# fhausmann/deepgrp

Measured on AMD Instinct MI355X. Metric: Mbp/sec predicted (whole node) at window=200 stride=50, 5-class, higher is better.
Workload: dtype f16

## Files before the change

deepgrp_amd/_lib.py:

```python
from __future__ import annotations

import ctypes as C
import os

_HERE = os.path.dirname(os.path.abspath(__file__))
LIB_PATH = os.path.join(_HERE, "libdeepgrp_hip.so")

i64, i32, vp, cint = C.c_int64, C.c_int32, C.c_void_p, C.c_int


class DgrpError(RuntimeError):
    """A libdeepgrp_hip call failed (message from dgrp_last_error())."""


class Segment(C.Structure):
    _fields_ = [("start", C.c_int64), ("end", C.c_int64), ("label", C.c_int32), ("contig", C.c_int32)]


class TrainJob(C.Structure):
    _fields_ = [("T", cint), ("u", cint), ("C", cint), ("attention", cint), ("d_params", vp), ("d_idx", vp), ("d_truth", vp),
                ("n", i64), ("d_starts", vp), ("B", i64), ("d_masks", vp), ("d_loss", vp), ("d_grads", vp), ("d_work", vp),
                ("work_bytes", i64)]


# ... 11 lines not shown
    "dgrp_fasta_batch_workspace_bytes": (i64, [i64, i64]),
    "dgrp_fasta_encode_batch": (cint, [vp, i64, vp, vp, vp, vp, vp, i64, vp]),
    "dgrp_fasta_chunks_workspace_bytes": (i64, [i64]),
    "dgrp_fasta_chunks": (cint, [vp, i64, i64, vp, vp, C.POINTER(i64), vp, i64, vp]),
    "dgrp_fasta_mask_workspace_bytes": (i64, [i64, i64, i64]),
    "dgrp_fasta_mask_batch": (cint, [vp, i64, vp, vp, vp, vp, cint, C.c_uint64, vp, vp, i64, vp]),
    "dgrp_fasta_extract_workspace_bytes": (i64, [i64, i64, i64]),
    "dgrp_fasta_extract_batch": (cint, [vp, i64, vp, vp, vp, vp, vp, vp, i64, cint, C.c_uint64, vp, i64, C.POINTER(i64), vp, C.POINTER(i64),
                                        vp, i64, vp]),
    "dgrp_twobit_workspace_bytes": (i64, [i64]),
    "dgrp_twobit_encode_batch": (cint, [vp, i64, i64, vp, vp, vp, vp, i64, vp, vp, i64, vp, i64, vp]),
    "dgrp_twobit_text_batch": (cint, [vp, i64, i64, vp, vp, vp, vp, vp, vp, i64, vp, vp, i64, vp, vp, i64, vp, i64, vp]),
    "dgrp_twobit_pack_workspace_bytes": (i64, [i64, i64]),
    "dgrp_twobit_pack_batch": (cint, [vp, i64, vp, vp, vp, i64, i64, vp, vp, vp, i64, vp]),
    "dgrp_format_rows_bound": (i64, [i64, i64]),
    "dgrp_format_rows": (cint, [vp, vp, i64, cint, vp, i64, vp, i64, C.POINTER(i64)]),
    "dgrp_track_workspace_bytes": (i64, [i64, i64]),
    "dgrp_track_text": (cint, [vp, i64, cint, cint, cint, i64, i64, C.c_char_p, i64, vp, i64, C.POINTER(i64), vp, i64, vp]),
    "dgrp_track_batch_workspace_bytes": (i64, [i64, vp, vp, i64, cint, i64]),
    "dgrp_track_text_batch": (cint, [vp, cint, i64, vp, vp, vp, C.c_char_p, vp, vp, cint, cint, i64, vp, i64, vp, vp, i64, vp]),
    "dgrp_track_index_workspace_bytes": (i64, [i64, vp, vp, i64, cint, i64]),
    "dgrp_track_index_batch": (cint, [vp, cint, i64, vp, vp, vp, C.c_char_p, vp, vp, cint, cint, i64, vp, i64, vp, vp, i64, vp, i64, vp]),
    "dgrp_track_sections_workspace_bytes": (i64, [i64, vp, vp, i64, cint]),
    "dgrp_track_sections_batch": (cint, [vp, cint, i64, vp, vp, vp, vp, cint, cint, i64, i64, vp, i64, vp, vp, i64, vp, vp, i64, vp]),
    "dgrp_track_zoom_workspace_bytes": (i64, [i64, vp, vp, i64, cint]),
    "dgrp_track_zoom_batch": (cint, [vp, cint, i64, vp, vp, vp, vp, cint, cint, i64, i64, vp, i64, vp, vp, i64, vp, vp, vp, i64, vp]),
    "dgrp_zlib_bound": (i64, [i64, i64]),
    "dgrp_zlib_workspace_bytes": (i64, [i64, cint]),
    "dgrp_zlib_compress_batch": (cint, [vp, i64, vp, i64, i64, cint, vp, i64, vp, C.POINTER(i64), vp, i64, vp]),
    "dgrp_zlib_compress_host": (cint, [vp, i64, vp, i64, i64, cint, vp, i64, vp, C.POINTER(i64)]),
    "dgrp_window_count":(i64, [i64, i64, i64]),
    "dgrp_windows_onehot": (cint, [vp, i64, i64, i64, i64, i64, cint, vp, vp]),
    "dgrp_model_create": (cint, [C.POINTER(vp), cint, cint, cint, cint, vp, vp, vp, vp, vp, vp]),
    "dgrp_model_create_lstm": (cint, [C.POINTER(vp), cint, cint, cint, vp, vp, vp, vp, vp]),
    "dgrp_model_destroy": (cint, [vp]),
    "dgrp_model_dims": (cint, [vp, C.POINTER(cint), C.POINTER(cint), C.POINTER(cint), C.POINTER(cint)]),
    "dgrp_model_flags": (cint, [vp]),
    "dgrp_model_set_precision": (cint, [vp, cint]),
    "dgrp_model_view": (cint, [vp, cint, C.POINTER(vp)]),
    "dgrp_model_plan": (cint, [vp, cint, i64, C.POINTER(cint), C.POINTER(i64), C.POINTER(cint), C.POINTER(cint)]),
    "dgrp_forward_workspace_bytes": (i64, [vp, i64]),
    "dgrp_forward_window_chunk": (i64, [vp]),
    "dgrp_forward_windows": (cint, [vp, vp, i64, i64, i64, i64, vp, vp, i64, vp]),
    "dgrp_forward_merge": (cint, [vp, vp, i64, i64, i64, i64, i64, vp, vp, i64, vp]),
    "dgrp_forward_merge_record": (cint, [vp, vp, i64, i64, i64, vp, vp, i64, vp]),
    "dgrp_forward_merge_record_workspace_bytes": (i64, [vp, i64, i64]),
    "dgrp_forward_reference_workspace_bytes": (i64, [vp, i64]),
    "dgrp_forward_windows_reference": (cint, [vp, vp, i64, i64, i64, i64, vp, vp, i64, vp]),
    "dgrp_get_max": (cint, [vp, i64, vp, i64, i64, i64, i64, vp]),
    "dgrp_scores": (cint, [vp, i64, cint, vp, vp, vp]),
    "dgrp_softmax_labels": (cint, [vp, i64, cint, vp, vp, vp, i64, vp]),
    "dgrp_mss_workspace_bytes": (i64, [i64]),
    "dgrp_mss_labels": (cint, [vp, vp, i64, cint, cint, cint, vp, vp, vp, i64, vp]),
    "dgrp_mss_segments_host": (cint, [vp, i64, vp, i64, C.POINTER(i64)]),
    "dgrp_mss_batch_workspace_bytes": (i64, [i64, i64]),
    "dgrp_mss_labels_batch": (cint, [vp, vp, i64, i64, vp, cint, cint, cint, vp, vp, i64, vp]),
    "dgrp_segments_workspace_bytes": (i64, [i64]),
    "dgrp_segments": (cint, [vp, i64, i64, i32, vp, i64, vp, vp, i64, vp]),
    "dgrp_record_workspace_bytes": (i64, [vp, i64, i64, cint]),
    "dgrp_predict_record": (cint, [vp, vp, i64, i64, i64, cint, cint, cint, i64, i32, vp, i64, C.POINTER(i64), vp, i64, vp]),
    "dgrp_batch_workspace_bytes": (i64, [vp, i64, vp, i64]),
    "dgrp_predict_batch": (cint, [vp, vp, i64, vp, vp, vp, vp, i64, i64, cint, cint, vp, i64, C.POINTER(i64), vp, i64, vp]),
    "dgrp_batch_rows": (i64, [i64, vp]),
    "dgrp_predict_batch_probs": (cint, [vp, vp, i64, vp, vp, vp, vp, i64, i64, cint, cint, vp, i64, C.POINTER(i64), vp, i64, vp, vp]),
    "dgrp_confusion_matrix": (cint, [vp, vp, i64, cint, vp, vp, vp]),
    "dgrp_filter_segments": (cint, [vp, vp, i64, i64, vp]),
    "dgrp_eval_workspace_bytes": (i64, [i64, i64]),
    "dgrp_paint_rows_batch": (cint, [vp, i64, vp, vp, vp, vp, vp, vp, i64, vp]),
    "dgrp_row_hits_batch": (cint, [vp, i64, vp, vp, vp, vp, vp, vp, vp, i64, vp]),
    "dgrp_row_scores_workspace_bytes": (i64, [i64, i64]),
    "dgrp_row_scores_batch": (cint, [vp, cint, i64, vp, vp, vp, vp, vp, vp, vp, i64, vp]),
    "dgrp_prob_hist_workspace_bytes": (i64, [i64, cint, cint]),
    "dgrp_prob_hist_batch": (cint, [vp, cint, i64, vp, vp, vp, vp, cint, vp, vp, vp, i64, vp]),
    "dgrp_row_detect_workspace_bytes": (i64, [i64, i64]),
    "dgrp_paint_row_keys_batch": (cint, [vp, i64, vp, vp, vp, vp, vp, vp, vp, i64, vp]),
    "dgrp_row_detect_batch": (cint, [vp, i64, vp, vp, vp, vp, vp, vp, vp, vp, i64, vp]),
    "dgrp_format_bed_bound": (i64, [i64, i64]),
    "dgrp_format_bed_rows": (cint, [vp, vp, i64, cint, vp, vp, i64, cint, vp, i64, C.POINTER(i64)]),
    "dgrp_bed_text_workspace_bytes": (i64, [i64, i64, i64]),
    "dgrp_bed_text_batch": (cint, [vp, vp, i64, cint, vp, vp, i64, cint, vp, i64, C.POINTER(i64), vp, i64, vp]),
    "dgrp_bed_index_workspace_bytes": (i64, [i64, i64, i64, i64]),
    "dgrp_bed_index_batch": (cint, [vp, vp, i64, cint, vp, vp, i64, cint, i64, vp, vp, i64, C.POINTER(i64), vp, i64, vp, vp, i64, vp]),
    "dgrp_gff_text_workspace_bytes": (i64, [i64, i64, i64, i64, i64]),
    "dgrp_gff_text_batch": (cint, [vp, vp, i64, cint, vp, vp, i64, vp, vp, i64, cint, i64, vp, i64, C.POINTER(i64), C.POINTER(i64), vp, i64,
                                   vp]),
    "dgrp_gff_index_workspace_bytes": (i64, [i64, i64, i64, i64, i64, i64]),
    "dgrp_gff_index_batch": (cint, [vp, vp, i64, cint, vp, vp, i64, vp, vp, i64, cint, i64, i64, vp, vp, i64, C.POINTER(i64), vp, i64, vp, vp,
                                    i64, vp]),
    "dgrp_bed_blocks_workspace_bytes": (i64, [i64, i64, vp]),
    "dgrp_bed_blocks_batch": (cint, [cint, vp, vp, i64, cint, i64, vp, i64, vp, i64, C.POINTER(i64), vp, i64, C.POINTER(i64), C.POINTER(i64),
                                     vp, i64, vp]),
    "dgrp_bed_zoom_workspace_bytes": (i64, [i64, i64, vp]),
    "dgrp_bed_zoom_batch": (cint, [cint, vp, vp, i64, cint, i64, vp, i64, vp, i64, vp, vp, i64, vp, vp, vp, i64, vp]),
    "dgrp_inflate_raw_host": (cint, [vp, i64, vp, i64, C.POINTER(i64), C.POINTER(i64), C.POINTER(cint)]),
    "dgrp_inflate_workspace_bytes": (i64, [i64]),
    "dgrp_inflate_batch": (cint, [vp, i64, i64, vp, vp, vp, vp, i64, C.POINTER(i64), C.POINTER(cint), vp, i64, vp]),
    "dgrp_bgzf_bound": (i64, [i64, cint]),
    "dgrp_bgzf_workspace_bytes": (i64, [i64]),
    "dgrp_bgzf_compress": (cint, [vp, i64, vp, i64, C.POINTER(i64), cint, vp, i64, vp]),
    "dgrp_bgzf_compress_host": (cint, [vp, i64, vp, i64, C.POINTER(i64), cint]),
    "dgrp_bgzf_workspace_bytes_level": (i64, [i64, cint]),
    "dgrp_bgzf_compress_level": (cint, [vp, i64, vp, i64, C.POINTER(i64), cint, cint, vp, i64, vp]),
    "dgrp_bgzf_compress_host_level": (cint, [vp, i64, vp, i64, C.POINTER(i64), cint, cint]),
    "dgrp_train_param_count": (i64, [cint, cint, cint]),
    "dgrp_train_workspace_bytes": (i64, [cint, cint, cint, cint, i64]),
    "dgrp_train_step": (cint, [cint, cint, cint, cint, vp, vp, vp, i64, vp, i64, vp, vp, vp, vp, i64, vp]),
# ... 50 lines not shown
```

deepgrp_amd/csrc/api.hip:

```cpp
#include "dgrp_model.h"

#include <stdarg.h>
#include <string.h>

#include <algorithm>
#include <vector>
#include <mutex>

static thread_local char g_err[512] = "";

void dgrp_set_error(const char *fmt, ...)
{
    va_list ap;
    va_start(ap, fmt);
    vsnprintf(g_err, sizeof(g_err), fmt, ap);
    va_end(ap);
}

DGRP_EXPORT int dgrp_abi_version(void) { return DGRP_ABI_VERSION; }
DGRP_EXPORT const char *dgrp_last_error(void) { return g_err; }

DGRP_EXPORT int dgrp_device_info(char *name, size_t name_cap, int *cu_count, int64_t *hbm_bytes)
{
    int dev = 0;
// ... 795 lines not shown

struct record_layout {
    int64_t out, scores, cls, labels, count, fwd, post, bytes, post_bytes, fwd_bytes;
};

static record_layout record_carve(const dgrp_model *m, int64_t n, int64_t s, int use_mss)
{
    record_layout l;
    int64_t p = 0;
    auto take = [&](int64_t b) { const int64_t q = p; p += dgrp_align_up(b, 256); return q; };
    const int64_t nwin = dgrp_window_count(n, m->T, s);
    l.out = take(n * m->C * 4);
    l.scores = take(use_mss ? n * 8 : 0);
    l.cls = take(use_mss ? n : 0);
    l.labels = take(n);
    l.count = take(8);
    l.fwd_bytes = record_forward_bytes(m, nwin);
    l.fwd = take(l.fwd_bytes);
    l.post_bytes = std::max<int64_t>(std::max<int64_t>(use_mss ? dgrp_mss_workspace_bytes(n) : 4096, dgrp_segments_workspace_bytes(n)), 4096);
    l.post = take(l.post_bytes);
    l.bytes = p;
    return l;
}

DGRP_EXPORT int64_t dgrp_record_workspace_bytes(const dgrp_model *m, int64_t n, int64_t s, int use_mss)
{
    if (!m || n < 0 || s < 1) return 0;
    return record_carve(m, n, s, use_mss).bytes;
}

DGRP_EXPORT int dgrp_predict_record(const dgrp_model *m, const uint8_t *d_idx, int64_t n, int64_t s, int64_t batch,
                                    int min_mss_len, int xdrop_len, int use_mss, int64_t offset, int32_t contig,
                                    dgrp_segment *d_records, int64_t cap, int64_t *h_count, void *d_work,
                                    int64_t work_bytes, void *stream_)
{
    hipStream_t stream = (hipStream_t)stream_;
    DGRP_REQUIRE(m && n >= 0 && s >= 1 && batch >= 1 && cap >= 0 && h_count, "dgrp_predict_record: bad arguments");
    *h_count = 0;
    if (n == 0) return DGRP_OK;
    DGRP_REQUIRE(d_idx && d_work && (cap == 0 || d_records), "dgrp_predict_record: NULL pointer");
    const record_layout l = record_carve(m, n, s, use_mss);
    if (work_bytes < l.bytes) {
        dgrp_set_error("dgrp_predict_record: workspace %lld < %lld bytes", (long long)work_bytes, (long long)l.bytes);
        return DGRP_ENOMEM;
    }
    char *w = (char *)d_work;
    float *out = (float *)(w + l.out);
    int8_t *labels = (int8_t *)(w + l.labels);
    int64_t *d_count = (int64_t *)(w + l.count);
    DGRP_HIP(hipMemsetAsync(out, 0, (size_t)n * m->C * 4, stream));
    int rc = dgrp_forward_merge_record(m, d_idx, n, s, batch, out, w + l.fwd, l.fwd_bytes, stream);
    if (rc) return rc;
    if (use_mss) {
        rc = dgrp_scores(out, n, m->C, (double *)(w + l.scores), (int8_t *)(w + l.cls), stream);
        if (rc) return rc;
        rc = dgrp_mss_labels((const double *)(w + l.scores), (const int8_t *)(w + l.cls), n, m->C, min_mss_len, xdrop_len,
                             labels, nullptr, w + l.post, l.post_bytes, stream);
    } else {
        rc = dgrp_softmax_labels(out, n, m->C, nullptr, labels, w + l.post, l.post_bytes, stream);
    }
    if (rc) return rc;
    rc = dgrp_segments(labels, n, offset, contig, d_records, cap, d_count, w + l.post, l.post_bytes, stream);
    if (rc) return rc;
    DGRP_HIP(hipMemcpyAsync(h_count, d_count, 8, hipMemcpyDeviceToHost, stream));
    DGRP_HIP(hipStreamSynchronize(stream));
    return DGRP_OK;
}

int dgrp_batch_marks(const int64_t *d_start, const int64_t *d_len, int64_t nrec, int64_t total_n, uint8_t *d_marks,
                     double *d_scores, int8_t *d_cls, hipStream_t stream);
int dgrp_batch_segments(const int8_t *d_labels, const uint8_t *d_marks, int64_t total_n, const int64_t *d_start, int64_t nrec,
                        const int64_t *d_startpos, const int32_t *d_contig, dgrp_segment *d_records, int64_t cap,
                        int64_t *d_count, void *d_work, int64_t work_bytes, hipStream_t stream);

struct batch_layout {
    int64_t out, scores, cls, labels, marks, count, recs, wgf, start, len, spos, contig, post, post_bytes, avg, pl, queue, bytes;
};

static batch_layout batch_carve(const dgrp_model *m, int64_t nrec, int64_t total_rows, int64_t total_windows)
{
    batch_layout l;
    int64_t p = 0;
    auto take = [&](int64_t b) { const int64_t q = p; p += dgrp_align_up(b, 256); return q; };
    l.out = take(total_rows * m->C * 4);
    l.scores = take(total_rows * 8);
    l.cls = take(total_rows);
    l.labels = take(total_rows);
    l.marks = take(total_rows);
    l.count = take(8);
    l.recs = take(nrec * 64);
    l.wgf = take((nrec + 1) * 8);
    l.start = take((nrec + 1) * 8);
    l.len = take(nrec * 8);
    l.spos = take(nrec * 8);
    l.contig = take(nrec * 4);
    l.post_bytes = std::max<int64_t>(std::max<int64_t>(dgrp_mss_batch_workspace_bytes(total_rows, nrec), dgrp_segments_workspace_bytes(total_rows)), 4096);
    l.post = take(l.post_bytes);
    l.avg = take(m->attention ? total_windows * m->T * (int64_t)m->UP * 4 : 0);
    l.pl = take(m->attention ? total_windows * m->T * (int64_t)m->C * 4 : 0);
    l.queue = take(4);
    l.bytes = p;
    return l;
}

static int64_t batch_windows(const dgrp_model *m, int64_t nrec, const int64_t *h_n, int64_t s)
{
    int64_t w = 0;
    for (int64_t r = 0; r < nrec; ++r) w += dgrp_window_count(h_n[r], m->T, s);
    return w;
}
// ... 114 lines not shown
```

deepgrp_amd/csrc/bigbed_kernels.hip:

```cpp
#include "dgrp_common.h"
#include "bbi_zoom.h"
#include "bed_rows.h"
#include "scan.h"
#include <string.h>
#include <vector>

namespace {

#define BB_BLOCK_ITEMS 512
#define BB_ITEM_MAX 60
#define BB_MAX_END 0xffffffffll
#define BB_R0 1024

struct bb_in {
    const dgrp_segment *rows;
    const dgrp_row_score *scores;
    int64_t nrows;
    const int64_t *rec_end;
    int64_t nrec;
    int by_contig;
    uint64_t min_score;
};

__device__ __forceinline__ int64_t bb_rec(const bb_in &A, const dgrp_segment &row) { return A.by_contig ? row.contig : 0; }
// ... 330 lines not shown
                                    dgrp_track_zoom_block *d_table, int64_t table_cap, int64_t *h_block_off, dgrp_track_totals *h_totals,
                                    void *d_work, int64_t work_bytes, void *stream_)
{
    static const char who[] = "dgrp_bed_zoom_batch";
    hipStream_t stream = (hipStream_t)stream_;
    DGRP_REQUIRE(h_record_off && h_block_off && h_totals, "%s: NULL h_record_off, h_block_off or h_totals", who);
    for (int s = 0; s <= BBI_LEVELS; ++s) h_record_off[s] = h_block_off[s] = 0;
    memset(h_totals, 0, sizeof *h_totals);
    const int rc = bb_check(who, by_contig, nrows, nrec, h_rec_end, chrom0, cap, table_cap);
    if (rc != DGRP_OK) return rc;
    if (nrows == 0) return DGRP_OK;
    DGRP_REQUIRE(d_rows && d_scores && (d_out || cap == 0) && (d_table || table_cap == 0), "%s: bad arguments (NULL rows, scores, output or table)",
                 who);
    DGRP_REQUIRE(((uintptr_t)d_out & 15) == 0 && ((uintptr_t)d_table & 7) == 0, "%s: d_out must be 16-byte and d_table 8-byte aligned", who);
    bbz_layout l;
    DGRP_REQUIRE(bbz_carve(nrows, nrec, h_rec_end, &l), "%s: too many zoom windows in one call", who);
    if (!d_work || work_bytes < l.bytes) {
        dgrp_set_error("%s: workspace too small (%lld < %lld bytes)", who, (long long)work_bytes, (long long)l.bytes);
        return DGRP_ENOMEM;
    }
    char *w = (char *)d_work;
    const bbi_levels &Z = l.Z;
    const std::vector<int64_t> wpref = bbi_wpref(Z, nrec, nullptr, h_rec_end);
    int64_t *d_wpref = (int64_t *)(w + l.wpref);
    DGRP_HIP(hipMemcpyAsync(d_wpref, wpref.data(), wpref.size() * 8, hipMemcpyHostToDevice, stream));
    std::vector<int64_t> tab;
    bb_in A;
    int rc2 = bb_front(by_contig, d_rows, d_scores, nrows, min_score, nrec, h_rec_end, w, l.rec_end, l.eidx, 0, l.len, l.tiles, stream, tab, &A);
    if (rc2 != DGRP_OK) return rc2;
    bed_head *d_head = (bed_head *)w;
    uint64_t *eidx = (uint64_t *)(w + l.eidx), *len = (uint64_t *)(w + l.len), *tiles = (uint64_t *)(w + l.tiles);
    uint64_t *wtiles = (uint64_t *)(w + l.wtiles), *grand = (uint64_t *)(w + l.grand), *segb = (uint64_t *)(w + l.segb);
    bbz_win *win = (bbz_win *)(w + l.win);
    bbz_rows Rw;
    Rw.count = &d_head->lines;
    Rw.skey = (uint64_t *)(w + l.skey); Rw.ekey = (uint64_t *)(w + l.ekey); Rw.lpref = (uint64_t *)(w + l.lpref);
    const dim3 grid((unsigned)((nrows + 255) / 256)), block(256);
    uint64_t *lsum = (uint64_t *)(w + l.lsum);
    rc2 = device_exclusive_scan(len, lsum, nrows, tiles, nullptr, stream);
    if (rc2 != DGRP_OK) return rc2;
    hipLaunchKernelGGL(bbz_compact_kernel, grid, block, 0, stream, A, (const uint64_t *)len, (const uint64_t *)lsum, (const uint64_t *)eidx, Rw);
    DGRP_LAUNCH_CHECK();
    hipLaunchKernelGGL(bbz_level0_kernel, dim3((unsigned)((Z.seg[1] - Z.seg[0]) / 256)), block, 0, stream, Rw, A.rec_end, (const int64_t *)d_wpref,
                       nrec, Z, win);
    DGRP_LAUNCH_CHECK();
    for (int k = 1; k < BBI_LEVELS; ++k) {
        hipLaunchKernelGGL((bbi_reduce_kernel<bbz_win, bbz_start>), dim3((unsigned)((Z.seg[k + 1] - Z.seg[k]) / 256)), block, 0, stream, bbz_start(),
                           (const int64_t *)d_wpref, nrec, Z, k, win);
        DGRP_LAUNCH_CHECK();
    }
    const int64_t ntiles = Z.seg[BBI_LEVELS] / 256;
    hipLaunchKernelGGL(bbi_count_kernel<bbz_win>, dim3((unsigned)ntiles), block, 0, stream, (const bbz_win *)win, wtiles);
    DGRP_LAUNCH_CHECK();
    hipLaunchKernelGGL(scan_sums_kernel, dim3(1), block, 0, stream, wtiles, ntiles, grand);
    DGRP_LAUNCH_CHECK();
    hipLaunchKernelGGL((bbi_bounds_kernel<bbz_win, true>), dim3(1), block, 0, stream, (const bbz_win *)win, (const uint64_t *)wtiles,
                       (const uint64_t *)grand, Z, 1, segb, grand + 1);
    DGRP_LAUNCH_CHECK();
    bed_head head;
    uint64_t off[2 * (BBI_LEVELS + 1)], covered = 0;
    DGRP_HIP(hipMemcpyAsync(&head, w, sizeof head, hipMemcpyDeviceToHost, stream));
    DGRP_HIP(hipMemcpyAsync(off, segb, sizeof off, hipMemcpyDeviceToHost, stream));
    DGRP_HIP(hipMemcpyAsync(&covered, grand + 1, 8, hipMemcpyDeviceToHost, stream));
    DGRP_HIP(hipStreamSynchronize(stream));
    rc2 = bed_refusal(who, head);
    if (rc2 != DGRP_OK) return rc2;
    for (int s = 0; s <= BBI_LEVELS; ++s) {
        h_record_off[s] = (int64_t)off[s];
        h_block_off[s] = (int64_t)off[BBI_LEVELS + 1 + s];
    }
    if (covered) {
        h_totals->covered = h_totals->sum = h_totals->sumsq = covered;
        h_totals->qmin = h_totals->qmax = 1;
    }
    if (h_record_off[BBI_LEVELS] == 0 || 32 * h_record_off[BBI_LEVELS] > cap || h_block_off[BBI_LEVELS] > table_cap) return DGRP_OK;
    hipLaunchKernelGGL((bbi_write_kernel<bbz_win, bbz_tail>), dim3((unsigned)ntiles), block, 0, stream, (const bbz_win *)win, (const int64_t *)d_wpref,
                       nrec, Z, bbz_tail(), (const uint64_t *)wtiles, (const uint64_t *)segb, 1, (uint32_t)chrom0, (uint4 *)d_out, d_table);
    DGRP_LAUNCH_CHECK();
    return DGRP_OK;
}
```

deepgrp_amd/csrc/bigwig_kernels.hip:

```cpp
#include "dgrp_common.h"
#include "deflate.h"
#include "deflate_blocks.h"
#include "scan.h"
#include "track_chain.h"
#include "bbi_zoom.h"
#include <string.h>
#include <vector>

namespace {

#define BW_SECTION_ITEMS 1024
#define BW_MAX_END 0xffffffffll

__device__ __forceinline__ float bw_value(uint64_t v, double scale) { return (float)((double)v / scale); }

struct bw_run { uint32_t v; bool first, last; int64_t r, lo, hi; };

__device__ __forceinline__ bw_run bw_run_of(const uint32_t *__restrict__ qk, const tb_rec *__restrict__ recs,
                                            const int64_t *__restrict__ pref, const tb_geom &G, int64_t r0, int64_t f0, int64_t f)
{
    bw_run t;
    t.v = f < G.NB ? qk[f] : 0u;
    t.first = t.last = false;
    t.r = t.lo = t.hi = 0;
// ... 396 lines not shown
}

static int64_t zlib_workspace(int64_t nblk, int level)
{
    const int64_t base = dgrp_align_up(nblk * DGRP_BGZF_SLOT, 256) + dgrp_align_up((nblk + 2) * 8, 256);
    return level == 0 ? base : base + nblk * DGRP_BGZF_BLOCK * (int64_t)sizeof(uint32_t);
}

}

DGRP_EXPORT int64_t dgrp_track_sections_workspace_bytes(int64_t nrec, const int64_t *h_n, const int64_t *h_startpos, int64_t bin, int ncls)
{
    bws_layout l;
    if (bin < 1 || ncls < 1) return 0;
    return bws_carve(nrec, h_n, h_startpos, bin, ncls, &l) ? l.bytes : 0;
}

DGRP_EXPORT int dgrp_track_sections_batch(const float *d_probs, int C, int64_t nrec, const int64_t *h_row0, const int64_t *h_n,
                                          const int64_t *h_startpos, const int *h_cls, int ncls, int digits, int64_t bin, int64_t chrom0,
                                          char *d_out, int64_t cap, int64_t *h_class_off, dgrp_track_section *d_table, int64_t table_cap,
                                          int64_t *h_section_off, void *d_work, int64_t work_bytes, void *stream_)
{
    const char *who = "dgrp_track_sections_batch";
    DGRP_REQUIRE(h_class_off && h_section_off, "%s: NULL h_class_off or h_section_off", who);
    if (ncls >= 1 && ncls <= DGRP_MAXC)
        for (int k = 0; k <= ncls; ++k) h_class_off[k] = h_section_off[k] = 0;
    const int rc0 = bw_check(who, d_probs, C, nrec, h_row0, h_n, h_startpos, h_cls, ncls, digits, bin, chrom0);
    if (rc0 != DGRP_OK) return rc0;
    DGRP_REQUIRE(cap >= 0 && table_cap >= 0, "%s: bad cap/table_cap (%lld, %lld)", who, (long long)cap, (long long)table_cap);
    if (nrec == 0) return DGRP_OK;
    DGRP_REQUIRE((d_out || cap == 0) && (d_table || table_cap == 0) && d_work, "%s: NULL pointer", who);
    DGRP_REQUIRE(((uintptr_t)d_out & 3) == 0 && ((uintptr_t)d_table & 7) == 0, "%s: d_out must be 4-byte and d_table 8-byte aligned", who);
    bws_layout l;
    DGRP_REQUIRE(bws_carve(nrec, h_n, h_startpos, bin, ncls, &l), "%s: too many bins in one call", who);
    if (work_bytes < l.bytes) {
        dgrp_set_error("%s: workspace %lld < %lld bytes", who, (long long)work_bytes, (long long)l.bytes);
        return DGRP_ENOMEM;
    }
    hipStream_t stream = (hipStream_t)stream_;
    char *w = (char *)d_work;
    unsigned long long *cnt = (unsigned long long *)(w + l.cnt);
    uint64_t *ipref = (uint64_t *)(w + l.ipref), *spref = (uint64_t *)(w + l.spref), *base = (uint64_t *)(w + l.base);
    uint64_t *hb = (uint64_t *)(w + l.hb);
    std::vector<int64_t> name_off((size_t)nrec + 1, 0);
    std::vector<char> tab;
    tb_dev D;
    const int rc = dgrp_tb_bins(d_probs, C, nrec, h_row0, h_n, h_startpos, nullptr, name_off.data(), h_cls, ncls, digits, bin, d_work, l.t,
                                stream, tab, &D);
    if (rc != DGRP_OK) return rc;
    DGRP_HIP(hipMemsetAsync(cnt, 0, (size_t)(nrec * ncls) * 8, stream));
    const dim3 grid((unsigned)D.ntiles), block(256);
    hipLaunchKernelGGL(bw_count_kernel, grid, block, 0, stream, D.q, D.recs, D.pref, D.G, D.tiles, cnt);
    DGRP_LAUNCH_CHECK();
    hipLaunchKernelGGL(scan_sums_kernel, dim3(1), block, 0, stream, D.tiles, D.ntiles, D.grand);
    DGRP_LAUNCH_CHECK();
    hipLaunchKernelGGL(bw_prefix_kernel, dim3((unsigned)ncls), block, 0, stream, cnt, nrec, ipref, spref);
    DGRP_LAUNCH_CHECK();
    hipLaunchKernelGGL(bw_bounds_kernel, dim3(1), dim3(64), 0, stream, ipref, spref, nrec, ncls, base, hb);
    DGRP_LAUNCH_CHECK();
    std::vector<uint64_t> off(2 * ((size_t)ncls + 1), 0);
    DGRP_HIP(hipMemcpyAsync(off.data(), hb, off.size() * 8, hipMemcpyDeviceToHost, stream));
    DGRP_HIP(hipStreamSynchronize(stream));
    for (int k = 0; k <= ncls; ++k) {
        h_class_off[k] = (int64_t)off[(size_t)k];
        h_section_off[k] = (int64_t)off[(size_t)(ncls + 1 + k)];
    }
    if (h_class_off[ncls] == 0 || h_class_off[ncls] > cap || h_section_off[ncls] > table_cap) return DGRP_OK;
    double scale = 1.0;
    for (int k = 0; k < digits; ++k) scale *= 10.0;
    hipLaunchKernelGGL(bw_write_kernel, grid, block, 0, stream, D.q, D.recs, D.pref, D.G, scale, D.tiles, cnt, ipref, spref, base, (uint32_t)chrom0,
                       d_out, d_table);
    DGRP_LAUNCH_CHECK();
    DGRP_HIP(hipStreamSynchronize(stream));
    return DGRP_OK;
}

DGRP_EXPORT int64_t dgrp_track_zoom_workspace_bytes(int64_t nrec, const int64_t *h_n, const int64_t *h_startpos, int64_t bin, int ncls)
{
    bwz_layout l;
    if (bin < 1 || ncls < 1) return 0;
    return bwz_carve(nrec, h_n, h_startpos, bin, ncls, &l) ? l.bytes : 0;
}

DGRP_EXPORT int dgrp_track_zoom_batch(const float *d_probs, int C, int64_t nrec, const int64_t *h_row0, const int64_t *h_n,
                                      const int64_t *h_startpos, const int *h_cls, int ncls, int digits, int64_t bin, int64_t chrom0,
                                      char *d_out, int64_t cap, int64_t *h_record_off, dgrp_track_zoom_block *d_table, int64_t table_cap,
                                      int64_t *h_block_off, dgrp_track_totals *h_totals, void *d_work, int64_t work_bytes, void *stream_)
{
    const char *who = "dgrp_track_zoom_batch";
    DGRP_REQUIRE(h_record_off && h_block_off && h_totals, "%s: NULL h_record_off, h_block_off or h_totals", who);
    if (ncls >= 1 && ncls <= DGRP_MAXC) {
        for (int s = 0; s <= ncls * BBI_LEVELS; ++s) h_record_off[s] = h_block_off[s] = 0;
        memset(h_totals, 0, (size_t)ncls * sizeof(dgrp_track_totals));
    }
    const int rc0 = bw_check(who, d_probs, C, nrec, h_row0, h_n, h_startpos, h_cls, ncls, digits, bin, chrom0);
    if (rc0 != DGRP_OK) return rc0;
    DGRP_REQUIRE(bin <= (1ll << 32), "%s: bad bin %lld (zoom windows of 16 * bin * 4^9 bases)", who, (long long)bin);
    DGRP_REQUIRE(cap >= 0 && table_cap >= 0, "%s: bad cap/table_cap (%lld, %lld)", who, (long long)cap, (long long)table_cap);
    if (nrec == 0) return DGRP_OK;
    DGRP_REQUIRE((d_out || cap == 0) && (d_table || table_cap == 0) && d_work, "%s: NULL pointer", who);
    DGRP_REQUIRE(((uintptr_t)d_out & 15) == 0 && ((uintptr_t)d_table & 7) == 0, "%s: d_out must be 16-byte and d_table 8-byte aligned", who);
    bwz_layout l;
    DGRP_REQUIRE(bwz_carve(nrec, h_n, h_startpos, bin, ncls, &l), "%s: too many bins in one call", who);
    if (work_bytes < l.bytes) {
        dgrp_set_error("%s: workspace %lld < %lld bytes", who, (long long)work_bytes, (long long)l.bytes);
        return DGRP_ENOMEM;
    }
    hipStream_t stream = (hipStream_t)stream_;
    char *w = (char *)d_work;
    const bbi_levels &Z = l.Z;
    int64_t *d_wpref = (int64_t *)(w + l.wpref);
    bwz_win *win = (bwz_win *)(w + l.win);
    uint64_t *tiles = (uint64_t *)(w + l.tiles), *grand = (uint64_t *)(w + l.grand), *segb = (uint64_t *)(w + l.segb);
    dgrp_track_totals *d_totals = (dgrp_track_totals *)(w + l.totals);
    const int nseg = ncls * BBI_LEVELS;
    const std::vector<int64_t> wpref = bbi_wpref(Z, nrec, h_startpos, h_n);
    DGRP_HIP(hipMemcpyAsync(d_wpref, wpref.data(), wpref.size() * 8, hipMemcpyHostToDevice, stream));
    std::vector<int64_t> name_off((size_t)nrec + 1, 0);
    std::vector<char> tab;
    tb_dev D;
    const int rc = dgrp_tb_bins(d_probs, C, nrec, h_row0, h_n, h_startpos, nullptr, name_off.data(), h_cls, ncls, digits, bin, d_work, l.t,
                                stream, tab, &D);
    if (rc != DGRP_OK) return rc;
    const dim3 block(256);
    hipLaunchKernelGGL(bwz_level0_kernel, dim3((unsigned)((Z.seg[1] - Z.seg[0]) / 256 * ncls)), block, 0, stream, D.q, D.recs, D.pref, d_wpref,
                       D.G, Z, win);
    DGRP_LAUNCH_CHECK();
    for (int k = 1; k < BBI_LEVELS; ++k) {
        hipLaunchKernelGGL((bbi_reduce_kernel<bwz_win, bwz_start>), dim3((unsigned)((Z.seg[k + 1] - Z.seg[k]) / 256 * ncls)), block, 0, stream,
                           bwz_start{D.recs}, d_wpref, nrec, Z, k, win);
        DGRP_LAUNCH_CHECK();
    }
    const int64_t ntiles = Z.seg[BBI_LEVELS] / 256 * ncls;
    hipLaunchKernelGGL(bbi_count_kernel<bwz_win>, dim3((unsigned)ntiles), block, 0, stream, win, tiles);
    DGRP_LAUNCH_CHECK();
    hipLaunchKernelGGL(scan_sums_kernel, dim3(1), block, 0, stream, tiles, ntiles, grand);
    DGRP_LAUNCH_CHECK();
    hipLaunchKernelGGL((bbi_bounds_kernel<bwz_win, false>), dim3(1), dim3(64), 0, stream, win, tiles, grand, Z, ncls, segb, nullptr);
    DGRP_LAUNCH_CHECK();
    hipLaunchKernelGGL(bwz_totals_kernel, dim3((unsigned)ncls), block, 0, stream, win, Z, d_totals);
    DGRP_LAUNCH_CHECK();
    std::vector<uint64_t> off(2 * ((size_t)nseg + 1), 0);
    DGRP_HIP(hipMemcpyAsync(off.data(), segb, off.size() * 8, hipMemcpyDeviceToHost, stream));
    DGRP_HIP(hipMemcpyAsync(h_totals, d_totals, (size_t)ncls * sizeof(dgrp_track_totals), hipMemcpyDeviceToHost, stream));
    DGRP_HIP(hipStreamSynchronize(stream));
    for (int s = 0; s <= nseg; ++s) {
        h_record_off[s] = (int64_t)off[(size_t)s];
        h_block_off[s] = (int64_t)off[(size_t)(nseg + 1 + s)];
    }
    if (h_record_off[nseg] == 0 || 32 * h_record_off[nseg] > cap || h_block_off[nseg] > table_cap) return DGRP_OK;
    double scale = 1.0;
    for (int k = 0; k < digits; ++k) scale *= 10.0;
    hipLaunchKernelGGL((bbi_write_kernel<bwz_win, bwz_tail>), dim3((unsigned)ntiles), block, 0, stream, win, d_wpref, nrec, Z, bwz_tail{scale}, tiles,
                       segb, ncls, (uint32_t)chrom0, (uint4 *)d_out, d_table);
    DGRP_LAUNCH_CHECK();
    DGRP_HIP(hipStreamSynchronize(stream));
    return DGRP_OK;
}

DGRP_EXPORT int64_t dgrp_zlib_bound(int64_t nblk, int64_t in_bytes) { return nblk < 0 || in_bytes < 0 ? 0 : in_bytes + ZLIB_EMPTY * nblk; }

DGRP_EXPORT int64_t dgrp_zlib_workspace_bytes(int64_t nblk, int level)
{
    return nblk < 0 || nblk > INT32_MAX - 1 || level < 0 || level > 1 ? 0 : zlib_workspace(nblk, level);
}

DGRP_EXPORT int dgrp_zlib_compress_batch(const uint8_t *d_in, int64_t in_bytes, const void *d_rows, int64_t stride, int64_t nblk, int level,
                                         uint8_t *d_out, int64_t out_cap, int64_t *d_sizes, int64_t *h_out_bytes, void *d_work,
                                         int64_t work_bytes, void *stream_)
{
    const char *who = "dgrp_zlib_compress_batch";
    DGRP_REQUIRE(h_out_bytes, "%s: NULL h_out_bytes", who);
    *h_out_bytes = 0;
    DGRP_REQUIRE(in_bytes >= 0 && nblk >= 0 && nblk <= INT32_MAX - 1 && out_cap >= 0 && work_bytes >= 0, "%s: bad arguments", who);
    DGRP_REQUIRE(stride >= 16 && stride % 8 == 0, "%s: a row is at least an int64 offset and an int64 length (stride %lld)", who,
                 (long long)stride);
    DGRP_REQUIRE(level == 0 || level == 1, "%s: level %d (0: literals, 1: matches)", who, level);
    if (nblk == 0) return DGRP_OK;
    DGRP_REQUIRE((d_in || in_bytes == 0) && d_rows && (d_out || out_cap == 0) && d_sizes && d_work, "%s: NULL pointer", who);
    DGRP_REQUIRE(((uintptr_t)d_work & 15) == 0 && ((uintptr_t)d_rows & 7) == 0, "%s: d_work must be 16-byte, d_rows 8-byte aligned", who);
    if (work_bytes < zlib_workspace(nblk, level)) {
        dgrp_set_error("%s: workspace too small", who);
        return DGRP_ENOMEM;
    }
    hipStream_t stream = (hipStream_t)stream_;
    uint8_t *slots = (uint8_t *)d_work;
    uint64_t *sizes = (uint64_t *)(slots + dgrp_align_up(nblk * DGRP_BGZF_SLOT, 256));
    uint32_t *lz = level == 0 ? nullptr : (uint32_t *)((uint8_t *)sizes + dgrp_align_up((nblk + 2) * 8, 256));
    unsigned long long *bad = (unsigned long long *)(sizes + nblk + 1);
    const char *rows = (const char *)d_rows;
    DGRP_HIP(hipMemsetAsync(bad, 0, 8, stream));
    const int rc = dgrp_deflate_members(d_in, in_bytes, rows, stride, nblk, level, slots, sizes, lz, stream);
    if (rc != DGRP_OK) return rc;
    hipLaunchKernelGGL(zlib_sizes_kernel, dim3((unsigned)((nblk + 255) / 256)), dim3(256), 0, stream, rows, stride, nblk, in_bytes, sizes, bad);
    DGRP_LAUNCH_CHECK();
    hipLaunchKernelGGL(scan_sums_kernel, dim3(1), dim3(256), 0, stream, sizes, nblk, sizes + nblk);
    DGRP_LAUNCH_CHECK();
    hipLaunchKernelGGL(zlib_place_kernel, dim3((unsigned)nblk), dim3(256), 0, stream, d_in, rows, stride, slots, sizes, nblk, bad, d_out, out_cap,
                       d_sizes);
    DGRP_LAUNCH_CHECK();
    uint64_t tail[2] = {0, 0};
    DGRP_HIP(hipMemcpyAsync(tail, sizes + nblk, 16, hipMemcpyDeviceToHost, stream));
    DGRP_HIP(hipStreamSynchronize(stream));
    DGRP_REQUIRE(tail[1] == 0, "%s: %llu rows do not lie in the input or are longer than 65280 bytes (nothing written)", who,
                 (unsigned long long)tail[1]);
    *h_out_bytes = (int64_t)tail[0];
    if (*h_out_bytes > out_cap) {
        dgrp_set_error("%s: output of %lld bytes, %lld needed (nothing written)", who, (long long)out_cap, (long long)*h_out_bytes);
        return DGRP_ENOMEM;
    }
    return DGRP_OK;
}

DGRP_EXPORT int dgrp_zlib_compress_host(const uint8_t *h_in, int64_t in_bytes, const void *h_rows, int64_t stride, int64_t nblk, int level,
                                        uint8_t *h_out, int64_t out_cap, int64_t *h_sizes, int64_t *h_out_bytes)
{
    const char *who = "dgrp_zlib_compress_host";
    DGRP_REQUIRE(h_out_bytes, "%s: NULL h_out_bytes", who);
    *h_out_bytes = 0;
    DGRP_REQUIRE(in_bytes >= 0 && nblk >= 0 && out_cap >= 0, "%s: bad arguments", who);
    DGRP_REQUIRE(stride >= 16 && stride % 8 == 0, "%s: a row is at least an int64 offset and an int64 length (stride %lld)", who,
                 (long long)stride);
    DGRP_REQUIRE(level == 0 || level == 1, "%s: level %d (0: literals, 1: matches)", who, level);
    if (nblk == 0) return DGRP_OK;
    DGRP_REQUIRE((h_in || in_bytes == 0) && h_rows && (h_out || out_cap == 0) && h_sizes, "%s: NULL pointer", who);
    for (int64_t m = 0; m < nblk; ++m) {
        const int64_t *row = (const int64_t *)((const char *)h_rows + m * stride);
        DGRP_REQUIRE(row[0] >= 0 && row[1] >= 0 && row[1] <= DGRP_BGZF_BLOCK && row[0] <= in_bytes - row[1],
                     "%s: row %lld (offset %lld, %lld bytes) does not lie in the input or is longer than 65280 bytes", who, (long long)m,
                     (long long)row[0], (long long)row[1]);
    }
    std::vector<uint32_t> slot(DGRP_BGZF_SLOT / 4), lz(level ? DGRP_BGZF_BLOCK : 0);
    std::vector<uint16_t> head(level ? 1 << DGRP_LZ_HASH_BITS : 0);
    dgrp_deflate_plan plan;
    dgrp_lz_plan lzplan;
    int64_t pos = 0;
    bool fits = true;
    for (int64_t m = 0; m < nblk; ++m) {
        const int64_t *row = (const int64_t *)((const char *)h_rows + m * stride);
        const uint8_t *src = h_in + row[0];
        const uint32_t len = (uint32_t)row[1];
        uint32_t size = ZLIB_EMPTY;
        if (len > 0)
            size = (level ? dgrp_bgzf_member_serial_lz(src, len, slot.data(), &plan, &lzplan, lz.data(), head.data())
                          : dgrp_bgzf_member_serial(src, len, slot.data(), &plan)) - 20;
        uint32_t a = 1, b = 0;
        for (uint32_t i = 0; i < len; ++i) {
            a = (a + src[i]) % ZLIB_MOD;
            b = (b + a) % ZLIB_MOD;
// ... 24 lines not shown
```

deepgrp_amd/csrc/deflate_kernels.hip:

```cpp
#include "dgrp_common.h"
#include "deflate.h"
#include "deflate_blocks.h"
#include "scan.h"
#include <string.h>
#include <mutex>
#include <vector>

namespace {

#define DEFLATE_THREADS 256
#define DEFLATE_RUN 16
#define DEFLATE_ROUND (DEFLATE_THREADS * DEFLATE_RUN)

struct deflate_shared {
    dgrp_deflate_plan plan;
    uint32_t hist[DEFLATE_THREADS / 64][DGRP_DEFLATE_NSYM];
    uint32_t crctab[256];
    uint64_t scan[4];
    uint32_t crc[DEFLATE_THREADS / 64];
};
struct deflate_lds {
    uint32_t image[DGRP_BGZF_SLOT / 4];
    deflate_shared s;
};
// ... 484 lines not shown

DGRP_EXPORT int64_t dgrp_bgzf_workspace_bytes(int64_t n) { return n < 0 ? 0 : bgzf_workspace(n, 0); }

DGRP_EXPORT int64_t dgrp_bgzf_workspace_bytes_level(int64_t n, int level)
{
    return n < 0 || level < 0 || level > 1 ? 0 : bgzf_workspace(n, level);
}

static int bgzf_compress_device(const char *who, const uint8_t *d_in, int64_t n, uint8_t *d_out, int64_t out_cap, int64_t *h_out_bytes, int eof,
                                int level, void *d_work, int64_t work_bytes, hipStream_t stream)
{
    if (!(n >= 0 && out_cap >= 0 && work_bytes >= 0 && h_out_bytes)) {
        dgrp_set_error("%s: bad arguments", who);
        return DGRP_EINVAL;
    }
    *h_out_bytes = 0;
    const int64_t nmem = bgzf_members(n);
    if (level < 0 || level > 1) {
        dgrp_set_error("%s: level %d (0: literals, 1: matches)", who, level);
        return DGRP_EINVAL;
    }
    if (nmem > INT32_MAX - 1) {
        dgrp_set_error("%s: too many members", who);
        return DGRP_EINVAL;
    }
    if (!(n == 0 || (d_in && d_work)) || !(d_out || (n == 0 && !eof) || out_cap == 0)) {
        dgrp_set_error("%s: NULL pointer", who);
        return DGRP_EINVAL;
    }
    if (n == 0) {
        if (!eof) return DGRP_OK;
        *h_out_bytes = DGRP_BGZF_EOF_BYTES;
        if (out_cap < DGRP_BGZF_EOF_BYTES) {
            dgrp_set_error("%s: output of %lld bytes, the EOF member takes %d", who, (long long)out_cap, DGRP_BGZF_EOF_BYTES);
            return DGRP_ENOMEM;
        }
        DGRP_HIP(hipMemcpyAsync(d_out, BGZF_EOF_MEMBER, DGRP_BGZF_EOF_BYTES, hipMemcpyHostToDevice, stream));
        DGRP_HIP(hipStreamSynchronize(stream));
        return DGRP_OK;
    }
    if (work_bytes < bgzf_workspace(n, level)) {
        dgrp_set_error("%s: workspace too small", who);
        return DGRP_ENOMEM;
    }
    if (((uintptr_t)d_work & 15) != 0) {
        dgrp_set_error("%s: d_work must be 16-byte aligned", who);
        return DGRP_EINVAL;
    }
    uint8_t *slots = (uint8_t *)d_work;
    uint64_t *sizes = (uint64_t *)(slots + dgrp_align_up(nmem * DGRP_BGZF_SLOT, 256));
    uint32_t *lz = level == 0 ? nullptr : (uint32_t *)((uint8_t *)sizes + dgrp_align_up((nmem + 1) * 8, 256));
    const int rc = dgrp_deflate_members(d_in, n, nullptr, 0, nmem, level, slots, sizes, lz, stream);
    if (rc != DGRP_OK) return rc;
    hipLaunchKernelGGL(scan_sums_kernel, dim3(1), dim3(256), 0, stream, sizes, nmem, sizes + nmem);
    DGRP_LAUNCH_CHECK();
    hipLaunchKernelGGL(bgzf_place_kernel, dim3((unsigned)(nmem + (eof ? 1 : 0))), dim3(256), 0, stream, slots, sizes, nmem, eof, d_out, out_cap);
    DGRP_LAUNCH_CHECK();
    uint64_t all = 0;
    DGRP_HIP(hipMemcpyAsync(&all, sizes + nmem, 8, hipMemcpyDeviceToHost, stream));
    DGRP_HIP(hipStreamSynchronize(stream));
    *h_out_bytes = (int64_t)all + (eof ? DGRP_BGZF_EOF_BYTES : 0);
    if (*h_out_bytes > out_cap) {
        dgrp_set_error("%s: output of %lld bytes, %lld needed (nothing written)", who, (long long)out_cap, (long long)*h_out_bytes);
        return DGRP_ENOMEM;
    }
    return DGRP_OK;
}

static int bgzf_compress_host(const char *who, const uint8_t *h_in, int64_t n, uint8_t *h_out, int64_t out_cap, int64_t *h_out_bytes, int eof,
                              int level)
{
    if (!(n >= 0 && out_cap >= 0 && h_out_bytes)) {
        dgrp_set_error("%s: bad arguments", who);
        return DGRP_EINVAL;
    }
    *h_out_bytes = 0;
    if (level < 0 || level > 1) {
        dgrp_set_error("%s: level %d (0: literals, 1: matches)", who, level);
        return DGRP_EINVAL;
    }
    if (!(h_in || n == 0) || !(h_out || (n == 0 && !eof) || out_cap == 0)) {
        dgrp_set_error("%s: NULL pointer", who);
        return DGRP_EINVAL;
    }
    std::vector<uint32_t> slot(DGRP_BGZF_SLOT / 4), lz(level ? DGRP_BGZF_BLOCK : 0);
    std::vector<uint16_t> head(level ? 1 << DGRP_LZ_HASH_BITS : 0);
    dgrp_deflate_plan plan;
    dgrp_lz_plan lzplan;
    int64_t pos = 0;
    bool fits = true;
    for (int64_t o = 0; o < n; o += DGRP_BGZF_BLOCK) {
        const uint32_t k = (uint32_t)(n - o < DGRP_BGZF_BLOCK ? n - o : DGRP_BGZF_BLOCK);
        const uint32_t size = level ? dgrp_bgzf_member_serial_lz(h_in + o, k, slot.data(), &plan, &lzplan, lz.data(), head.data())
                                    : dgrp_bgzf_member_serial(h_in + o, k, slot.data(), &plan);
        fits = fits && pos + size <= out_cap;
        if (fits) memcpy(h_out + pos, slot.data(), size);
        pos += size;
    }
    if (eof) {
        fits = fits && pos + DGRP_BGZF_EOF_BYTES <= out_cap;
        if (fits) memcpy(h_out + pos, BGZF_EOF_MEMBER, DGRP_BGZF_EOF_BYTES);
        pos += DGRP_BGZF_EOF_BYTES;
    }
    *h_out_bytes = pos;
    if (!fits) {
        dgrp_set_error("%s: output of %lld bytes, %lld needed", who, (long long)out_cap, (long long)pos);
        return DGRP_ENOMEM;
// ... 28 lines not shown
```

deepgrp_amd/csrc/extract_kernels.hip:

```cpp
#include "dgrp_common.h"
#include "body_tiles.h"
#include "scan.h"
#include <vector>

namespace {

#define EXTRACT_TILE 4096
#define BODY_WORDS (BODY_TILE / 16)

__global__ void __launch_bounds__(256) extract_count_kernel(const uint8_t *__restrict__ raw, const int64_t *__restrict__ tile0,
                                                            const int64_t *__restrict__ off, const int64_t *__restrict__ len,
                                                            int64_t nrec, uint64_t *__restrict__ tilecnt, uint16_t *__restrict__ wordpre)
{
    __shared__ uint64_t lds[4];
    __shared__ int64_t s_rec;
    const int64_t t = blockIdx.x;
    if (threadIdx.x == 0) s_rec = dgrp_record_of(tile0, nrec, t);
    __syncthreads();
    const int64_t r = s_rec;
    const body_span s = body_lane_span(off[r], len[r], t - tile0[r]);
    alignas(16) uint8_t b[16];
    body_load(raw, s, b);
    uint64_t c = 0;
    for (int j = 0; j < 16; ++j) c += body_lineend(b[j]) ? 0 : 1;
// ... 289 lines not shown
                     "dgrp_fasta_extract_batch: record ranges must ascend and not overlap (record %lld)", (long long)r);
        DGRP_REQUIRE(h_row_off[r + 1] >= h_row_off[r], "dgrp_fasta_extract_batch: row offsets must ascend (record %lld)", (long long)r);
        DGRP_REQUIRE(h_name_off[r + 1] >= h_name_off[r] && h_name_off[r + 1] - h_name_off[r] <= (1 << 20),
                     "dgrp_fasta_extract_batch: name offsets must ascend, a name has at most 2^20 bytes (record %lld)", (long long)r);
        total += h_len[r];
        off[r] = h_off[r];
        len[r] = h_len[r];
        tile0[r + 1] = tile0[r] + body_tiles_of(h_off[r], h_len[r]);
    }
    for (int64_t r = 0; r <= nrec; ++r) {
        row_off[r] = h_row_off[r];
        name_off[r] = h_name_off[r];
    }
    const int64_t ntiles = tile0[nrec], nrows = row_off[nrec] - row_off[0];
    if (nrows == 0) return DGRP_OK;
    DGRP_REQUIRE(nrows < ((int64_t)1 << 31), "dgrp_fasta_extract_batch: more than 2^31 - 1 rows");
    if (work_bytes < dgrp_fasta_extract_workspace_bytes(nrec, total, nrows)) {
        dgrp_set_error("dgrp_fasta_extract_batch: workspace too small");
        return DGRP_ENOMEM;
    }
    DGRP_REQUIRE(d_work && d_rows && (ntiles == 0 || d_raw) && (name_off[nrec] == name_off[0] || d_names) && (text_cap == 0 || d_text),
                 "dgrp_fasta_extract_batch: NULL device pointer");
    DGRP_REQUIRE(((uintptr_t)d_raw & 15) == 0, "dgrp_fasta_extract_batch: d_raw must be 16-byte aligned");
    DGRP_REQUIRE(((uintptr_t)d_entries & 7) == 0 && ((uintptr_t)d_rows & 7) == 0 && ((uintptr_t)d_work & 255) == 0,
                 "dgrp_fasta_extract_batch: d_rows and d_entries must be 8-byte aligned, d_work 256-byte aligned");
    char *w = (char *)d_work;
    unsigned long long *g = (unsigned long long *)w;
    w += 256;
    uint64_t *ex = (uint64_t *)w;
    w += dgrp_align_up((body_tile_bound(nrec, total) + 1) * 8, 256);
    uint16_t *wordpre = (uint16_t *)w;
    w += dgrp_align_up(body_tile_bound(nrec, total) * BODY_WORDS * 2, 256);
    int64_t *d_tab = (int64_t *)w;
    w += dgrp_align_up((5 * nrec + 3) * 8, 256);
    uint64_t *rowpos = (uint64_t *)w;
    w += dgrp_align_up((nrows + 1) * 8, 256);
    uint64_t *kidx = (uint64_t *)w;
    w += dgrp_align_up((nrows + 1) * 8, 256);
    uint64_t *scan_a = (uint64_t *)w;
    w += dgrp_align_up(extract_scan_tiles(nrows) * 8, 256);
    uint64_t *scan_b = (uint64_t *)w;
    extract_tables T;
    T.tile0 = d_tab; T.off = d_tab + nrec + 1; T.len = T.off + nrec; T.row_off = T.len + nrec; T.name_off = T.row_off + nrec + 1;
    T.ex = ex; T.wordpre = wordpre; T.rows = d_rows; T.names = d_names;
    T.nrec = nrec; T.flank = flank; T.width = width; T.class_mask = class_mask;
    const unsigned long long init[4] = { 0ull, ~0ull, 0ull, 0ull };
    DGRP_HIP(hipMemcpyAsync(g, init, sizeof(init), hipMemcpyHostToDevice, stream));
    DGRP_HIP(hipMemcpyAsync(d_tab, tab.data(), tab.size() * 8, hipMemcpyHostToDevice, stream));
    if (ntiles > 0) {
        hipLaunchKernelGGL(extract_count_kernel, dim3((unsigned)ntiles), dim3(256), 0, stream, d_raw, T.tile0, T.off, T.len, nrec, ex,
                           wordpre);
        DGRP_LAUNCH_CHECK();
    }
    hipLaunchKernelGGL(scan_sums_kernel, dim3(1), dim3(256), 0, stream, ex, ntiles, ex + ntiles);
    DGRP_LAUNCH_CHECK();
    hipLaunchKernelGGL(extract_size_kernel, dim3((unsigned)((nrows + 1 + 255) / 256)), dim3(256), 0, stream, T, g, rowpos, kidx);
    DGRP_LAUNCH_CHECK();
    int rc = device_exclusive_scan(rowpos, rowpos, nrows + 1, scan_a, (uint64_t *)(g + 2), stream);
    if (rc != DGRP_OK) return rc;
    rc = device_exclusive_scan(kidx, kidx, nrows + 1, scan_b, (uint64_t *)(g + 3), stream);
    if (rc != DGRP_OK) return rc;
    unsigned long long hg[4];
    DGRP_HIP(hipMemcpyAsync(hg, g, sizeof(hg), hipMemcpyDeviceToHost, stream));
    DGRP_HIP(hipStreamSynchronize(stream));
    if (hg[0]) {
        const int64_t i = (int64_t)hg[1];
        int64_t r = 0;
        while (r + 1 < nrec && row_off[r + 1] <= i) ++r;
        dgrp_segment q;
        uint64_t e[2];
        DGRP_HIP(hipMemcpyAsync(&q, d_rows + i, sizeof(q), hipMemcpyDeviceToHost, stream));
        DGRP_HIP(hipMemcpyAsync(&e[0], ex + tile0[r], 8, hipMemcpyDeviceToHost, stream));
        DGRP_HIP(hipMemcpyAsync(&e[1], ex + tile0[r + 1], 8, hipMemcpyDeviceToHost, stream));
        DGRP_HIP(hipStreamSynchronize(stream));
        DGRP_REQUIRE(false, "dgrp_fasta_extract_batch: row %lld [%lld, %lld) of record %lld is empty, out of order or beyond its "
                            "sequence of %lld characters", (long long)i, (long long)q.start, (long long)q.end, (long long)r,
                     (long long)(e[1] - e[0]));
    }
    const int64_t text_bytes = (int64_t)hg[2];
    *h_text_bytes = text_bytes;
    *h_kept = (int64_t)hg[3];
    if (text_bytes > text_cap) {
        dgrp_set_error("dgrp_fasta_extract_batch: the text has %lld bytes, d_text holds %lld", (long long)text_bytes, (long long)text_cap);
        return DGRP_ENOMEM;
    }
    if (text_bytes == 0) return DGRP_OK;
    DGRP_REQUIRE((text_bytes + EXTRACT_TILE - 1) / EXTRACT_TILE < ((int64_t)1 << 31), "dgrp_fasta_extract_batch: more than 2^43 bytes of text");
    if (d_entries) {
        hipLaunchKernelGGL(extract_entries_kernel, dim3((unsigned)((nrows + 255) / 256)), dim3(256), 0, stream, T, rowpos, kidx,
                           d_entries);
        DGRP_LAUNCH_CHECK();
    }
    hipLaunchKernelGGL(extract_write_kernel, dim3((unsigned)((text_bytes + EXTRACT_TILE - 1) / EXTRACT_TILE)), dim3(256), 0, stream,
                       d_raw, T, rowpos, text_bytes, d_text);
    DGRP_LAUNCH_CHECK();
    return DGRP_OK;
}
```

deepgrp_amd/csrc/fasta_kernels.hip:

```cpp
#include "dgrp_common.h"
#include "scan.h"
#include <vector>
#include <algorithm>
#include <string.h>

__device__ __forceinline__ uint32_t fasta_class_of(uint32_t c)
{
    uint32_t l = c | 0x20u;
    return l == 'a' ? 0u : l == 'c' ? 1u : l == 'g' ? 2u : l == 't' ? 3u : 4u;
}

__global__ void __launch_bounds__(256) fasta_count_kernel(const uint8_t *__restrict__ raw, int64_t n, uint64_t *__restrict__ tilecnt,
                                                          unsigned long long *__restrict__ g)
{
    __shared__ uint64_t lds[4];
    const int64_t base = (int64_t)blockIdx.x * SCAN_TILE;
    uint64_t c = 0;
    bool bad = false;
    for (int j = 0; j < 8; ++j) {
        const int64_t i = base + j * 256 + threadIdx.x;
        if (i < n) {
            const uint32_t b = raw[i];
            const bool lineend = b == '\n' || b == '\r';
            c += lineend ? 0 : 1;
// ... 34 lines not shown
        if ((b[j] | 0x20u) != 'n') {
            if ((long long)ex < first) first = (long long)ex;
            last = (long long)ex + 1;
        }
        ++ex;
    }
    for (int o = 32; o > 0; o >>= 1) {
        const long long f2 = __shfl_xor(first, o), l2 = __shfl_xor(last, o);
        first = f2 < first ? f2 : first;
        last = l2 > last ? l2 : last;
    }
    __shared__ long long red[8];
    if ((threadIdx.x & 63) == 0) { red[threadIdx.x >> 6] = first; red[4 + (threadIdx.x >> 6)] = last; }
    __syncthreads();
    if (threadIdx.x == 0) {
        for (int w = 1; w < 4; ++w) {
            first = red[w] < first ? red[w] : first;
            last = red[4 + w] > last ? red[4 + w] : last;
        }
        if (last >= 0) {
            const volatile unsigned long long *gv = g;
            if ((unsigned long long)first < gv[1]) atomicMin((unsigned long long *)&g[1], (unsigned long long)first);
            if ((unsigned long long)last > gv[2]) atomicMax((unsigned long long *)&g[2], (unsigned long long)last);
        }
    }
}

DGRP_EXPORT int64_t dgrp_fasta_workspace_bytes(int64_t nbytes)
{
    if (nbytes < 0) return 0;
    return dgrp_align_up(((nbytes + SCAN_TILE - 1) / SCAN_TILE + 2) * 8, 256) + 256;
}

DGRP_EXPORT int dgrp_fasta_encode(const uint8_t *d_raw, int64_t nbytes, uint8_t *d_idx, int64_t *h_info, void *d_work,
                                  int64_t work_bytes, void *stream_)
{
    hipStream_t stream = (hipStream_t)stream_;
    DGRP_REQUIRE(nbytes >= 0 && h_info, "dgrp_fasta_encode: bad arguments");
    h_info[0] = 1; h_info[1] = 0; h_info[2] = 0; h_info[3] = 0;
    if (nbytes == 0) return DGRP_OK;
    DGRP_REQUIRE(d_raw && d_idx && d_work, "dgrp_fasta_encode: NULL pointer");
    if (work_bytes < dgrp_fasta_workspace_bytes(nbytes)) {
        dgrp_set_error("dgrp_fasta_encode: workspace too small");
        return DGRP_ENOMEM;
    }
    const int64_t ntiles = (nbytes + SCAN_TILE - 1) / SCAN_TILE;
    uint64_t *tiles = (uint64_t *)d_work;
    uint64_t *grand = tiles + ntiles + 1;
    unsigned long long *g = (unsigned long long *)((char *)d_work + dgrp_fasta_workspace_bytes(nbytes) - 256);
    const unsigned long long init[3] = { 0ull, 0x7fffffffffffffffull, 0ull };
    DGRP_HIP(hipMemcpyAsync(g, init, sizeof(init), hipMemcpyHostToDevice, stream));
    hipLaunchKernelGGL(fasta_count_kernel, dim3((unsigned)ntiles), dim3(256), 0, stream, d_raw, nbytes, tiles, g);
    DGRP_LAUNCH_CHECK();
    hipLaunchKernelGGL(scan_sums_kernel, dim3(1), dim3(256), 0, stream, tiles, ntiles, grand);
    DGRP_LAUNCH_CHECK();
    hipLaunchKernelGGL(fasta_scatter_kernel, dim3((unsigned)ntiles), dim3(256), 0, stream, d_raw, nbytes, tiles, d_idx, g);
    DGRP_LAUNCH_CHECK();
    unsigned long long hg[3];
    uint64_t total = 0;
    DGRP_HIP(hipMemcpyAsync(hg, g, sizeof(hg), hipMemcpyDeviceToHost, stream));
    DGRP_HIP(hipMemcpyAsync(&total, grand, 8, hipMemcpyDeviceToHost, stream));
    DGRP_HIP(hipStreamSynchronize(stream));
    h_info[0] = hg[0] ? 0 : 1;
    h_info[1] = (int64_t)total;
    if (hg[2] == 0) {
        h_info[2] = (int64_t)total;
        h_info[3] = -(int64_t)total;
    } else {
        h_info[2] = (int64_t)hg[1];
        h_info[3] = (int64_t)hg[2] - (int64_t)hg[1];
    }
    return DGRP_OK;
}

__global__ void __launch_bounds__(256) fasta_record_kernel(const uint8_t *__restrict__ raw_base, const int64_t *__restrict__ off,
                                                           const int64_t *__restrict__ len, const uint8_t *__restrict__ small,
                                                           uint8_t *__restrict__ idx_base, unsigned long long *__restrict__ gbase)
{
    __shared__ uint64_t lds[4];
    const int64_t r = blockIdx.x;
    if (!small[r]) return;
    const int64_t n = len[r];
    const uint8_t *raw = raw_base + off[r];
    uint8_t *idx = idx_base + off[r];
    unsigned long long *g = gbase + r * 32;
    uint64_t running = 0;
    bool bad = false;
    long long first = 0x7fffffffffffffffll, last = -1;
    for (int64_t t0 = 0; t0 < n; t0 += SCAN_TILE) {
        const int64_t base = t0 + (int64_t)threadIdx.x * 8;
        uint32_t b[8];
        uint64_t c = 0;
        for (int j = 0; j < 8; ++j) {
            const int64_t i = base + j;
            b[j] = i < n ? raw[i] : (uint32_t)'\n';
            if (i < n) {
                const bool lineend = b[j] == '\n' || b[j] == '\r';
                c += lineend ? 0 : 1;
                if (b[j] >= 128 || (b[j] <= 32 && !lineend)) bad = true;
                if (b[j] == '\r' && (i + 1 >= n || raw[i + 1] != '\n')) bad = true;
                if (b[j] == '\n') {
                    if (i == 0) bad = true;
                    if (i + 1 < n && raw[i + 1] == '\n') bad = true;
                    if (i + 2 < n && raw[i + 1] == '\r' && raw[i + 2] == '\n') bad = true;
                }
                if (b[j] == '\r' && i == 0) bad = true;
            }
// ... 31 lines not shown
{
    if (nrec < 0 || total_bytes < 0) return 0;
    return dgrp_align_up(((total_bytes + SCAN_TILE - 1) / SCAN_TILE + 4 * nrec + 8) * 8, 256) + nrec * 256 + dgrp_align_up(nrec * 17, 256) + 256;
}

DGRP_EXPORT int dgrp_fasta_encode_batch(const uint8_t *d_raw, int64_t nrec, const int64_t *h_off, const int64_t *h_len,
                                        uint8_t *d_idx, int64_t *h_info, void *d_work, int64_t work_bytes, void *stream_)
{
    hipStream_t stream = (hipStream_t)stream_;
    DGRP_REQUIRE(nrec >= 0 && (nrec == 0 || (h_off && h_len && h_info)), "dgrp_fasta_encode_batch: bad arguments");
    if (nrec == 0) return DGRP_OK;
    int64_t total = 0;
    for (int64_t r = 0; r < nrec; ++r) {
        DGRP_REQUIRE(h_off[r] >= 0 && h_len[r] >= 0, "dgrp_fasta_encode_batch: negative range");
        total += h_len[r];
    }
    DGRP_REQUIRE(total == 0 || (d_raw && d_idx && d_work), "dgrp_fasta_encode_batch: NULL pointer");
    if (work_bytes < dgrp_fasta_batch_workspace_bytes(nrec, total)) {
        dgrp_set_error("dgrp_fasta_encode_batch: workspace too small");
        return DGRP_ENOMEM;
    }
    const int64_t tile_words = (total + SCAN_TILE - 1) / SCAN_TILE + 4 * nrec + 8;
    uint64_t *tiles_base = (uint64_t *)d_work;
    unsigned long long *gbase = (unsigned long long *)((char *)d_work + dgrp_align_up(tile_words * 8, 256));
    std::vector<unsigned long long> init((size_t)nrec * 32, 0ull);
    for (int64_t r = 0; r < nrec; ++r) init[(size_t)r * 32 + 1] = 0x7fffffffffffffffull;
    DGRP_HIP(hipMemcpyAsync(gbase, init.data(), init.size() * 8, hipMemcpyHostToDevice, stream));
    const int64_t SMALL_BYTES = 1 << 20;
    unsigned char *tab = (unsigned char *)(gbase + nrec * 32);
    int64_t *d_off = (int64_t *)tab, *d_len = d_off + nrec;
    uint8_t *d_small = (uint8_t *)(d_len + nrec);
    std::vector<uint8_t> small((size_t)nrec);
    bool any_small = false;
    for (int64_t r = 0; r < nrec; ++r) { small[(size_t)r] = h_len[r] > 0 && h_len[r] <= SMALL_BYTES; any_small |= small[(size_t)r] != 0; }
    if (any_small) {
        DGRP_HIP(hipMemcpyAsync(d_off, h_off, (size_t)nrec * 8, hipMemcpyHostToDevice, stream));
        DGRP_HIP(hipMemcpyAsync(d_len, h_len, (size_t)nrec * 8, hipMemcpyHostToDevice, stream));
        DGRP_HIP(hipMemcpyAsync(d_small, small.data(), (size_t)nrec, hipMemcpyHostToDevice, stream));
        hipLaunchKernelGGL(fasta_record_kernel, dim3((unsigned)nrec), dim3(256), 0, stream, d_raw, d_off, d_len, d_small, d_idx, gbase);
    }
    std::vector<int64_t> grand_at((size_t)nrec, -1);
    int64_t word = 0;
    for (int64_t r = 0; r < nrec; ++r) {
        const int64_t nbytes = h_len[r];
        if (nbytes == 0 || small[(size_t)r]) continue;
        const int64_t ntiles = (nbytes + SCAN_TILE - 1) / SCAN_TILE;
        uint64_t *tiles = tiles_base + word;
        uint64_t *grand = tiles + ntiles + 1;
        grand_at[(size_t)r] = word + ntiles + 1;
        word += ntiles + 3;
        unsigned long long *g = gbase + r * 32;
        const uint8_t *raw = d_raw + h_off[r];
        hipLaunchKernelGGL(fasta_count_kernel, dim3((unsigned)ntiles), dim3(256), 0, stream, raw, nbytes, tiles, g);
        hipLaunchKernelGGL(scan_sums_kernel, dim3(1), dim3(256), 0, stream, tiles, ntiles, grand);
        hipLaunchKernelGGL(fasta_scatter_kernel, dim3((unsigned)ntiles), dim3(256), 0, stream, raw, nbytes, tiles,
                           d_idx + h_off[r], g);
    }
    DGRP_LAUNCH_CHECK();
    std::vector<unsigned long long> hg((size_t)nrec * 32);
    std::vector<uint64_t> htiles((size_t)(word > 0 ? word : 1));
    DGRP_HIP(hipMemcpyAsync(hg.data(), gbase, hg.size() * 8, hipMemcpyDeviceToHost, stream));
    if (word > 0) DGRP_HIP(hipMemcpyAsync(htiles.data(), tiles_base, (size_t)word * 8, hipMemcpyDeviceToHost, stream));
    DGRP_HIP(hipStreamSynchronize(stream));
    for (int64_t r = 0; r < nrec; ++r) {
        int64_t *info = h_info + 4 * r;
        if (h_len[r] == 0) { info[0] = 1; info[1] = 0; info[2] = 0; info[3] = 0; continue; }
        const unsigned long long *g = hg.data() + (size_t)r * 32;
        const int64_t tot = small[(size_t)r] ? (int64_t)g[3] : (int64_t)htiles[(size_t)grand_at[(size_t)r]];
        info[0] = g[0] ? 0 : 1;
        info[1] = tot;
        if (g[2] == 0) { info[2] = tot; info[3] = -tot; }
        else { info[2] = (int64_t)g[1]; info[3] = (int64_t)g[2] - (int64_t)g[1]; }
    }
    return DGRP_OK;
}

__global__ void __launch_bounds__(256) fasta_gt_kernel(const uint8_t *__restrict__ raw, int64_t n, int64_t cap,
                                                       unsigned long long *__restrict__ count, int64_t *__restrict__ list)
{
    const int64_t nvec = n / 16;
    for (int64_t v = (int64_t)blockIdx.x * blockDim.x + threadIdx.x; v <= nvec; v += (int64_t)gridDim.x * blockDim.x) {
        const int64_t p0 = v * 16;
        union { uint4 q; uint8_t b[16]; } u;
        uint8_t *b = u.b;
        int m = 16;
        if (v < nvec) {
            u.q = *(const uint4 *)(raw + p0);
        } else {
            m = (int)(n - p0);
            for (int j = 0; j < m; ++j) b[j] = raw[p0 + j];
        }
        bool any = false;
        for (int j = 0; j < m; ++j) any = any || b[j] == '>';
        if (!any) continue;
        uint8_t prev = p0 > 0 ? raw[p0 - 1] : 0;
        for (int j = 0; j < m; ++j) {
            if (b[j] == '>' && prev == 10 ) {
                const unsigned long long at = atomicAdd(count, 1ull);
                if ((int64_t)at < cap) list[at] = p0 + j;
            }
            prev = b[j];
        }
    }
}

__global__ void __launch_bounds__(256) fasta_firstlf_kernel(const uint8_t *__restrict__ raw, int64_t n, const int64_t *__restrict__ start,
                                                            int64_t nchunks, int64_t *__restrict__ first_lf)
// ... 169 lines not shown
```

deepgrp_amd/csrc/mask_kernels.hip:

```cpp
#include "dgrp_common.h"
#include "body_tiles.h"
#include "scan.h"
#include <vector>

namespace {

#define MASK_LDS_ROWS 256

__global__ void __launch_bounds__(256) mask_count_kernel(const uint8_t *__restrict__ raw, const int64_t *__restrict__ tile0,
                                                         const int64_t *__restrict__ off, const int64_t *__restrict__ len,
                                                         int64_t nrec, uint64_t *__restrict__ tilecnt)
{
    __shared__ uint64_t lds[4];
    __shared__ int64_t s_rec;
    const int64_t t = blockIdx.x;
    if (threadIdx.x == 0) s_rec = dgrp_record_of(tile0, nrec, t);
    __syncthreads();
    const int64_t r = s_rec;
    const body_span s = body_lane_span(off[r], len[r], t - tile0[r]);
    alignas(16) uint8_t b[16];
    body_load(raw, s, b);
    uint64_t c = 0;
    for (int j = 0; j < 16; ++j) c += body_lineend(b[j]) ? 0 : 1;
    for (int o = 32; o > 0; o >>= 1) c += __shfl_xor(c, o);
// ... 98 lines not shown
    } else {
        for (int k = s.lo; k < s.hi; ++k) out[s.word + k] = b[k];
    }
}

}

DGRP_EXPORT int64_t dgrp_fasta_mask_workspace_bytes(int64_t nrec, int64_t total_bytes, int64_t nrows)
{
    if (nrec < 0 || total_bytes < 0 || nrows < 0) return 0;
    const int64_t tiles = body_tile_bound(nrec, total_bytes);
    return 256 + dgrp_align_up((tiles + 1) * 8, 256) + dgrp_align_up((4 * nrec + 2) * 8, 256);
}

DGRP_EXPORT int dgrp_fasta_mask_batch(const uint8_t *d_raw, int64_t nrec, const int64_t *h_off, const int64_t *h_len,
                                      const dgrp_segment *d_rows, const int64_t *h_row_off, int mode, uint64_t class_mask,
                                      uint8_t *d_out, void *d_work, int64_t work_bytes, void *stream_)
{
    hipStream_t stream = (hipStream_t)stream_;
    DGRP_REQUIRE(nrec >= 0 && (nrec == 0 || (h_off && h_len && h_row_off)), "dgrp_fasta_mask_batch: bad arguments");
    DGRP_REQUIRE(mode == 0 || mode == 1, "dgrp_fasta_mask_batch: mode must be 0 (soft) or 1 (hard), got %d", mode);
    if (nrec == 0) return DGRP_OK;
    int64_t total = 0;
    std::vector<int64_t> tab((size_t)(4 * nrec + 2));
    int64_t *tile0 = tab.data(), *off = tile0 + nrec + 1, *len = off + nrec, *row_off = len + nrec;
    DGRP_REQUIRE(h_row_off[0] >= 0, "dgrp_fasta_mask_batch: negative row offset");
    tile0[0] = 0;
    for (int64_t r = 0; r < nrec; ++r) {
        DGRP_REQUIRE(h_off[r] >= 0 && h_len[r] >= 0, "dgrp_fasta_mask_batch: negative range (record %lld)", (long long)r);
        DGRP_REQUIRE(h_row_off[r + 1] >= h_row_off[r], "dgrp_fasta_mask_batch: row offsets must ascend (record %lld)", (long long)r);
        total += h_len[r];
        off[r] = h_off[r];
        len[r] = h_len[r];
        tile0[r + 1] = tile0[r] + body_tiles_of(h_off[r], h_len[r]);
    }
    for (int64_t r = 0; r <= nrec; ++r) row_off[r] = h_row_off[r];
    const int64_t ntiles = tile0[nrec], nrows = row_off[nrec] - row_off[0];
    if (ntiles == 0) return DGRP_OK;
    DGRP_REQUIRE(d_raw && d_out && d_work && (nrows == 0 || d_rows), "dgrp_fasta_mask_batch: NULL pointer");
    DGRP_REQUIRE(((uintptr_t)d_raw & 15) == 0 && ((uintptr_t)d_out & 15) == 0, "dgrp_fasta_mask_batch: d_raw and d_out must be 16-byte aligned");
    if (work_bytes < dgrp_fasta_mask_workspace_bytes(nrec, total, nrows)) {
        dgrp_set_error("dgrp_fasta_mask_batch: workspace too small");
        return DGRP_ENOMEM;
    }
    unsigned long long *g = (unsigned long long *)d_work;
    uint64_t *ex = (uint64_t *)((char *)d_work + 256);
    int64_t *d_tab = (int64_t *)((char *)ex + dgrp_align_up((ntiles + 1) * 8, 256));
    int64_t *d_tile0 = d_tab, *d_off = d_tile0 + nrec + 1, *d_len = d_off + nrec, *d_row_off = d_len + nrec;
    const unsigned long long init[2] = { 0ull, ~0ull };
    DGRP_HIP(hipMemcpyAsync(g, init, sizeof(init), hipMemcpyHostToDevice, stream));
    DGRP_HIP(hipMemcpyAsync(d_tab, tab.data(), tab.size() * 8, hipMemcpyHostToDevice, stream));
    hipLaunchKernelGGL(mask_count_kernel, dim3((unsigned)ntiles), dim3(256), 0, stream, d_raw, d_tile0, d_off, d_len, nrec, ex);
    DGRP_LAUNCH_CHECK();
    hipLaunchKernelGGL(scan_sums_kernel, dim3(1), dim3(256), 0, stream, ex, ntiles, ex + ntiles);
    DGRP_LAUNCH_CHECK();
    if (nrows > 0) {
        hipLaunchKernelGGL(mask_check_kernel, dim3((unsigned)((nrows + 255) / 256)), dim3(256), 0, stream, d_rows, d_row_off, nrec,
                           d_tile0, ex, g);
        DGRP_LAUNCH_CHECK();
        unsigned long long hg[2];
        DGRP_HIP(hipMemcpyAsync(hg, g, sizeof(hg), hipMemcpyDeviceToHost, stream));
        DGRP_HIP(hipStreamSynchronize(stream));
        if (hg[0]) {
            const int64_t i = (int64_t)hg[1];
            int64_t r = 0;
            while (r + 1 < nrec && row_off[r + 1] <= i) ++r;
            dgrp_segment q;
            uint64_t e[2];
            DGRP_HIP(hipMemcpy(&q, d_rows + i, sizeof(q), hipMemcpyDeviceToHost));
            DGRP_HIP(hipMemcpy(&e[0], ex + tile0[r], 8, hipMemcpyDeviceToHost));
            DGRP_HIP(hipMemcpy(&e[1], ex + tile0[r + 1], 8, hipMemcpyDeviceToHost));
            DGRP_REQUIRE(false, "dgrp_fasta_mask_batch: row %lld [%lld, %lld) of record %lld is empty, out of order or beyond its "
                                "sequence of %lld characters", (long long)i, (long long)q.start, (long long)q.end, (long long)r,
                         (long long)(e[1] - e[0]));
        }
    }
    hipLaunchKernelGGL(mask_apply_kernel, dim3((unsigned)ntiles), dim3(256), 0, stream, d_raw, d_out, d_tile0, d_off, d_len,
                       d_row_off, nrec, ex, d_rows, mode, class_mask);
    DGRP_LAUNCH_CHECK();
    if (nrows == 0) DGRP_HIP(hipStreamSynchronize(stream));
    return DGRP_OK;
}
```

deepgrp_amd/csrc/mss_kernels.hip:

```cpp
#include "dgrp_common.h"
#include "scan.h"
#include <vector>
#include <math.h>

struct mss_cand { int32_t st, en; double L, R; int32_t pre, pad; };

#define MSS_SUB_MIN 256
#define MSS_SUBENT_BYTES 80
struct mss_subent {
    int64_t start, run;
    double L, peak, run_L;
    int64_t run_st;
    int32_t open, first;
    int32_t vci, nst;
    int32_t reset, pad;
    double Lf;
};
static_assert(sizeof(mss_subent) == 80, "MSS_SUBENT_BYTES");
#define MSS_LCAP 160
#define MSS_NEG (-1e30)
#define MSS_QNONE (-4096)
#define MSS_QBAD 4096

struct mss_layout {
    int64_t nblk;
    uint64_t *blk;
    double *blk_sum;
    double *blk_abs;
    int32_t *blk_q;
    uint8_t *flags;
    int64_t nsup;
    double *sup_sum, *sup_abs;
    int32_t *sup_q;
    uint8_t *sup_flags;
    uint64_t *tiles;
    uint64_t *grand;
    int64_t *ustart;
    int64_t *urun;
    double *exitL[2];
    uint64_t *segcnt;
    uint64_t *cutcnt;
    uint64_t *lblk;
    int64_t *lstart, *lrun;
    uint8_t *lforced;
    void *lstate[2];
    int64_t *cut_st, *cut_run;
    double *cut_L;
    int2 *cut_kj;
    int64_t *ustart2, *urun2;
    double *entry2;
    void *subs;
    int64_t dump_cap;
    mss_cand *dump;
    mss_cand *stack;
// ... 71 lines not shown
{
    const int qL = quantum_exp(L);
    const int Q = qL > q_scores ? qL : q_scores;
    if (Q >= MSS_QBAD) return false;
    const int ex = 53 - Q;
    if (ex > 1000) return true;
    if (ex < -1000) return false;
    return (fabs(L) + sumabs) * 1.0000001 < ldexp(1.0, ex);
}

__device__ __forceinline__ double wave_sum(double v)
{
#pragma unroll
    for (int o = 32; o > 0; o >>= 1) v += __shfl_xor(v, o);
    return v;
}
__device__ __forceinline__ int wave_max(int v)
{
#pragma unroll
    for (int o = 32; o > 0; o >>= 1) { int w = __shfl_xor(v, o); v = w > v ? w : v; }
    return v;
}

__device__ __forceinline__ double lane_value(double x, int l)
{
    const long long b = __double_as_longlong(x);
    const int lo = __builtin_amdgcn_readlane((int)b, l), hi = __builtin_amdgcn_readlane((int)(b >> 32), l);
    return __longlong_as_double(((long long)hi << 32) | (unsigned int)lo);
}

__global__ void __launch_bounds__(256) mss_blockstat_kernel(const double *__restrict__ S, int64_t n,
                                                            uint64_t *__restrict__ blk, double *__restrict__ blk_sum,
                                                            double *__restrict__ blk_abs, int32_t *__restrict__ blk_q,
                                                            uint8_t *__restrict__ flags)
{
    const int lane = threadIdx.x & 63;
    const int64_t b = (int64_t)blockIdx.x * 4 + (threadIdx.x >> 6);
    if (b * 64 >= n) return;
    const int64_t i = b * 64 + lane;
    const double s = i < n ? S[i] : 0.0;
    const bool pos = i < n && s > 0;
    const bool prevpos = i > 0 && i < n && S[i - 1] > 0;
    const unsigned long long mpos = __ballot(pos);
    const unsigned long long mstart = __ballot(pos && !prevpos);
    const double sum = wave_sum(s), sabs = wave_sum(fabs(s));
    const int q = wave_max(quantum_exp(s));
    if (lane == 0) {
        flags[b] = (uint8_t)(mpos != 0ull ? 1 : 0);
        blk[b] = (uint64_t)__popcll(mstart);
        blk_sum[b] = sum;
        blk_abs[b] = sabs;
        blk_q[b] = q;
    }
}

__global__ void __launch_bounds__(256) mss_superstat_kernel(const double *__restrict__ blk_sum, const double *__restrict__ blk_abs,
                                                            const int32_t *__restrict__ blk_q, const uint8_t *__restrict__ flags,
                                                            int64_t nblk, double *__restrict__ sup_sum, double *__restrict__ sup_abs,
                                                            int32_t *__restrict__ sup_q, uint8_t *__restrict__ sup_flags)
{
    const int lane = threadIdx.x & 63;
    const int64_t g = (int64_t)blockIdx.x * 4 + (threadIdx.x >> 6);
    if (g * 64 >= nblk) return;
    const int64_t b = g * 64 + lane;
    const bool in = b < nblk;
    const unsigned long long mp = __ballot(in && (flags[b] & 1));
    const double sum = wave_sum(in ? blk_sum[b] : 0.0), sabs = wave_sum(in ? blk_abs[b] : 0.0);
    const int q = wave_max(in ? blk_q[b] : MSS_QNONE);
    if (lane == 0) {
        sup_flags[g] = (uint8_t)(mp != 0ull ? 1 : 0);
        sup_sum[g] = sum;
        sup_abs[g] = sabs;
        sup_q[g] = q;
    }
}

__device__ __forceinline__ bool mss_is_boundary(const uint8_t *flags, const double *blk_sum, int64_t b, int64_t nblk,
                                                int64_t n, double thr)
{
    if (!(thr > 0.0) || b + 1 >= nblk || (flags[b] & 1) || !(flags[b + 1] & 1)) return false;
    if (b * 64 + 64 > n) return false;
    double cum = 0.0;
    for (int64_t j = b; j >= 0 && j > b - 16; --j) {
        if (flags[j] & 1) break;
        cum += blk_sum[j];
        if (cum < -thr) return true;
    }
    return false;
}

__global__ void __launch_bounds__(256) mss_boundary_kernel(const uint8_t *__restrict__ flags, const double *__restrict__ blk_sum,
                                                           int64_t nblk, int64_t n, double thr, uint64_t *__restrict__ blk)
{
    const int64_t b = (int64_t)blockIdx.x * blockDim.x + threadIdx.x;
    if (b >= nblk) return;
    if (mss_is_boundary(flags, blk_sum, b, nblk, n, thr)) blk[b] |= 1ull << 32;
}

__global__ void __launch_bounds__(256) mss_units_kernel(const uint64_t *__restrict__ blk, const uint8_t *__restrict__ flags,
                                                        const double *__restrict__ blk_sum, int64_t nblk, int64_t n, double thr,
                                                        int64_t *__restrict__ ustart, int64_t *__restrict__ urun,
                                                        const uint64_t *__restrict__ grand)
{
    const int64_t b = (int64_t)blockIdx.x * blockDim.x + threadIdx.x;
    if (b == 0) {
        ustart[0] = 0;
// ... 889 lines not shown
            for (int c = 2; c < nof_labels; ++c)
                if (bv < hist[c]) { best = c; bv = hist[c]; }
        }
        for (int64_t c0 = st + (int64_t)blockIdx.x * MSS_VOTE_CHUNK; c0 < en; c0 += (int64_t)gridDim.x * MSS_VOTE_CHUNK) {
            const int64_t c1 = min(c0 + (int64_t)MSS_VOTE_CHUNK, en);
            if (PHASE == 0) {
                __shared__ int sh[DGRP_MAXC];
                if (threadIdx.x < DGRP_MAXC) sh[threadIdx.x] = 0;
                __syncthreads();
                for (int b0 = 0; b0 < nof_labels; b0 += 16) {
                    int cnt[16];
#pragma unroll
                    for (int c = 0; c < 16; ++c) cnt[c] = 0;
                    for (int64_t j = c0 + threadIdx.x; j < c1; j += 256) {
                        const int l = cls[j] - b0;
#pragma unroll
                        for (int c = 0; c < 16; ++c) cnt[c] += (l == c);
                    }
#pragma unroll
                    for (int c = 0; c < 16; ++c) {
                        int v = cnt[c];
                        for (int o = 32; o > 0; o >>= 1) v += __shfl_xor(v, o);
                        if ((threadIdx.x & 63) == 0 && v && b0 + c >= 1 && b0 + c < DGRP_MAXC) atomicAdd(&sh[b0 + c], v);
                    }
                }
                __syncthreads();
                if (threadIdx.x >= 1 && threadIdx.x < DGRP_MAXC && sh[threadIdx.x]) atomicAdd(&hist[threadIdx.x], sh[threadIdx.x]);
                __syncthreads();
            } else {
                for (int64_t j = c0 + threadIdx.x; j < c1; j += 256)
                    if (cls[j] == 0) out[j] = (int8_t)best;
            }
        }
    }
}

static int mss_vote_all(const mss_layout &l, const int8_t *d_cls, int nof_labels, int8_t *d_labels_out, int64_t n, hipStream_t stream)
{
    const int64_t longcap = n / MSS_VOTE_LONG + 1;
    unsigned long long *nlong = (unsigned long long *)l.grand;
    DGRP_HIP(hipMemsetAsync(nlong, 0, 8, stream));
    hipLaunchKernelGGL(mss_vote_kernel, dim3(1024), dim3(256), 0, stream, l.segs_out, l.grand + 3, d_cls, nof_labels, d_labels_out, nlong,
                       l.segs, longcap);
    DGRP_LAUNCH_CHECK();
    hipLaunchKernelGGL(mss_vote_long_kernel<0>, dim3(1024), dim3(256), 0, stream, l.segs_out, d_cls, nof_labels, d_labels_out, nlong, l.segs,
                       longcap);
    DGRP_LAUNCH_CHECK();
    hipLaunchKernelGGL(mss_vote_long_kernel<1>, dim3(1024), dim3(256), 0, stream, l.segs_out, d_cls, nof_labels, d_labels_out, nlong, l.segs,
                       longcap);
    DGRP_LAUNCH_CHECK();
    return DGRP_OK;
}

DGRP_EXPORT int dgrp_mss_labels(const double *d_scores, const int8_t *d_cls, int64_t n, int nof_labels,
                                int min_mss_len, int xdrop_len, int8_t *d_labels_out, int64_t *d_nseg,
                                void *d_work, int64_t work_bytes, void *stream_)
{
    hipStream_t stream = (hipStream_t)stream_;
    DGRP_REQUIRE(n >= 0 && n < (1ll << 31), "dgrp_mss_labels: n=%lld out of range (the reference indexes with int)", (long long)n);
    DGRP_REQUIRE(nof_labels >= 2 && nof_labels <= DGRP_MAXC, "dgrp_mss_labels: nof_labels must be in 2..64");
    if (n == 0) {
        if (d_nseg) DGRP_HIP(hipMemsetAsync(d_nseg, 0, sizeof(int64_t), stream));
        return DGRP_OK;
    }
    DGRP_REQUIRE(d_scores && d_cls && d_labels_out && d_work, "dgrp_mss_labels: NULL pointer");
    mss_layout l = mss_carve(d_work, n);
    if (work_bytes < l.bytes) {
        dgrp_set_error("dgrp_mss_labels: workspace %lld < %lld bytes", (long long)work_bytes, (long long)l.bytes);
        return DGRP_ENOMEM;
    }
    const double s0 = log(0.99 / (1.0 - 0.99));
    const double xdrop = xdrop_len > 0 ? s0 * xdrop_len * 10.0 : -1;
    const int min_sc = (int)(s0 * min_mss_len);
    const double thr = xdrop > 0.0 ? xdrop + 1.0 : -1.0;

    DGRP_HIP(hipMemsetAsync(l.blk, 0, (l.nblk + 1) * 8, stream));
    hipLaunchKernelGGL(mss_blockstat_kernel, dim3((unsigned)((l.nblk + 3) / 4)), dim3(256), 0, stream, d_scores, n, l.blk,
                       l.blk_sum, l.blk_abs, l.blk_q, l.flags);
    DGRP_LAUNCH_CHECK();
    hipLaunchKernelGGL(mss_superstat_kernel, dim3((unsigned)((l.nsup + 3) / 4)), dim3(256), 0, stream, l.blk_sum, l.blk_abs,
                       l.blk_q, l.flags, l.nblk, l.sup_sum, l.sup_abs, l.sup_q, l.sup_flags);
    DGRP_LAUNCH_CHECK();

    bool single = false;
    for (int attempt = 0; attempt < 2; ++attempt) {
        int64_t nunits = 1;
        DGRP_HIP(hipMemsetAsync(l.grand, 0, 64, stream));
        if (!single && xdrop > 0.0) {
            if (attempt == 0) {
                hipLaunchKernelGGL(mss_boundary_kernel, dim3((unsigned)((l.nblk + 255) / 256)), dim3(256), 0, stream,
                                   l.flags, l.blk_sum, l.nblk, n, thr, l.blk);
                DGRP_LAUNCH_CHECK();
                int rc = device_exclusive_scan(l.blk, l.blk, l.nblk, l.tiles, l.grand, stream);
                if (rc) return rc;
            }
            hipLaunchKernelGGL(mss_units_kernel, dim3((unsigned)((l.nblk + 255) / 256)), dim3(256), 0, stream, l.blk, l.flags,
                               l.blk_sum, l.nblk, n, thr, l.ustart, l.urun, l.grand);
            DGRP_LAUNCH_CHECK();
            uint64_t g = 0;
            DGRP_HIP(hipMemcpyAsync(&g, l.grand, 8, hipMemcpyDeviceToHost, stream));
            DGRP_HIP(hipStreamSynchronize(stream));
            nunits = (int64_t)(g >> 32) + 1;
        } else {
            int64_t h[2] = { 0, n };
            DGRP_HIP(hipMemcpyAsync(l.ustart, h, 16, hipMemcpyHostToDevice, stream));
            int64_t r[2] = { 0, 0 };
            DGRP_HIP(hipMemcpyAsync(l.urun, r, 16, hipMemcpyHostToDevice, stream));
            DGRP_HIP(hipStreamSynchronize(stream));
        }
        DGRP_REQUIRE(nunits < (1ll << 31), "dgrp_mss_labels: too many stretches");
        DGRP_HIP(hipMemsetAsync(l.exitL[0], 0, nunits * 8, stream));
        DGRP_HIP(hipMemsetAsync(l.exitL[1], 0, nunits * 8, stream));
        bool failed = false;
        bool done = false;
        if (!single && !getenv("DGRP_MSS_NO_CUTS")) {
            int64_t nl = 1;
            if (xdrop > 0.0) {
                const char *e = getenv("DGRP_MSS_SUB");
                const int sub = e && atoi(e) > 0 ? atoi(e) : MSS_LIGHT_SUB;
                hipLaunchKernelGGL(mss_lightflag_kernel, dim3((unsigned)((l.nblk + 255) / 256)), dim3(256), 0, stream, l.flags, l.blk_sum,
                                   l.nblk, n, thr, sub, 1, l.lblk);
                DGRP_LAUNCH_CHECK();
                int rc1 = device_exclusive_scan(l.lblk, l.lblk, l.nblk, l.tiles, l.grand + 6, stream);
                if (rc1) return rc1;
                hipLaunchKernelGGL(mss_lightunits_kernel, dim3((unsigned)((l.nblk + 255) / 256)), dim3(256), 0, stream, l.lblk, l.grand + 6,
                                   l.flags, l.blk_sum, l.blk, l.grand, l.nblk, n, thr, sub, 1, l.lstart, l.lrun, l.lforced);
                DGRP_LAUNCH_CHECK();
                uint64_t g6 = 0;
                DGRP_HIP(hipMemcpyAsync(&g6, l.grand + 6, 8, hipMemcpyDeviceToHost, stream));
                DGRP_HIP(hipStreamSynchronize(stream));
                nl = (int64_t)g6 + 1;
            } else {
// ... 104 lines not shown
                uint64_t g[3] = { 0, 0, 0 };
                DGRP_HIP(hipMemcpyAsync(g, l.grand, 24, hipMemcpyDeviceToHost, stream));
                DGRP_HIP(hipStreamSynchronize(stream));
                if (!g[1] && !g[2]) {
                    int rc3 = device_exclusive_scan(l.segcnt, l.segcnt, npieces, l.tiles, l.grand + 3, stream);
                    if (rc3) return rc3;
                    hipLaunchKernelGGL(mss_compact_kernel, dim3((unsigned)((npieces + 255) / 256)), dim3(256), 0, stream, l.segs, l.urun2,
                                       l.segcnt, l.grand + 3, npieces, l.segs_out, (const mss_subent *)nullptr);
                    DGRP_LAUNCH_CHECK();
                    done = true;
                }
                }
            }
            if (done) break;
            DGRP_HIP(hipMemsetAsync(l.exitL[0], 0, nunits * 8, stream));
            DGRP_HIP(hipMemsetAsync(l.exitL[1], 0, nunits * 8, stream));
            DGRP_HIP(hipMemsetAsync(l.grand + 1, 0, 16, stream));
        }
        for (int pass = 0;; ++pass) {
            DGRP_HIP(hipMemsetAsync(l.grand + 1, 0, 8, stream));
            hipLaunchKernelGGL(mss_scan_kernel, dim3((unsigned)nunits), dim3(64), 0, stream, d_scores, l.ustart, l.urun,
                               nunits, l.exitL[(pass + 1) & 1], l.exitL[pass & 1], l.stack, l.segs, l.segcnt, min_sc, xdrop,
                               l.grand, pass, l.blk_sum, l.blk_abs, l.blk_q, l.flags, l.sup_sum, l.sup_abs, l.sup_q,
                               l.sup_flags, 1, 0, 0, (mss_subent *)nullptr, (mss_cand *)nullptr);
            DGRP_LAUNCH_CHECK();
            uint64_t g[3] = { 0, 0, 0 };
            DGRP_HIP(hipMemcpyAsync(g, l.grand, 24, hipMemcpyDeviceToHost, stream));
            DGRP_HIP(hipStreamSynchronize(stream));
            if (g[2]) { failed = true; break; }
            if (nunits == 1 || (pass > 0 && g[1] == 0)) break;
            if (pass > nunits + 2) { failed = true; break; }
        }
        if (failed) {
            if (single) { dgrp_set_error("dgrp_mss_labels: sequential scan reported an inconsistent state"); return DGRP_EHIP; }
            single = true;
            continue;
        }
        int rc = device_exclusive_scan(l.segcnt, l.segcnt, nunits, l.tiles, l.grand + 3, stream);
        if (rc) return rc;
        hipLaunchKernelGGL(mss_compact_kernel, dim3((unsigned)((nunits + 255) / 256)), dim3(256), 0, stream, l.segs, l.urun,
                           l.segcnt, l.grand + 3, nunits, l.segs_out, (const mss_subent *)nullptr);
        DGRP_LAUNCH_CHECK();
        break;
    }
    DGRP_HIP(hipMemcpyAsync(d_labels_out, d_cls, n, hipMemcpyDeviceToDevice, stream));
    {
        const int rcv = mss_vote_all(l, d_cls, nof_labels, d_labels_out, n, stream);
        if (rcv) return rcv;
    }
    if (d_nseg) DGRP_HIP(hipMemcpyAsync(d_nseg, l.grand + 3, 8, hipMemcpyDeviceToDevice, stream));
    return DGRP_OK;
}

DGRP_EXPORT int dgrp_mss_segments_host(const void *d_work, int64_t work_bytes, int32_t *h_st_en, int64_t cap, int64_t *n_seg)
{
    DGRP_REQUIRE(d_work && n_seg, "dgrp_mss_segments_host: NULL pointer");
    int64_t lo = 0, hi = (1ll << 31) - 1;
    while (lo < hi) {
        int64_t mid = lo + (hi - lo + 1) / 2;
        if (mss_carve(nullptr, mid).bytes <= work_bytes) lo = mid; else hi = mid - 1;
    }
    mss_layout l = mss_carve((void *)d_work, lo);
    uint64_t cnt = 0;
    DGRP_HIP(hipDeviceSynchronize());
    DGRP_HIP(hipMemcpy(&cnt, l.grand + 3, 8, hipMemcpyDeviceToHost));
    *n_seg = (int64_t)cnt;
    const int64_t take = (int64_t)cnt < cap ? (int64_t)cnt : cap;
    if (take > 0 && h_st_en) DGRP_HIP(hipMemcpy(h_st_en, l.segs_out, take * 8, hipMemcpyDeviceToHost));
    return DGRP_OK;
}

DGRP_EXPORT int64_t dgrp_mss_batch_workspace_bytes(int64_t total_n, int64_t nrec)
{
    if (total_n < 0 || nrec < 0) return 0;
    return mss_carve(nullptr, total_n + 4 * nrec + 64).bytes;
}

DGRP_EXPORT int dgrp_mss_labels_batch(const double *d_scores, const int8_t *d_cls, int64_t total_n, int64_t nrec,
                                      const int64_t *h_start, int nof_labels, int min_mss_len, int xdrop_len,
                                      int8_t *d_labels_out, void *d_work, int64_t work_bytes, void *stream_)
{
    hipStream_t stream = (hipStream_t)stream_;
    DGRP_REQUIRE(total_n >= 0 && total_n < (1ll << 31) && nrec >= 0 && (nrec == 0 || h_start), "dgrp_mss_labels_batch: bad arguments");
    DGRP_REQUIRE(nof_labels >= 2 && nof_labels <= DGRP_MAXC, "dgrp_mss_labels_batch: nof_labels must be in 2..64");
    if (nrec == 0 || total_n == 0) return DGRP_OK;
    DGRP_REQUIRE(d_scores && d_cls && d_labels_out && d_work, "dgrp_mss_labels_batch: NULL pointer");
    DGRP_REQUIRE(h_start[0] == 0 && h_start[nrec] == total_n, "dgrp_mss_labels_batch: starts must run from 0 to total_n");
    for (int64_t r = 0; r < nrec; ++r)
        DGRP_REQUIRE((h_start[r] & 63) == 0 && h_start[r + 1] > h_start[r], "dgrp_mss_labels_batch: record %lld: starts must be increasing multiples of 64", (long long)r);
    mss_layout l = mss_carve(d_work, total_n + 4 * nrec + 64);
    if (work_bytes < l.bytes) {
        dgrp_set_error("dgrp_mss_labels_batch: workspace %lld < %lld bytes", (long long)work_bytes, (long long)l.bytes);
        return DGRP_ENOMEM;
    }
    l.nblk = (total_n + 63) / 64;
    l.nsup = (l.nblk + 63) / 64;
    const double s0 = log(0.99 / (1.0 - 0.99));
    const double xdrop = xdrop_len > 0 ? s0 * xdrop_len * 10.0 : -1;
    const int min_sc = (int)(s0 * min_mss_len);
    hipLaunchKernelGGL(mss_blockstat_kernel, dim3((unsigned)((l.nblk + 3) / 4)), dim3(256), 0, stream, d_scores, total_n, l.blk,
                       l.blk_sum, l.blk_abs, l.blk_q, l.flags);
    hipLaunchKernelGGL(mss_superstat_kernel, dim3((unsigned)((l.nsup + 3) / 4)), dim3(256), 0, stream, l.blk_sum, l.blk_abs,
                       l.blk_q, l.flags, l.nblk, l.sup_sum, l.sup_abs, l.sup_q, l.sup_flags);
    DGRP_LAUNCH_CHECK();
    std::vector<int64_t> urun((size_t)nrec + 1);
    for (int64_t r = 0; r <= nrec; ++r) urun[(size_t)r] = h_start[r] / 2 + 2 * r;
// ... 21 lines not shown
```

deepgrp_amd/csrc/post_kernels.hip:

```cpp
#include "dgrp_common.h"
#include "scan.h"
#include <vector>

#include <math.h>

__device__ __forceinline__ float np_logf(float xin)
{
    const uint32_t bits = __float_as_uint(xin);
    float k = (float)((int)(bits >> 23) - 126);
    float m = __uint_as_float((bits & 0x007fffffu) | 0x3f000000u);
    if (m <= 0.70710678118654752440f) { m = m + m; k = k - 1.0f; }
    const float x = m - 1.0f;
    float den = fmaf(5.875095403124574342950e-03f, x, 1.546476374983906719538e-01f);
    den = fmaf(den, x, 9.864942958519418960339e-01f);
    den = fmaf(den, x, 2.453006071784736363091e+00f);
    den = fmaf(den, x, 2.612677543073109236779e+00f);
    den = fmaf(den, x, 1.0f);
    float num = fmaf(2.589979117907922693523e-02f, x, 3.808837741388407920751e-01f);
    num = fmaf(num, x, 1.480000633576506585156e+00f);
    num = fmaf(num, x, 2.112677543073053063722e+00f);
    num = fmaf(num, x, 9.999999999999998702752e-01f);
    num = fmaf(num, x, 0.0f);
    return fmaf(k, 0.693147180559945309417232121458176568f, __fdiv_rn(num, den));
}

__device__ __forceinline__ float np_expf(float x)
{
    if (x != x) return x;
    if (x >= 88.72283905206835f) return INFINITY;
    if (x <= -103.97208404541015625f) return 0.0f;
    const float q = rintf(x * 1.44269504088896340736f);
    float r = fmaf(q, -6.93145752e-1f, x);
    r = fmaf(q, -1.42860677e-6f, r);
    float num = fmaf(5.082762527590693718096e-04f, r, 6.757896990527504603057e-03f);
    num = fmaf(num, r, 5.114512081637298353406e-02f);
    num = fmaf(num, r, 2.473615434895520810817e-01f);
    num = fmaf(num, r, 7.257664613233124478488e-01f);
    num = fmaf(num, r, 9.999999999980870924916e-01f);
    float den = fmaf(2.159509375685829852307e-02f, r, -2.742335390411667452936e-01f);
    den = fmaf(den, r, 1.0f);
    return ldexpf(__fdiv_rn(num, den), (int)q);
}

__global__ void __launch_bounds__(256) scores_kernel(const float *__restrict__ probs, int64_t n, int C,
                                                     double *__restrict__ scores, int8_t *__restrict__ cls)
{
    const int64_t nthreads = (int64_t)gridDim.x * blockDim.x;
    for (int64_t i = (int64_t)blockIdx.x * blockDim.x + threadIdx.x; i < n; i += nthreads) {
        const float *p = probs + i * C;
        int a = 0;
        float mx = p[0];
        for (int c = 1; c < C; ++c) {
            const float v = p[c];
            if (v > mx) { mx = v; a = c; }
        }
        float m = mx + 1e-6f;
        if (m > 0.99f) m = 0.99f;
        const float t = np_logf(__fdiv_rn(m, 1.0f - m));
        const float sc = a > 0 ? t : -10.0f * t;
        scores[i] = (double)sc;
        cls[i] = (int8_t)a;
    }
}

DGRP_EXPORT int dgrp_scores(const float *d_probs, int64_t n, int C, double *d_scores, int8_t *d_cls, void *stream)
{
    DGRP_REQUIRE(n >= 0 && C >= 1 && C <= DGRP_MAXC, "dgrp_scores: bad n/C");
    if (n == 0) return DGRP_OK;
    DGRP_REQUIRE(d_probs && d_scores && d_cls, "dgrp_scores: NULL pointer");
    hipLaunchKernelGGL(scores_kernel, dim3(grid_for(n, 256, 256 * 16)), dim3(256), 0, (hipStream_t)stream, d_probs, n,
                       C, d_scores, d_cls);
    DGRP_LAUNCH_CHECK();
    return DGRP_OK;
}

__global__ void __launch_bounds__(256) blockmax_kernel(const float *__restrict__ a, int64_t total, float *__restrict__ part)
{
    __shared__ float red[4];
    const int64_t nthreads = (int64_t)gridDim.x * blockDim.x;
    float m = -INFINITY;
    for (int64_t i = (int64_t)blockIdx.x * blockDim.x + threadIdx.x; i < total; i += nthreads) m = fmaxf(m, a[i]);
    for (int o = 32; o > 0; o >>= 1) m = fmaxf(m, __shfl_xor(m, o));
    if ((threadIdx.x & 63) == 0) red[threadIdx.x >> 6] = m;
    __syncthreads();
    if (threadIdx.x == 0) part[blockIdx.x] = fmaxf(fmaxf(red[0], red[1]), fmaxf(red[2], red[3]));
}

__global__ void __launch_bounds__(256) softmax_labels_kernel(const float *__restrict__ a, int64_t n, int C,
                                                             const float *__restrict__ part, int nparts,
                                                             float *__restrict__ sm, int8_t *__restrict__ labels)
{
    float gmax = -INFINITY;
    for (int i = 0; i < nparts; ++i) gmax = fmaxf(gmax, part[i]);
    const int64_t nthreads = (int64_t)gridDim.x * blockDim.x;
    for (int64_t i = (int64_t)blockIdx.x * blockDim.x + threadIdx.x; i < n; i += nthreads) {
        const float *row = a + i * C;
        float sum;
        if (C < 8) {
            sum = np_expf(row[0] - gmax);
            for (int c = 1; c < C; ++c) sum = sum + np_expf(row[c] - gmax);
        } else {
            float r[8];
#pragma unroll
            for (int k = 0; k < 8; ++k) r[k] = np_expf(row[k] - gmax);
            const int whole = C - C % 8;
            int c = 8;
            for (; c < whole; c += 8) {
#pragma unroll
                for (int k = 0; k < 8; ++k) r[k] = r[k] + np_expf(row[c + k] - gmax);
            }
            sum = ((r[0] + r[1]) + (r[2] + r[3])) + ((r[4] + r[5]) + (r[6] + r[7]));
            for (; c < C; ++c) sum = sum + np_expf(row[c] - gmax);
        }
        int best = 0;
        float bv = __fdiv_rn(np_expf(a[i * C] - gmax), sum);
        if (sm) sm[i * C] = bv;
        for (int c = 1; c < C; ++c) {
            const float v = __fdiv_rn(np_expf(a[i * C + c] - gmax), sum);
            if (sm) sm[i * C + c] = v;
            if (v > bv) { bv = v; best = c; }
        }
        labels[i] = (int8_t)best;
    }
}

DGRP_EXPORT int dgrp_softmax_labels(const float *d_probs, int64_t n, int C, float *d_softmax, int8_t *d_labels,
                                    void *d_work, int64_t work_bytes, void *stream)
{
    DGRP_REQUIRE(n >= 0 && C >= 1 && C <= DGRP_MAXC, "dgrp_softmax_labels: bad n/C");
    if (n == 0) return DGRP_OK;
    const int nparts = 1024;
    DGRP_REQUIRE(d_probs && d_labels && d_work && work_bytes >= (int64_t)(nparts * sizeof(float)),
                 "dgrp_softmax_labels: need %d bytes of workspace", (int)(nparts * sizeof(float)));
    float *part = (float *)d_work;
    hipLaunchKernelGGL(blockmax_kernel, dim3(nparts), dim3(256), 0, (hipStream_t)stream, d_probs, n * C, part);
    DGRP_LAUNCH_CHECK();
    hipLaunchKernelGGL(softmax_labels_kernel, dim3(grid_for(n, 256, 256 * 16)), dim3(256), 0, (hipStream_t)stream,
                       d_probs, n, C, part, nparts, d_softmax, d_labels);
    DGRP_LAUNCH_CHECK();
    return DGRP_OK;
}

__device__ __forceinline__ bool seg_is_start(const int8_t *lab, int64_t i, int64_t n)
{
    const int8_t v = lab[i];
    return v != 0 && (i == 0 || i == n - 1 || lab[i - 1] != v);
}
__device__ __forceinline__ bool seg_is_end(const int8_t *lab, int64_t i, int64_t n)
{
    const int8_t v = lab[i];
    return v != 0 && (i >= n - 2 || lab[i + 1] != v);
}

__device__ __forceinline__ uint64_t seg_flags_batch(const int8_t *lab, const uint8_t *marks, int64_t i)
{
    const uint8_t m = marks[i];
    const int8_t v = lab[i];
    if ((m & 8) || v == 0) return 0;
    const bool st = (m & 1) || (m & 2) || lab[i - 1] != v;
    const bool en = (m & 2) || (m & 4) || lab[i + 1] != v;
    return ((uint64_t)st << 32) + (uint64_t)en;
}

template <bool BATCH>
__device__ __forceinline__ uint64_t seg_flags(const int8_t *lab, const uint8_t *marks, int64_t i, int64_t n)
{
    if (BATCH) return seg_flags_batch(lab, marks, i);
    return ((uint64_t)seg_is_start(lab, i, n) << 32) + (uint64_t)seg_is_end(lab, i, n);
}

struct seg_records {
    const int64_t *start;
    const int64_t *startpos;
    const int32_t *contig;
    int64_t nrec;
};

template <bool BATCH>
__global__ void __launch_bounds__(256) seg_count_kernel(const int8_t *__restrict__ lab, const uint8_t *__restrict__ marks, int64_t n,
                                                        uint64_t *__restrict__ tilecnt)
{
    __shared__ uint64_t lds[4];
    const int64_t base = (int64_t)blockIdx.x * SCAN_TILE;
    uint64_t c = 0;
    for (int j = 0; j < 8; ++j) {
        const int64_t i = base + j * 256 + threadIdx.x;
        if (i < n) c += seg_flags<BATCH>(lab, marks, i, n);
    }
    for (int o = 32; o > 0; o >>= 1) c += __shfl_xor(c, o);
    if ((threadIdx.x & 63) == 0) lds[threadIdx.x >> 6] = c;
    __syncthreads();
    if (threadIdx.x == 0) tilecnt[blockIdx.x] = lds[0] + lds[1] + lds[2] + lds[3];
}

template <bool BATCH>
__global__ void __launch_bounds__(256) seg_emit_kernel(const int8_t *__restrict__ lab, const uint8_t *__restrict__ marks, int64_t n,
                                                       int64_t offset, int32_t contig, seg_records recs,
                                                       const uint64_t *__restrict__ tileoff, dgrp_segment *__restrict__ rec, int64_t cap)
{
    __shared__ uint64_t lds[4];
    const int64_t base = (int64_t)blockIdx.x * SCAN_TILE + (int64_t)threadIdx.x * 8;
    uint64_t f[8], s = 0;
    for (int j = 0; j < 8; ++j) {
        const int64_t i = base + j;
        f[j] = i < n ? seg_flags<BATCH>(lab, marks, i, n) : 0;
        s += f[j];
    }
    uint64_t ex = block_exclusive_scan(s, nullptr, lds) + tileoff[blockIdx.x];
    for (int j = 0; j < 8; ++j) {
        const int64_t i = base + j;
        if (f[j]) {
            int64_t off = offset;
            int32_t tag = contig;
            if (BATCH) {
                int64_t lo = 0, hi = recs.nrec;
                while (hi - lo > 1) {
                    const int64_t mid = (lo + hi) >> 1;
                    if (recs.start[mid] <= i) lo = mid; else hi = mid;
                }
                off = recs.startpos[lo] - recs.start[lo];
                tag = recs.contig[lo];
            }
            if (f[j] >> 32) {
                const int64_t k = (int64_t)(ex >> 32);
                if (k < cap) { rec[k].start = i + off; rec[k].label = lab[i]; rec[k].contig = tag; }
            }
            if (f[j] & 1) {
                const int64_t k = (int64_t)(ex & 0xffffffffull);
                if (k < cap) rec[k].end = i + 1 + off;
            }
        }
        ex += f[j];
    }
}

__global__ void seg_total_kernel(const uint64_t *__restrict__ grand, int64_t *__restrict__ count)
{
    *count = (int64_t)(*grand >> 32);
}

__global__ void __launch_bounds__(64) rec_marks_kernel(const int64_t *__restrict__ start, const int64_t *__restrict__ len,
                                                       int64_t nrec, uint8_t *__restrict__ marks, double *__restrict__ scores,
                                                       int8_t *__restrict__ cls)
{
    const int64_t r = blockIdx.x;
    if (r >= nrec) return;
    const int64_t a = start[r], n = len[r], b = start[r + 1];
    if (threadIdx.x == 0) {
        uint8_t m0 = 1;
        if (n == 1) m0 |= 2;
        if (n == 2) m0 |= 4;
        marks[a] = m0;
        if (n >= 2) marks[a + n - 1] = (uint8_t)(2 | (n == 1 ? 1 : 0));
        if (n >= 3) marks[a + n - 2] = 4;
    }
    for (int64_t i = a + n + threadIdx.x; i < b; i += 64) {
        marks[i] = 8;
        if (scores) scores[i] = 0.0;
        if (cls) cls[i] = 0;
    }
}

int dgrp_batch_marks(const int64_t *d_start, const int64_t *d_len, int64_t nrec, int64_t total_n, uint8_t *d_marks,
                     double *d_scores, int8_t *d_cls, hipStream_t stream)
{
    DGRP_HIP(hipMemsetAsync(d_marks, 0, (size_t)total_n, stream));
    hipLaunchKernelGGL(rec_marks_kernel, dim3((unsigned)nrec), dim3(64), 0, stream, d_start, d_len, nrec, d_marks, d_scores, d_cls);
    DGRP_LAUNCH_CHECK();
    return DGRP_OK;
}

int dgrp_batch_segments(const int8_t *d_labels, const uint8_t *d_marks, int64_t total_n, const int64_t *d_start, int64_t nrec,
                        const int64_t *d_startpos, const int32_t *d_contig, dgrp_segment *d_records, int64_t cap,
                        int64_t *d_count, void *d_work, int64_t work_bytes, hipStream_t stream)
{
    if (work_bytes < dgrp_segments_workspace_bytes(total_n)) {
        dgrp_set_error("dgrp_batch_segments: workspace too small");
        return DGRP_ENOMEM;
    }
    const int64_t ntiles = (total_n + SCAN_TILE - 1) / SCAN_TILE;
    uint64_t *tiles = (uint64_t *)d_work;
    uint64_t *grand = tiles + ntiles + 1;
    hipLaunchKernelGGL(seg_count_kernel<true>, dim3((unsigned)ntiles), dim3(256), 0, stream, d_labels, d_marks, total_n, tiles);
    hipLaunchKernelGGL(scan_sums_kernel, dim3(1), dim3(256), 0, stream, tiles, ntiles, grand);
    hipLaunchKernelGGL(seg_emit_kernel<true>, dim3((unsigned)ntiles), dim3(256), 0, stream, d_labels, d_marks, total_n, (int64_t)0,
                       (int32_t)0, seg_records{ d_start, d_startpos, d_contig, nrec }, tiles, d_records, cap);
    hipLaunchKernelGGL(seg_total_kernel, dim3(1), dim3(1), 0, stream, grand, d_count);
    DGRP_LAUNCH_CHECK();
    return DGRP_OK;
}

DGRP_EXPORT int64_t dgrp_segments_workspace_bytes(int64_t n)
{
    if (n < 0) return 0;
    return dgrp_align_up(((n + SCAN_TILE - 1) / SCAN_TILE + 2) * 8, 256) + 256;
}

DGRP_EXPORT int dgrp_segments(const int8_t *d_labels, int64_t n, int64_t offset, int32_t contig, dgrp_segment *d_records,
                              int64_t cap, int64_t *d_count, void *d_work, int64_t work_bytes, void *stream_)
{
    hipStream_t stream = (hipStream_t)stream_;
    DGRP_REQUIRE(n >= 0 && n < (1ll << 31) && cap >= 0 && d_count, "dgrp_segments: bad arguments");
    if (n == 0) {
        DGRP_HIP(hipMemsetAsync(d_count, 0, sizeof(int64_t), stream));
        return DGRP_OK;
    }
    DGRP_REQUIRE(d_labels && d_work && (cap == 0 || d_records), "dgrp_segments: NULL pointer");
    if (work_bytes < dgrp_segments_workspace_bytes(n)) {
        dgrp_set_error("dgrp_segments: workspace too small");
        return DGRP_ENOMEM;
    }
    const int64_t ntiles = (n + SCAN_TILE - 1) / SCAN_TILE;
    uint64_t *tiles = (uint64_t *)d_work;
    uint64_t *grand = tiles + ntiles + 1;
    hipLaunchKernelGGL(seg_count_kernel<false>, dim3((unsigned)ntiles), dim3(256), 0, stream, d_labels, (const uint8_t *)nullptr, n, tiles);
    DGRP_LAUNCH_CHECK();
    hipLaunchKernelGGL(scan_sums_kernel, dim3(1), dim3(256), 0, stream, tiles, ntiles, grand);
    DGRP_LAUNCH_CHECK();
    hipLaunchKernelGGL(seg_emit_kernel<false>, dim3((unsigned)ntiles), dim3(256), 0, stream, d_labels, (const uint8_t *)nullptr, n, offset,
                       contig, seg_records{ nullptr, nullptr, nullptr, 0 }, tiles, d_records, cap);
    DGRP_LAUNCH_CHECK();
    hipLaunchKernelGGL(seg_total_kernel, dim3(1), dim3(1), 0, stream, grand, d_count);
    DGRP_LAUNCH_CHECK();
    return DGRP_OK;
}
```

deepgrp_amd/csrc/scan.h:

```cpp
#pragma once
#include "dgrp_common.h"

namespace {

static inline int grid_for(int64_t work_items, int block, int max_blocks = 256 * 8)
{
    int64_t g = (work_items + block - 1) / block;
    if (g < 1) g = 1;
    if (g > max_blocks) g = max_blocks;
    return (int)g;
}

#define SCAN_TILE 2048

__device__ __forceinline__ uint64_t block_exclusive_scan(uint64_t v, uint64_t *total, uint64_t *lds)
{
    const int lane = threadIdx.x & 63, wave = threadIdx.x >> 6;
    uint64_t x = v;
#pragma unroll
    for (int o = 1; o < 64; o <<= 1) {
        uint64_t y = __shfl_up(x, o);
        if (lane >= o) x += y;
    }
    if (lane == 63) lds[wave] = x;
    __syncthreads();
    uint64_t base = 0;
    for (int w = 0; w < wave; ++w) base += lds[w];
    if (total) *total = lds[0] + lds[1] + lds[2] + lds[3];
    __syncthreads();
    return base + x - v;
}

__global__ void __launch_bounds__(256) scan_tilesum_kernel(const uint64_t *__restrict__ in, int64_t n, uint64_t *__restrict__ tilesum)
{
    __shared__ uint64_t lds[4];
    const int64_t base = (int64_t)blockIdx.x * SCAN_TILE;
    uint64_t s = 0;
    for (int j = 0; j < 8; ++j) {
        const int64_t i = base + j * 256 + threadIdx.x;
        if (i < n) s += in[i];
    }
    for (int o = 32; o > 0; o >>= 1) s += __shfl_xor(s, o);
    if ((threadIdx.x & 63) == 0) lds[threadIdx.x >> 6] = s;
    __syncthreads();
    if (threadIdx.x == 0) tilesum[blockIdx.x] = lds[0] + lds[1] + lds[2] + lds[3];
}

__global__ void __launch_bounds__(256) scan_sums_kernel(uint64_t *__restrict__ tilesum, int64_t ntiles, uint64_t *__restrict__ grand)
{
    __shared__ uint64_t lds[4];
    uint64_t carry = 0;
    for (int64_t base = 0; base < ntiles; base += 256) {
        const int64_t i = base + threadIdx.x;
        const uint64_t v = i < ntiles ? tilesum[i] : 0;
        uint64_t tot;
        const uint64_t ex = block_exclusive_scan(v, &tot, lds);
        if (i < ntiles) tilesum[i] = carry + ex;
        carry += tot;
    }
    if (threadIdx.x == 0 && grand) *grand = carry;
}

__global__ void __launch_bounds__(256) scan_apply_kernel(const uint64_t *__restrict__ in, int64_t n,
                                                         const uint64_t *__restrict__ tilesum, uint64_t *__restrict__ out)
{
    __shared__ uint64_t lds[4];
    const int64_t base = (int64_t)blockIdx.x * SCAN_TILE + (int64_t)threadIdx.x * 8;
    uint64_t v[8], s = 0;
    for (int j = 0; j < 8; ++j) { v[j] = base + j < n ? in[base + j] : 0; s += v[j]; }
    uint64_t ex = block_exclusive_scan(s, nullptr, lds) + tilesum[blockIdx.x];
    for (int j = 0; j < 8; ++j) {
        if (base + j < n) out[base + j] = ex;
        ex += v[j];
    }
}

static int device_exclusive_scan(const uint64_t *in, uint64_t *out, int64_t n, uint64_t *tiles, uint64_t *grand,
                                 hipStream_t stream)
{
    if (n <= 0) {
        if (grand) DGRP_HIP(hipMemsetAsync(grand, 0, sizeof(uint64_t), stream));
        return DGRP_OK;
    }
    const int64_t ntiles = (n + SCAN_TILE - 1) / SCAN_TILE;
    hipLaunchKernelGGL(scan_tilesum_kernel, dim3((unsigned)ntiles), dim3(256), 0, stream, in, n, tiles);
    DGRP_LAUNCH_CHECK();
    hipLaunchKernelGGL(scan_sums_kernel, dim3(1), dim3(256), 0, stream, tiles, ntiles, grand);
    DGRP_LAUNCH_CHECK();
    hipLaunchKernelGGL(scan_apply_kernel, dim3((unsigned)ntiles), dim3(256), 0, stream, in, n, tiles, out);
    DGRP_LAUNCH_CHECK();
    return DGRP_OK;
}

}
```

deepgrp_amd/csrc/track_kernels.hip:

```cpp
#include "dgrp_common.h"
#include "scan.h"
#include "tabix_bins.h"
#include "track_chain.h"
#include <string.h>
#include <vector>

namespace {

#define TRACK_WAVE_BIN 64

__device__ __forceinline__ uint32_t track_quantise(float v, float scale, uint32_t qmax)
{
    const float t = v * scale;
    const float q = floorf(t + 0.5f);
    return q <= 0.0f ? 0u : q >= (float)qmax ? qmax : (uint32_t)q;
}

__device__ __forceinline__ int track_decimal_width(uint64_t v)
{
    int w = 1;
    for (uint64_t p = 10; w < 19 && v >= p; p *= 10) ++w;
    return w;
}

// ... 256 lines not shown
    for (int64_t r = 0; r < nrec; ++r) {
        tb_rec &R = recs[r];
        R.row0 = h_row0[r]; R.n = h_n[r]; R.offset = h_startpos[r];
        R.kb0 = R.offset / bin;
        R.nb = (R.offset + R.n - 1) / bin - R.kb0 + 1;
        R.name_off = h_name_off[r]; R.name_len = h_name_off[r + 1] - h_name_off[r]; R.pad = 0;
        pref[r + 1] = pref[r] + R.nb;
    }
    memcpy(tab.data() + l.cls, h_cls, (size_t)ncls * 4);
    if (names_bytes > 0) memcpy(tab.data() + l.names, names, (size_t)names_bytes);
    char *w = (char *)d_work;
    DGRP_HIP(hipMemcpyAsync(w + l.tables, tab.data(), tab.size(), hipMemcpyHostToDevice, stream));
    uint64_t *grand = (uint64_t *)w, *bounds = (uint64_t *)(w + 256);
    const tb_rec *d_recs = (const tb_rec *)(w + l.tables + l.recs);
    const int64_t *d_pref = (const int64_t *)(w + l.tables + l.pref);
    const int *d_cls = (const int *)(w + l.tables + l.cls);
    uint32_t *q = (uint32_t *)(w + l.q);
    uint64_t *tiles = (uint64_t *)(w + l.tiles);
    tb_geom G;
    G.nrec = nrec; G.NB = pref[nrec]; G.NBpad = l.NBpad; G.bin = bin; G.C = C; G.ncls = ncls; G.digits = digits;
    uint32_t qmax = 1;
    for (int k = 0; k < digits; ++k) qmax *= 10;
    const float scale = (float)qmax;
    const int64_t tpc = l.NBpad / TRACK_TILE, ntiles = tpc * ncls;

    if (bin <= TRACK_WAVE_BIN) {
        hipLaunchKernelGGL(tb_bin_lane_kernel, dim3((unsigned)((G.NB + 255) / 256)), dim3(256), 0, stream, d_probs, d_recs, d_pref, d_cls, G,
                           scale, qmax, q);
    } else {
        hipLaunchKernelGGL(tb_bin_wave_kernel, dim3(grid_for(G.NB * 64, 256)), dim3(256), 0, stream, d_probs, d_recs, d_pref, d_cls, G,
                           scale, qmax, q);
    }
    DGRP_LAUNCH_CHECK();
    D->grand = grand; D->bounds = bounds; D->recs = d_recs; D->pref = d_pref; D->cls = d_cls; D->names = w + l.tables + l.names;
    D->q = q; D->tiles = tiles; D->G = G; D->qmax = qmax; D->tpc = tpc; D->ntiles = ntiles;
    return DGRP_OK;
}

static int tb_front(const float *d_probs, int C, int64_t nrec, const int64_t *h_row0, const int64_t *h_n, const int64_t *h_startpos,
                    const char *names, const int64_t *h_name_off, const int *h_cls, int ncls, int digits, int64_t bin,
                    int64_t *h_class_off, void *d_work, const tb_layout &l, hipStream_t stream, tb_dev *D)
{
    std::vector<char> tab;
    const int rc = tb_bins(d_probs, C, nrec, h_row0, h_n, h_startpos, names, h_name_off, h_cls, ncls, digits, bin, d_work, l, stream, tab, D);
    if (rc != DGRP_OK) return rc;
    const tb_rec *d_recs = D->recs;
    const int64_t *d_pref = D->pref;
    uint32_t *q = D->q;
    uint64_t *tiles = D->tiles, *grand = D->grand, *bounds = D->bounds;
    const tb_geom G = D->G;
    const int64_t tpc = D->tpc, ntiles = D->ntiles;
    hipLaunchKernelGGL(tb_count_kernel, dim3((unsigned)ntiles), dim3(256), 0, stream, q, d_recs, d_pref, G, tiles);
    DGRP_LAUNCH_CHECK();
    hipLaunchKernelGGL(scan_sums_kernel, dim3(1), dim3(256), 0, stream, tiles, ntiles, grand);
    DGRP_LAUNCH_CHECK();
    hipLaunchKernelGGL(tb_bounds_kernel, dim3(1), dim3(128), 0, stream, tiles, tpc, ncls, grand, bounds);
    DGRP_LAUNCH_CHECK();
    std::vector<uint64_t> off((size_t)ncls + 1, 0);
    DGRP_HIP(hipMemcpyAsync(off.data(), bounds, off.size() * 8, hipMemcpyDeviceToHost, stream));
    DGRP_HIP(hipStreamSynchronize(stream));
    for (int k = 0; k <= ncls; ++k) h_class_off[k] = (int64_t)off[(size_t)k];
    return DGRP_OK;
}

static int tb_run(const float *d_probs, int C, int64_t nrec, const int64_t *h_row0, const int64_t *h_n, const int64_t *h_startpos,
                  const char *names, const int64_t *h_name_off, const int *h_cls, int ncls, int digits, int64_t bin, char *d_text,
                  int64_t cap, int64_t *h_class_off, void *d_work, const tb_layout &l, hipStream_t stream)
{
    tb_dev D;
    const int rc = tb_front(d_probs, C, nrec, h_row0, h_n, h_startpos, names, h_name_off, h_cls, ncls, digits, bin, h_class_off, d_work, l,
                            stream, &D);
    if (rc != DGRP_OK) return rc;
    const int64_t total = h_class_off[ncls];
    if (total == 0 || total > cap) return DGRP_OK;
    hipLaunchKernelGGL(tb_write_kernel, dim3((unsigned)D.ntiles), dim3(256), 0, stream, D.q, D.recs, D.pref, D.names, D.G, D.qmax, D.tiles,
                       d_text);
    DGRP_LAUNCH_CHECK();
    DGRP_HIP(hipStreamSynchronize(stream));
    return DGRP_OK;
}

static bool track_carve_one(int64_t n, int64_t bin, tb_layout *l)
{
    if (n < 0 || n > TRACK_MAX_EXTENT || bin < 1 || bin > TRACK_MAX_EXTENT) return false;
    return tb_carve_bins(1, n / bin + 2, 1, DGRP_TRACK_NAME_ROOM, l);
}

struct ix_top2 { int64_t a, b; };
struct ix_state { ix_top2 F, L; };

__device__ __forceinline__ ix_top2 ix_join(ix_top2 l, ix_top2 r)
{
    if (r.a < 0) return l;
    ix_top2 o;
    o.a = r.a;
    o.b = r.b >= 0 ? r.b : l.a;
    return o;
}

__device__ __forceinline__ ix_state ix_join(const ix_state &l, const ix_state &r)
{
    ix_state o;
    o.F = ix_join(l.F, r.F);
    o.L = ix_join(l.L, r.L);
    return o;
}

// ... 296 lines not shown
        DGRP_REQUIRE(h_cls[k] >= 0 && h_cls[k] < C, "dgrp_track_index_batch: class %d is not in 0..%d", h_cls[k], C - 1);
    DGRP_REQUIRE(digits >= 1 && digits <= 4, "dgrp_track_index_batch: digits must lie in 1..4, got %d", digits);
    DGRP_REQUIRE(bin >= 1 && bin <= TRACK_MAX_EXTENT, "dgrp_track_index_batch: bad bin %lld", (long long)bin);
    DGRP_REQUIRE(chunk_cap >= 0 && linear_cap >= 0, "dgrp_track_index_batch: bad chunk_cap/linear_cap (%lld, %lld)", (long long)chunk_cap,
                 (long long)linear_cap);
    if (nrec == 0) return DGRP_OK;
    DGRP_REQUIRE(h_row0 && h_n && h_startpos && h_name_off, "dgrp_track_index_batch: NULL host table");
    DGRP_REQUIRE(h_name_off[0] >= 0, "dgrp_track_index_batch: record 0: bad name offset %lld", (long long)h_name_off[0]);
    std::vector<int64_t> wpref((size_t)nrec + 1, 0);
    for (int64_t r = 0; r < nrec; ++r) {
        DGRP_REQUIRE(h_n[r] >= 1 && h_n[r] <= TRACK_MAX_EXTENT, "dgrp_track_index_batch: record %lld: bad n %lld", (long long)r,
                     (long long)h_n[r]);
        DGRP_REQUIRE(h_startpos[r] >= 0 && h_startpos[r] <= TRACK_MAX_EXTENT, "dgrp_track_index_batch: record %lld: bad offset %lld",
                     (long long)r, (long long)h_startpos[r]);
        DGRP_REQUIRE(h_startpos[r] + h_n[r] <= TABIX_MAX_END,
                     "dgrp_track_index_batch: record %lld ends at %lld, above 2^29 = 536870912, the largest coordinate of a tabix index",
                     (long long)r, (long long)(h_startpos[r] + h_n[r]));
        DGRP_REQUIRE(h_row0[r] >= 0, "dgrp_track_index_batch: record %lld: bad first row %lld", (long long)r, (long long)h_row0[r]);
        DGRP_REQUIRE(h_name_off[r + 1] >= h_name_off[r], "dgrp_track_index_batch: record %lld: descending name offsets (%lld, %lld)",
                     (long long)r, (long long)h_name_off[r], (long long)h_name_off[r + 1]);
        wpref[(size_t)r + 1] = wpref[(size_t)r] + ((h_startpos[r] + h_n[r] - 1) >> TABIX_MIN_SHIFT) + 1;
    }
    const int64_t names_bytes = h_name_off[nrec], W = wpref[(size_t)nrec];
    DGRP_REQUIRE(linear_cap >= W * ncls, "dgrp_track_index_batch: linear_cap %lld < %lld windows of %d classes", (long long)linear_cap,
                 (long long)(W * ncls), ncls);
    DGRP_REQUIRE((names || names_bytes == 0) && (d_chunks || chunk_cap == 0) && d_linear && d_probs && d_work,
                 "dgrp_track_index_batch: NULL pointer");
    ix_layout l;
    DGRP_REQUIRE(ix_carve(nrec, h_n, h_startpos, bin, ncls, names_bytes, &l), "dgrp_track_index_batch: too many bins in one call");
    if (work_bytes < l.bytes) {
        dgrp_set_error("dgrp_track_index_batch: workspace %lld < %lld bytes", (long long)work_bytes, (long long)l.bytes);
        return DGRP_ENOMEM;
    }
    hipStream_t stream = (hipStream_t)stream_;
    char *w = (char *)d_work;
    int64_t *d_wpref = (int64_t *)(w + l.wpref);
    ix_state *state = (ix_state *)(w + l.state);
    uint64_t *tilechunks = (uint64_t *)(w + l.tilechunks), *cgrand = (uint64_t *)(w + l.cgrand), *cbounds = (uint64_t *)(w + l.cbounds);
    DGRP_HIP(hipMemcpyAsync(d_wpref, wpref.data(), wpref.size() * 8, hipMemcpyHostToDevice, stream));
    tb_dev D;
    std::vector<int64_t> text_off((size_t)ncls + 1, 0);
    const int rc = tb_front(d_probs, C, nrec, h_row0, h_n, h_startpos, names, h_name_off, h_cls, ncls, digits, bin, text_off.data(), d_work,
                            l.t, stream, &D);
    if (rc != DGRP_OK) return rc;
    const dim3 grid((unsigned)D.ntiles), block(256);
    hipLaunchKernelGGL(ix_tile_kernel<0>, grid, block, 0, stream, D.q, D.recs, D.pref, d_wpref, D.G, W, D.tiles, D.bounds, state, tilechunks,
                       cbounds, d_chunks, d_linear);
    DGRP_LAUNCH_CHECK();
    hipLaunchKernelGGL(ix_carry_kernel, dim3((unsigned)ncls), block, 0, stream, state, D.tpc);
    DGRP_LAUNCH_CHECK();
    hipLaunchKernelGGL(ix_tile_kernel<1>, grid, block, 0, stream, D.q, D.recs, D.pref, d_wpref, D.G, W, D.tiles, D.bounds, state, tilechunks,
                       cbounds, d_chunks, d_linear);
    DGRP_LAUNCH_CHECK();
    hipLaunchKernelGGL(scan_sums_kernel, dim3(1), block, 0, stream, tilechunks, D.ntiles, cgrand);
    DGRP_LAUNCH_CHECK();
    hipLaunchKernelGGL(tb_bounds_kernel, dim3(1), dim3(128), 0, stream, tilechunks, D.tpc, ncls, cgrand, cbounds);
    DGRP_LAUNCH_CHECK();
    std::vector<uint64_t> off((size_t)ncls + 1, 0);
    DGRP_HIP(hipMemcpyAsync(off.data(), cbounds, off.size() * 8, hipMemcpyDeviceToHost, stream));
    DGRP_HIP(hipStreamSynchronize(stream));
    for (int k = 0; k <= ncls; ++k) h_chunk_off[k] = (int64_t)off[(size_t)k];
    if (h_chunk_off[ncls] > chunk_cap) return DGRP_OK;
    DGRP_HIP(hipMemsetAsync(d_linear, 0xff, (size_t)(W * ncls) * 8, stream));
    hipLaunchKernelGGL(ix_tile_kernel<2>, grid, block, 0, stream, D.q, D.recs, D.pref, d_wpref, D.G, W, D.tiles, D.bounds, state, tilechunks,
                       cbounds, d_chunks, d_linear);
    DGRP_LAUNCH_CHECK();
    hipLaunchKernelGGL(ix_ends_kernel, dim3(1), dim3(128), 0, stream, cbounds, D.bounds, ncls, d_chunks);
    DGRP_LAUNCH_CHECK();
    DGRP_HIP(hipStreamSynchronize(stream));
    return DGRP_OK;
}
```

deepgrp_amd/pipeline.py:

```python
from __future__ import annotations

import ctypes as C
from typing import NamedTuple, Optional, Tuple

import numpy as np
import torch

from ._lib import check, lib, name_blob
from .fasta import DeviceRecord

SEGMENT_DTYPE = np.dtype([("start", "<i8"), ("end", "<i8"), ("label", "<i4"), ("contig", "<i4")])
ROW_SCORE_DTYPE = np.dtype([("sum", "<u8"), ("bases", "<i8"), ("agree", "<i8"), ("qmin", "<u4"), ("pad", "<u4")])


def require_gpu() -> torch.device:
    if not torch.cuda.is_available():
        raise RuntimeError("deepgrp_amd needs an AMD MI355X (gfx950) visible to PyTorch-ROCm; "
                           "there is no CPU fallback")
    return torch.device("cuda", torch.cuda.current_device())


def stream_ptr() -> int:
    return torch.cuda.current_stream().cuda_stream

# ... 280 lines not shown
        out = torch.zeros((n, m.classes), dtype=torch.float32, device=d_idx.device)
        nwin = L.dgrp_window_count(n, m.vecsize, self.step)
        if self.fp32:
            B = self.batch
            fit = (4 << 30) // (2 * m.vecsize * m.units * 4 + m.vecsize * (m.classes + 1) * 4)
            per = max(B, min(self.chunk_windows, fit) // B * B)
            w0 = i = 0
            while w0 < nwin:
                nw = min(per, nwin - w0)
                probs = m.forward_windows_reference(d_idx, self.step, w0, nw)
                for off in range(0, nw, B):
                    b = min(B, nw - off)
                    index = i * b * self.step
                    if index < n:
                        check(L.dgrp_get_max(_ptr(out[index:]), n - index, _ptr(probs[off:off + b]), m.vecsize, m.classes,
                                             self.step, b, stream_ptr()), "dgrp_get_max")
                    i += 1
                w0 += nw
            return out
        if self.event_log is None and self.chunk_windows >= (1 << 20):
            wb = L.dgrp_forward_merge_record_workspace_bytes(self.handle, n, self.step)
            work = torch.empty(max(wb, 256), dtype=torch.uint8, device=d_idx.device)
            check(L.dgrp_forward_merge_record(self.handle, _ptr(d_idx), n, self.step, self.batch, _ptr(out), _ptr(work), work.numel(),
                                              stream_ptr()), "dgrp_forward_merge_record")
            return out
        chunk = max(16, min(self.chunk_windows, L.dgrp_forward_window_chunk(self.handle)))
        work = None
        w0 = 0
        while w0 < nwin:
            nw = min(chunk, nwin - w0)
            wb = L.dgrp_forward_workspace_bytes(self.handle, nw)
            if work is None or work.numel() < wb:
                work = torch.empty(max(wb, 256), dtype=torch.uint8, device=d_idx.device)
            if self.event_log is not None:
                ev0, ev1 = torch.cuda.Event(enable_timing=True), torch.cuda.Event(enable_timing=True)
                ev0.record()
            check(L.dgrp_forward_merge(self.handle, _ptr(d_idx), n, self.step, self.batch, w0, nw, _ptr(out),
                                       _ptr(work), work.numel(), stream_ptr()), "dgrp_forward_merge")
            if self.event_log is not None:
                ev1.record()
                self.event_log.append((ev0, ev1, nw))
            w0 += nw
        return out

    def labels(self, merged: torch.Tensor) -> torch.Tensor:
        L = lib()
        n, c = merged.shape
        dev = merged.device
        if n == 0:
            return torch.empty(0, dtype=torch.int8, device=dev)
        if self.use_mss:
            scores = torch.empty(n, dtype=torch.float64, device=dev)
            cls = torch.empty(n, dtype=torch.int8, device=dev)
            check(L.dgrp_scores(_ptr(merged), n, c, _ptr(scores), _ptr(cls), stream_ptr()), "dgrp_scores")
            return self.labels_from_scores(scores, cls)
        labels = torch.empty(n, dtype=torch.int8, device=dev)
        work = torch.empty(4096, dtype=torch.uint8, device=dev)
        check(L.dgrp_softmax_labels(_ptr(merged), n, c, None, _ptr(labels), _ptr(work), work.numel(),
                                    stream_ptr()), "dgrp_softmax_labels")
        return labels

    def labels_from_scores(self, scores: torch.Tensor, cls: torch.Tensor) -> torch.Tensor:
        L = lib()
        n, dev = scores.numel(), scores.device
        labels = torch.empty(n, dtype=torch.int8, device=dev)
        if n == 0:
            return labels
        wb = L.dgrp_mss_workspace_bytes(n)
        work = torch.empty(wb, dtype=torch.uint8, device=dev)
        check(L.dgrp_mss_labels(_ptr(scores), _ptr(cls), n, self.model.classes, self.min_mss_len, self.xdrop_len, _ptr(labels),
                                None, _ptr(work), wb, stream_ptr()), "dgrp_mss_labels")
        return labels

    def segments(self, labels: torch.Tensor, offset: int, contig: int = 0, cap: Optional[int] = None) -> np.ndarray:
        L = lib()
        n = labels.numel()
        dev = labels.device
        if n == 0:
            return np.zeros(0, SEGMENT_DTYPE)
        wb = L.dgrp_segments_workspace_bytes(n)
        work = torch.empty(wb, dtype=torch.uint8, device=dev)
        count = torch.zeros(1, dtype=torch.int64, device=dev)

        def launch(rec, cap):
            check(L.dgrp_segments(_ptr(labels), n, offset, contig, _ptr(rec), cap, _ptr(count), _ptr(work), wb,
                                  stream_ptr()), "dgrp_segments")
            return int(count.item())
        return _segment_rows(dev, cap if cap is not None else max(1024, n // 64), launch)

    def track_text(self, merged: torch.Tensor, startpos: int, name, cls: int, digits: int = 2, bin: int = 1) -> bytes:
        return self.track_text_device(merged, startpos, name, cls, digits, bin).cpu().numpy().tobytes()

    def track_text_device(self, merged: torch.Tensor, startpos: int, name, cls: int, digits: int = 2, bin: int = 1) -> torch.Tensor:
        if merged.ndim == 2 and merged.shape[0] == 0:
            return torch.empty(0, dtype=torch.uint8, device=merged.device)
        return self.track_text_batch_device(merged, [0], [len(merged)], [startpos], [name], [cls], digits, bin)[0]

    def run_idx(self, d_idx: torch.Tensor, startpos: int, contig: int = 0) -> np.ndarray:
        if self.event_log is not None or self.fp32:
            return self.segments(self.labels(self.merged(d_idx)), startpos, contig)
        L = lib()
        n = d_idx.numel()
        if n == 0:
            return np.zeros(0, SEGMENT_DTYPE)
        dev = d_idx.device
        wb = L.dgrp_record_workspace_bytes(self.handle, n, self.step, int(self.use_mss))
        work = torch.empty(wb, dtype=torch.uint8, device=dev)
        count = C.c_int64(0)
# ... 486 lines not shown
```

include/deepgrp_hip.h:

```cpp
#ifndef DEEPGRP_HIP_H_
#define DEEPGRP_HIP_H_

#include <stddef.h>
#include <stdint.h>

#ifdef __cplusplus
extern "C" {
#endif

#define DGRP_OK 0
#define DGRP_EINVAL (-1)
#define DGRP_EHIP (-2)
#define DGRP_ENOMEM (-3)
#define DGRP_ENODEV (-4)

#define DGRP_ABI_VERSION 1

typedef struct dgrp_segment {
    int64_t start;
    int64_t end;
    int32_t label;
    int32_t contig;
} dgrp_segment;

// ... 59 lines not shown
int dgrp_model_create(dgrp_model **out, int T, int u, int C, int attention, const float *h_kernel,
                      const float *h_recurrent, const float *h_bias, const float *h_scale,
                      const float *h_ff_kernel, const float *h_ff_bias);
int dgrp_model_create_lstm(dgrp_model **out, int T, int u, int C, const float *h_kernel,
                           const float *h_recurrent, const float *h_bias, const float *h_ff_kernel,
                           const float *h_ff_bias);
int dgrp_model_destroy(dgrp_model *m);
int dgrp_model_dims(const dgrp_model *m, int *T, int *u, int *C, int *attention);
int dgrp_model_flags(const dgrp_model *m);
int dgrp_model_set_precision(dgrp_model *m, int level);
int dgrp_model_view(const dgrp_model *m, int level, dgrp_model **out);

#define DGRP_KERNEL_NONE 0
#define DGRP_KERNEL_WAVE 1
#define DGRP_KERNEL_SPLIT2 2
#define DGRP_KERNEL_STREAM64 3
#define DGRP_KERNEL_STREAM 4
#define DGRP_KERNEL_SPLIT 5
#define DGRP_KERNEL_LSTM 6
#define DGRP_KERNEL_FUSED 7
#define DGRP_KERNEL_FP32 8
int dgrp_model_plan(const dgrp_model *m, int mode, int64_t step, int *kernel, int64_t *lds_bytes, int *ospan, int *avg_up);

int64_t dgrp_forward_workspace_bytes(const dgrp_model *m, int64_t nw);
int64_t dgrp_forward_window_chunk(const dgrp_model *m);
int dgrp_forward_windows(const dgrp_model *m, const uint8_t *d_idx, int64_t n, int64_t s,
                         int64_t w0, int64_t nw, float *d_probs, void *d_work, int64_t work_bytes,
                         void *stream);

int dgrp_forward_merge(const dgrp_model *m, const uint8_t *d_idx, int64_t n, int64_t s,
                       int64_t batch, int64_t w0, int64_t nw, float *d_out, void *d_work,
                       int64_t work_bytes, void *stream);

int64_t dgrp_forward_merge_record_workspace_bytes(const dgrp_model *m, int64_t n, int64_t s);
int dgrp_forward_merge_record(const dgrp_model *m, const uint8_t *d_idx, int64_t n, int64_t s, int64_t batch, float *d_out,
                              void *d_work, int64_t work_bytes, void *stream);

int64_t dgrp_forward_reference_workspace_bytes(const dgrp_model *m, int64_t nw);
int dgrp_forward_windows_reference(const dgrp_model *m, const uint8_t *d_idx, int64_t n, int64_t s, int64_t w0,
                                   int64_t nw, float *d_probs, void *d_work, int64_t work_bytes, void *stream);

int dgrp_get_max(float *d_output, int64_t out_rows, const float *d_inputs, int64_t dim0,
                 int64_t dim1, int64_t stride, int64_t batchsize, void *stream);

int dgrp_scores(const float *d_probs, int64_t n, int C, double *d_scores, int8_t *d_cls,
                void *stream);
int dgrp_softmax_labels(const float *d_probs, int64_t n, int C, float *d_softmax, int8_t *d_labels,
                        void *d_work, int64_t work_bytes, void *stream);

int64_t dgrp_mss_workspace_bytes(int64_t n);
int dgrp_mss_labels(const double *d_scores, const int8_t *d_cls, int64_t n, int nof_labels,
                    int min_mss_len, int xdrop_len, int8_t *d_labels_out, int64_t *d_nseg,
                    void *d_work, int64_t work_bytes, void *stream);
int dgrp_mss_segments_host(const void *d_work, int64_t work_bytes, int32_t *h_st_en, int64_t cap,
                           int64_t *n_seg);

int64_t dgrp_mss_batch_workspace_bytes(int64_t total_n, int64_t nrec);
int dgrp_mss_labels_batch(const double *d_scores, const int8_t *d_cls, int64_t total_n, int64_t nrec,
                          const int64_t *h_start, int nof_labels, int min_mss_len, int xdrop_len,
                          int8_t *d_labels_out, void *d_work, int64_t work_bytes, void *stream);

int64_t dgrp_segments_workspace_bytes(int64_t n);
int dgrp_segments(const int8_t *d_labels, int64_t n, int64_t offset, int32_t contig,
                  dgrp_segment *d_records, int64_t cap, int64_t *d_count, void *d_work,
                  int64_t work_bytes, void *stream);

int64_t dgrp_format_rows_bound(int64_t nrows, int64_t longest_prefix);
int dgrp_format_rows(const char *prefixes, const int64_t *prefix_off, int64_t nprefix, int by_contig,
                     const dgrp_segment *rows, int64_t nrows, char *out, int64_t cap, int64_t *written);

#define DGRP_TRACK_NAME_ROOM 65536
int64_t dgrp_track_workspace_bytes(int64_t n, int64_t bin);
int dgrp_track_text(const float *d_probs, int64_t n, int C, int cls, int digits, int64_t bin, int64_t offset,
                    const char *name, int64_t name_len, char *d_text, int64_t cap, int64_t *h_bytes,
                    void *d_work, int64_t work_bytes, void *stream);

int64_t dgrp_track_batch_workspace_bytes(int64_t nrec, const int64_t *h_n, const int64_t *h_startpos, int64_t bin, int ncls,
                                         int64_t names_bytes);
int dgrp_track_text_batch(const float *d_probs, int C, int64_t nrec, const int64_t *h_row0, const int64_t *h_n,
                          const int64_t *h_startpos, const char *names, const int64_t *h_name_off, const int *h_cls, int ncls,
                          int digits, int64_t bin, char *d_text, int64_t cap, int64_t *h_class_off, void *d_work,
                          int64_t work_bytes, void *stream);

typedef struct { int64_t beg, end; int32_t rec; uint32_t bin; } dgrp_track_chunk;
int64_t dgrp_track_index_workspace_bytes(int64_t nrec, const int64_t *h_n, const int64_t *h_startpos, int64_t bin, int ncls,
                                         int64_t names_bytes);
int dgrp_track_index_batch(const float *d_probs, int C, int64_t nrec, const int64_t *h_row0, const int64_t *h_n,
                           const int64_t *h_startpos, const char *names, const int64_t *h_name_off, const int *h_cls, int ncls,
                           int digits, int64_t bin, dgrp_track_chunk *d_chunks, int64_t chunk_cap, int64_t *h_chunk_off,
                           int64_t *d_linear, int64_t linear_cap, void *d_work, int64_t work_bytes, void *stream);

typedef struct { int64_t off, bytes; int32_t rec; uint32_t start, end, pad; } dgrp_track_section;
int64_t dgrp_track_sections_workspace_bytes(int64_t nrec, const int64_t *h_n, const int64_t *h_startpos, int64_t bin, int ncls);
int dgrp_track_sections_batch(const float *d_probs, int C, int64_t nrec, const int64_t *h_row0, const int64_t *h_n,
                              const int64_t *h_startpos, const int *h_cls, int ncls, int digits, int64_t bin, int64_t chrom0, char *d_out,
                              int64_t cap, int64_t *h_class_off, dgrp_track_section *d_table, int64_t table_cap, int64_t *h_section_off,
                              void *d_work, int64_t work_bytes, void *stream);

#define DGRP_TRACK_ZOOM_LEVELS 10
typedef struct { int64_t off, bytes; int32_t cls, level, rec0, rec1; uint32_t start, end; } dgrp_track_zoom_block;
typedef struct { uint64_t covered, qmin, qmax, sum, sumsq; } dgrp_track_totals;
int64_t dgrp_track_zoom_workspace_bytes(int64_t nrec, const int64_t *h_n, const int64_t *h_startpos, int64_t bin, int ncls);
int dgrp_track_zoom_batch(const float *d_probs, int C, int64_t nrec, const int64_t *h_row0, const int64_t *h_n,
                          const int64_t *h_startpos, const int *h_cls, int ncls, int digits, int64_t bin, int64_t chrom0, char *d_out,
                          int64_t cap, int64_t *h_record_off, dgrp_track_zoom_block *d_table, int64_t table_cap, int64_t *h_block_off,
                          dgrp_track_totals *h_totals, void *d_work, int64_t work_bytes, void *stream);
// ... 179 lines not shown
```

Before: 565.1.

## Fuse score computation into MSS block statistics kernel and widen scan-sums kernel

Adds a kernel that computes per-position scores and classes from the probabilities and emits the MSS per-block statistics in one pass. Rows are staged through LDS with prefetch of the next block, which removes the separate scores kernel and the re-read of the double scores array. The single-block scan_sums kernel is also widened to 1024 threads with 8 items per thread, so each loop iteration covers more tiles. The fused path duplicates the score transform on device, so its results must match the old dgrp_scores exactly.

```diff
diff --git a/deepgrp_amd/_lib.py b/deepgrp_amd/_lib.py
--- a/deepgrp_amd/_lib.py
+++ b/deepgrp_amd/_lib.py
@@ -87,6 +87,9 @@
     "dgrp_softmax_labels": (cint, [vp, i64, cint, vp, vp, vp, i64, vp]),
     "dgrp_mss_workspace_bytes": (i64, [i64]),
     "dgrp_mss_labels": (cint, [vp, vp, i64, cint, cint, cint, vp, vp, vp, i64, vp]),
+    "dgrp_mss_blockstats": (cint, [vp, i64, vp, vp, vp, vp, vp, vp]),
+    "dgrp_scores_blockstats": (cint, [vp, i64, cint, vp, vp, vp, vp, vp, vp, vp, vp]),
+    "dgrp_scores_mss_labels": (cint, [vp, i64, cint, cint, cint, vp, vp, vp, vp, vp, i64, vp]),
     "dgrp_mss_segments_host": (cint, [vp, i64, vp, i64, C.POINTER(i64)]),
     "dgrp_mss_batch_workspace_bytes": (i64, [i64, i64]),
     "dgrp_mss_labels_batch": (cint, [vp, vp, i64, i64, vp, cint, cint, cint, vp, vp, i64, vp]),
diff --git a/deepgrp_amd/csrc/api.hip b/deepgrp_amd/csrc/api.hip
--- a/deepgrp_amd/csrc/api.hip
+++ b/deepgrp_amd/csrc/api.hip
@@ -871,10 +871,8 @@
     int rc = dgrp_forward_merge_record(m, d_idx, n, s, batch, out, w + l.fwd, l.fwd_bytes, stream);
     if (rc) return rc;
     if (use_mss) {
-        rc = dgrp_scores(out, n, m->C, (double *)(w + l.scores), (int8_t *)(w + l.cls), stream);
-        if (rc) return rc;
-        rc = dgrp_mss_labels((const double *)(w + l.scores), (const int8_t *)(w + l.cls), n, m->C, min_mss_len, xdrop_len,
-                             labels, nullptr, w + l.post, l.post_bytes, stream);
+        rc = dgrp_scores_mss_labels(out, n, m->C, min_mss_len, xdrop_len, (double *)(w + l.scores), (int8_t *)(w + l.cls), labels, nullptr,
+                                    w + l.post, l.post_bytes, stream);
     } else {
         rc = dgrp_softmax_labels(out, n, m->C, nullptr, labels, w + l.post, l.post_bytes, stream);
     }
diff --git a/deepgrp_amd/csrc/bigbed_kernels.hip b/deepgrp_amd/csrc/bigbed_kernels.hip
--- a/deepgrp_amd/csrc/bigbed_kernels.hip
+++ b/deepgrp_amd/csrc/bigbed_kernels.hip
@@ -406,7 +406,7 @@
     const int64_t ntiles = Z.seg[BBI_LEVELS] / 256;
     hipLaunchKernelGGL(bbi_count_kernel<bbz_win>, dim3((unsigned)ntiles), block, 0, stream, (const bbz_win *)win, wtiles);
     DGRP_LAUNCH_CHECK();
-    hipLaunchKernelGGL(scan_sums_kernel, dim3(1), block, 0, stream, wtiles, ntiles, grand);
+    hipLaunchKernelGGL(scan_sums_kernel, dim3(1), dim3(SCAN_SUMS_THREADS), 0, stream, wtiles, ntiles, grand);
     DGRP_LAUNCH_CHECK();
     hipLaunchKernelGGL((bbi_bounds_kernel<bbz_win, true>), dim3(1), block, 0, stream, (const bbz_win *)win, (const uint64_t *)wtiles,
                        (const uint64_t *)grand, Z, 1, segb, grand + 1);
diff --git a/deepgrp_amd/csrc/bigwig_kernels.hip b/deepgrp_amd/csrc/bigwig_kernels.hip
--- a/deepgrp_amd/csrc/bigwig_kernels.hip
+++ b/deepgrp_amd/csrc/bigwig_kernels.hip
@@ -472,7 +472,7 @@
     const dim3 grid((unsigned)D.ntiles), block(256);
     hipLaunchKernelGGL(bw_count_kernel, grid, block, 0, stream, D.q, D.recs, D.pref, D.G, D.tiles, cnt);
     DGRP_LAUNCH_CHECK();
-    hipLaunchKernelGGL(scan_sums_kernel, dim3(1), block, 0, stream, D.tiles, D.ntiles, D.grand);
+    hipLaunchKernelGGL(scan_sums_kernel, dim3(1), dim3(SCAN_SUMS_THREADS), 0, stream, D.tiles, D.ntiles, D.grand);
     DGRP_LAUNCH_CHECK();
     hipLaunchKernelGGL(bw_prefix_kernel, dim3((unsigned)ncls), block, 0, stream, cnt, nrec, ipref, spref);
     DGRP_LAUNCH_CHECK();
@@ -554,7 +554,7 @@
     const int64_t ntiles = Z.seg[BBI_LEVELS] / 256 * ncls;
     hipLaunchKernelGGL(bbi_count_kernel<bwz_win>, dim3((unsigned)ntiles), block, 0, stream, win, tiles);
     DGRP_LAUNCH_CHECK();
-    hipLaunchKernelGGL(scan_sums_kernel, dim3(1), block, 0, stream, tiles, ntiles, grand);
+    hipLaunchKernelGGL(scan_sums_kernel, dim3(1), dim3(SCAN_SUMS_THREADS), 0, stream, tiles, ntiles, grand);
     DGRP_LAUNCH_CHECK();
     hipLaunchKernelGGL((bbi_bounds_kernel<bwz_win, false>), dim3(1), dim3(64), 0, stream, win, tiles, grand, Z, ncls, segb, nullptr);
     DGRP_LAUNCH_CHECK();
@@ -614,7 +614,7 @@
     if (rc != DGRP_OK) return rc;
     hipLaunchKernelGGL(zlib_sizes_kernel, dim3((unsigned)((nblk + 255) / 256)), dim3(256), 0, stream, rows, stride, nblk, in_bytes, sizes, bad);
     DGRP_LAUNCH_CHECK();
-    hipLaunchKernelGGL(scan_sums_kernel, dim3(1), dim3(256), 0, stream, sizes, nblk, sizes + nblk);
+    hipLaunchKernelGGL(scan_sums_kernel, dim3(1), dim3(SCAN_SUMS_THREADS), 0, stream, sizes, nblk, sizes + nblk);
     DGRP_LAUNCH_CHECK();
     hipLaunchKernelGGL(zlib_place_kernel, dim3((unsigned)nblk), dim3(256), 0, stream, d_in, rows, stride, slots, sizes, nblk, bad, d_out, out_cap,
                        d_sizes);
diff --git a/deepgrp_amd/csrc/deflate_kernels.hip b/deepgrp_amd/csrc/deflate_kernels.hip
--- a/deepgrp_amd/csrc/deflate_kernels.hip
+++ b/deepgrp_amd/csrc/deflate_kernels.hip
@@ -560,7 +560,7 @@
     uint32_t *lz = level == 0 ? nullptr : (uint32_t *)((uint8_t *)sizes + dgrp_align_up((nmem + 1) * 8, 256));
     const int rc = dgrp_deflate_members(d_in, n, nullptr, 0, nmem, level, slots, sizes, lz, stream);
     if (rc != DGRP_OK) return rc;
-    hipLaunchKernelGGL(scan_sums_kernel, dim3(1), dim3(256), 0, stream, sizes, nmem, sizes + nmem);
+    hipLaunchKernelGGL(scan_sums_kernel, dim3(1), dim3(SCAN_SUMS_THREADS), 0, stream, sizes, nmem, sizes + nmem);
     DGRP_LAUNCH_CHECK();
     hipLaunchKernelGGL(bgzf_place_kernel, dim3((unsigned)(nmem + (eof ? 1 : 0))), dim3(256), 0, stream, slots, sizes, nmem, eof, d_out, out_cap);
     DGRP_LAUNCH_CHECK();
diff --git a/deepgrp_amd/csrc/extract_kernels.hip b/deepgrp_amd/csrc/extract_kernels.hip
--- a/deepgrp_amd/csrc/extract_kernels.hip
+++ b/deepgrp_amd/csrc/extract_kernels.hip
@@ -365,7 +365,7 @@
                            wordpre);
         DGRP_LAUNCH_CHECK();
     }
-    hipLaunchKernelGGL(scan_sums_kernel, dim3(1), dim3(256), 0, stream, ex, ntiles, ex + ntiles);
+    hipLaunchKernelGGL(scan_sums_kernel, dim3(1), dim3(SCAN_SUMS_THREADS), 0, stream, ex, ntiles, ex + ntiles);
     DGRP_LAUNCH_CHECK();
     hipLaunchKernelGGL(extract_size_kernel, dim3((unsigned)((nrows + 1 + 255) / 256)), dim3(256), 0, stream, T, g, rowpos, kidx);
     DGRP_LAUNCH_CHECK();
diff --git a/deepgrp_amd/csrc/fasta_kernels.hip b/deepgrp_amd/csrc/fasta_kernels.hip
--- a/deepgrp_amd/csrc/fasta_kernels.hip
+++ b/deepgrp_amd/csrc/fasta_kernels.hip
@@ -110,7 +110,7 @@
     DGRP_HIP(hipMemcpyAsync(g, init, sizeof(init), hipMemcpyHostToDevice, stream));
     hipLaunchKernelGGL(fasta_count_kernel, dim3((unsigned)ntiles), dim3(256), 0, stream, d_raw, nbytes, tiles, g);
     DGRP_LAUNCH_CHECK();
-    hipLaunchKernelGGL(scan_sums_kernel, dim3(1), dim3(256), 0, stream, tiles, ntiles, grand);
+    hipLaunchKernelGGL(scan_sums_kernel, dim3(1), dim3(SCAN_SUMS_THREADS), 0, stream, tiles, ntiles, grand);
     DGRP_LAUNCH_CHECK();
     hipLaunchKernelGGL(fasta_scatter_kernel, dim3((unsigned)ntiles), dim3(256), 0, stream, d_raw, nbytes, tiles, d_idx, g);
     DGRP_LAUNCH_CHECK();
@@ -248,7 +248,7 @@
         unsigned long long *g = gbase + r * 32;
         const uint8_t *raw = d_raw + h_off[r];
         hipLaunchKernelGGL(fasta_count_kernel, dim3((unsigned)ntiles), dim3(256), 0, stream, raw, nbytes, tiles, g);
-        hipLaunchKernelGGL(scan_sums_kernel, dim3(1), dim3(256), 0, stream, tiles, ntiles, grand);
+        hipLaunchKernelGGL(scan_sums_kernel, dim3(1), dim3(SCAN_SUMS_THREADS), 0, stream, tiles, ntiles, grand);
         hipLaunchKernelGGL(fasta_scatter_kernel, dim3((unsigned)ntiles), dim3(256), 0, stream, raw, nbytes, tiles,
                            d_idx + h_off[r], g);
     }
diff --git a/deepgrp_amd/csrc/mask_kernels.hip b/deepgrp_amd/csrc/mask_kernels.hip
--- a/deepgrp_amd/csrc/mask_kernels.hip
+++ b/deepgrp_amd/csrc/mask_kernels.hip
@@ -174,7 +174,7 @@
     DGRP_HIP(hipMemcpyAsync(d_tab, tab.data(), tab.size() * 8, hipMemcpyHostToDevice, stream));
     hipLaunchKernelGGL(mask_count_kernel, dim3((unsigned)ntiles), dim3(256), 0, stream, d_raw, d_tile0, d_off, d_len, nrec, ex);
     DGRP_LAUNCH_CHECK();
-    hipLaunchKernelGGL(scan_sums_kernel, dim3(1), dim3(256), 0, stream, ex, ntiles, ex + ntiles);
+    hipLaunchKernelGGL(scan_sums_kernel, dim3(1), dim3(SCAN_SUMS_THREADS), 0, stream, ex, ntiles, ex + ntiles);
     DGRP_LAUNCH_CHECK();
     if (nrows > 0) {
         hipLaunchKernelGGL(mask_check_kernel, dim3((unsigned)((nrows + 255) / 256)), dim3(256), 0, stream, d_rows, d_row_off, nrec,
diff --git a/deepgrp_amd/csrc/mss_kernels.hip b/deepgrp_amd/csrc/mss_kernels.hip
--- a/deepgrp_amd/csrc/mss_kernels.hip
+++ b/deepgrp_amd/csrc/mss_kernels.hip
@@ -1,5 +1,6 @@
 #include "dgrp_common.h"
 #include "scan.h"
+#include "score_transform.h"
 #include <vector>
 #include <math.h>
 
@@ -177,6 +178,142 @@
         blk_abs[b] = sabs;
         blk_q[b] = q;
     }
+}
+
+#define SBS_BLOCKS 8
+#define SBS_STAGE_MAXC 32
+
+__device__ __forceinline__ void wave_lds_sync()
+{
+    __builtin_amdgcn_fence(__ATOMIC_RELEASE, "wavefront");
+    __builtin_amdgcn_wave_barrier();
+    __builtin_amdgcn_fence(__ATOMIC_ACQUIRE, "wavefront");
+}
+
+typedef float sbs_f4 __attribute__((ext_vector_type(4)));
+template <int TRIPS>
+struct sbs_span { sbs_f4 v[TRIPS]; };
+
+template <int TRIPS>
+__device__ __forceinline__ void sbs_fetch(const sbs_f4 *__restrict__ src, int nq, int lane, sbs_span<TRIPS> &r)
+{
+#pragma unroll
+    for (int t = 0; t < TRIPS; ++t)
+        if (lane + 64 * t < nq) r.v[t] = src[lane + 64 * t];
+}
+
+template <int CT>
+__global__ void __launch_bounds__(256) scores_blockstat_kernel(const float *__restrict__ probs, int64_t n, int Crt, int staged,
+                                                               double *__restrict__ scores, int8_t *__restrict__ cls,
+                                                               uint64_t *__restrict__ blk, double *__restrict__ blk_sum,
+                                                               double *__restrict__ blk_abs, int32_t *__restrict__ blk_q,
+                                                               uint8_t *__restrict__ flags)
+{
+    extern __shared__ sbs_f4 sbs_stage[];
+    constexpr int TRIPS = CT ? (CT + 3) / 4 : SBS_STAGE_MAXC / 4;
+    const int C = CT ? CT : Crt;
+    const int lane = threadIdx.x & 63, wave = threadIdx.x >> 6;
+    const int64_t nblk = (n + 63) / 64;
+    const int64_t bfirst = ((int64_t)blockIdx.x * 4 + wave) * SBS_BLOCKS;
+    sbs_f4 *mine = sbs_stage + wave * 16 * C;
+    sbs_span<TRIPS> cur, nxt;
+    auto fetch = [&](int64_t b, sbs_span<TRIPS> &r) {
+        if (staged && b < nblk && b * 64 + 64 <= n) sbs_fetch<TRIPS>((const sbs_f4 *)(probs + b * 64 * C), 16 * C, lane, r);
+    };
+    fetch(bfirst, cur);
+    unsigned long long front = 0;
+    for (int k = 0; k < SBS_BLOCKS; ++k) {
+        const int64_t b = bfirst + k;
+        if (b >= nblk) break;
+        if (k + 1 < SBS_BLOCKS) fetch(b + 1, nxt);
+        const int64_t i = b * 64 + lane;
+        float mx = 0.0f;
+        int a = 0;
+        if (staged && b * 64 + 64 <= n) {
+#pragma unroll
+            for (int t = 0; t < TRIPS; ++t)
+                if (lane + 64 * t < 16 * C) mine[lane + 64 * t] = cur.v[t];
+            wave_lds_sync();
+            mx = row_first_max((const float *)mine + lane * C, C, a);
+            wave_lds_sync();
+        } else if (i < n) {
+            mx = row_first_max(probs + i * C, C, a);
+        }
+        if (k == 0 && b > 0) {
+            int f = 0;
+            if (lane == 0) {
+                int pa;
+                const float pm = row_first_max(probs + (i - 1) * C, C, pa);
+                f = score_of_max(pm, pa) > 0.0f ? 1 : 0;
+            }
+            front = (unsigned long long)__builtin_amdgcn_readfirstlane(f);
+        }
+        const double s = i < n ? (double)score_of_max(mx, a) : 0.0;
+        if (i < n) {
+            scores[i] = s;
+            cls[i] = (int8_t)a;
+        }
+        const bool pos = i < n && s > 0;
+        const unsigned long long mpos = __ballot(pos);
+        const unsigned long long mstart = mpos & ~((mpos << 1) | front);
+        const double sum = wave_sum(s), sabs = wave_sum(fabs(s));
+        const int q = wave_max(quantum_exp(s));
+        if (lane == 0) {
+            flags[b] = (uint8_t)(mpos != 0ull ? 1 : 0);
+            blk[b] = (uint64_t)__popcll(mstart);
+            blk_sum[b] = sum;
+            blk_abs[b] = sabs;
+            blk_q[b] = q;
+        }
+        front = mpos >> 63;
+        cur = nxt;
+    }
+}
+
+static int launch_blockstat(const double *d_scores, int64_t n, uint64_t *blk, double *blk_sum, double *blk_abs, int32_t *blk_q,
+                            uint8_t *flags, hipStream_t stream)
+{
+    const int64_t nblk = (n + 63) / 64;
+    hipLaunchKernelGGL(mss_blockstat_kernel, dim3((unsigned)((nblk + 3) / 4)), dim3(256), 0, stream, d_scores, n, blk, blk_sum, blk_abs,
+                       blk_q, flags);
+    DGRP_LAUNCH_CHECK();
+    return DGRP_OK;
+}
+
+static int launch_scores_blockstat(const float *d_probs, int64_t n, int C, double *d_scores, int8_t *d_cls, uint64_t *blk,
+                                   double *blk_sum, double *blk_abs, int32_t *blk_q, uint8_t *flags, hipStream_t stream)
+{
+    const int64_t nblk = (n + 63) / 64;
+    const int staged = C <= SBS_STAGE_MAXC && ((uintptr_t)d_probs & 15) == 0 ? 1 : 0;
+    const dim3 grid((unsigned)((nblk + 4 * SBS_BLOCKS - 1) / (4 * SBS_BLOCKS)));
+    const size_t lds = staged ? (size_t)4 * 256 * C : 0;
+    if (C == 5)
+        hipLaunchKernelGGL(scores_blockstat_kernel<5>, grid, dim3(256), lds, stream, d_probs, n, C, staged, d_scores, d_cls, blk, blk_sum,
+                           blk_abs, blk_q, flags);
+    else
+        hipLaunchKernelGGL(scores_blockstat_kernel<0>, grid, dim3(256), lds, stream, d_probs, n, C, staged, d_scores, d_cls, blk, blk_sum,
+                           blk_abs, blk_q, flags);
+    DGRP_LAUNCH_CHECK();
+    return DGRP_OK;
+}
+
+DGRP_EXPORT int dgrp_mss_blockstats(const double *d_scores, int64_t n, uint64_t *d_blk, double *d_blk_sum, double *d_blk_abs,
+                                    int32_t *d_blk_q, uint8_t *d_flags, void *stream)
+{
+    DGRP_REQUIRE(n >= 0 && n < (1ll << 31), "dgrp_mss_blockstats: bad n");
+    if (n == 0) return DGRP_OK;
+    DGRP_REQUIRE(d_scores && d_blk && d_blk_sum && d_blk_abs && d_blk_q && d_flags, "dgrp_mss_blockstats: NULL pointer");
+    return launch_blockstat(d_scores, n, d_blk, d_blk_sum, d_blk_abs, d_blk_q, d_flags, (hipStream_t)stream);
+}
+
+DGRP_EXPORT int dgrp_scores_blockstats(const float *d_probs, int64_t n, int C, double *d_scores, int8_t *d_cls, uint64_t *d_blk,
+                                       double *d_blk_sum, double *d_blk_abs, int32_t *d_blk_q, uint8_t *d_flags, void *stream)
+{
+    DGRP_REQUIRE(n >= 0 && n < (1ll << 31) && C >= 1 && C <= DGRP_MAXC, "dgrp_scores_blockstats: bad n/C");
+    if (n == 0) return DGRP_OK;
+    DGRP_REQUIRE(d_probs && d_scores && d_cls && d_blk && d_blk_sum && d_blk_abs && d_blk_q && d_flags,
+                 "dgrp_scores_blockstats: NULL pointer");
+    return launch_scores_blockstat(d_probs, n, C, d_scores, d_cls, d_blk, d_blk_sum, d_blk_abs, d_blk_q, d_flags, (hipStream_t)stream);
 }
 
 __global__ void __launch_bounds__(256) mss_superstat_kernel(const double *__restrict__ blk_sum, const double *__restrict__ blk_abs,
@@ -1172,32 +1309,14 @@
     return DGRP_OK;
 }
 
-DGRP_EXPORT int dgrp_mss_labels(const double *d_scores, const int8_t *d_cls, int64_t n, int nof_labels,
-                                int min_mss_len, int xdrop_len, int8_t *d_labels_out, int64_t *d_nseg,
-                                void *d_work, int64_t work_bytes, void *stream_)
-{
-    hipStream_t stream = (hipStream_t)stream_;
-    DGRP_REQUIRE(n >= 0 && n < (1ll << 31), "dgrp_mss_labels: n=%lld out of range (the reference indexes with int)", (long long)n);
-    DGRP_REQUIRE(nof_labels >= 2 && nof_labels <= DGRP_MAXC, "dgrp_mss_labels: nof_labels must be in 2..64");
-    if (n == 0) {
-        if (d_nseg) DGRP_HIP(hipMemsetAsync(d_nseg, 0, sizeof(int64_t), stream));
-        return DGRP_OK;
-    }
-    DGRP_REQUIRE(d_scores && d_cls && d_labels_out && d_work, "dgrp_mss_labels: NULL pointer");
-    mss_layout l = mss_carve(d_work, n);
-    if (work_bytes < l.bytes) {
-        dgrp_set_error("dgrp_mss_labels: workspace %lld < %lld bytes", (long long)work_bytes, (long long)l.bytes);
-        return DGRP_ENOMEM;
-    }
+static int mss_labels_from_stats(const mss_layout &l, const double *d_scores, const int8_t *d_cls, int64_t n, int nof_labels,
+                                 int min_mss_len, int xdrop_len, int8_t *d_labels_out, int64_t *d_nseg, hipStream_t stream)
+{
     const double s0 = log(0.99 / (1.0 - 0.99));
     const double xdrop = xdrop_len > 0 ? s0 * xdrop_len * 10.0 : -1;
     const int min_sc = (int)(s0 * min_mss_len);
     const double thr = xdrop > 0.0 ? xdrop + 1.0 : -1.0;
 
-    DGRP_HIP(hipMemsetAsync(l.blk, 0, (l.nblk + 1) * 8, stream));
-    hipLaunchKernelGGL(mss_blockstat_kernel, dim3((unsigned)((l.nblk + 3) / 4)), dim3(256), 0, stream, d_scores, n, l.blk,
-                       l.blk_sum, l.blk_abs, l.blk_q, l.flags);
-    DGRP_LAUNCH_CHECK();
     hipLaunchKernelGGL(mss_superstat_kernel, dim3((unsigned)((l.nsup + 3) / 4)), dim3(256), 0, stream, l.blk_sum, l.blk_abs,
                        l.blk_q, l.flags, l.nblk, l.sup_sum, l.sup_abs, l.sup_q, l.sup_flags);
     DGRP_LAUNCH_CHECK();
@@ -1408,6 +1527,52 @@
     return DGRP_OK;
 }
 
+DGRP_EXPORT int dgrp_mss_labels(const double *d_scores, const int8_t *d_cls, int64_t n, int nof_labels,
+                                int min_mss_len, int xdrop_len, int8_t *d_labels_out, int64_t *d_nseg,
+                                void *d_work, int64_t work_bytes, void *stream_)
+{
+    hipStream_t stream = (hipStream_t)stream_;
+    DGRP_REQUIRE(n >= 0 && n < (1ll << 31), "dgrp_mss_labels: n=%lld out of range (the reference indexes with int)", (long long)n);
+    DGRP_REQUIRE(nof_labels >= 2 && nof_labels <= DGRP_MAXC, "dgrp_mss_labels: nof_labels must be in 2..64");
+    if (n == 0) {
+        if (d_nseg) DGRP_HIP(hipMemsetAsync(d_nseg, 0, sizeof(int64_t), stream));
+        return DGRP_OK;
+    }
+    DGRP_REQUIRE(d_scores && d_cls && d_labels_out && d_work, "dgrp_mss_labels: NULL pointer");
+    mss_layout l = mss_carve(d_work, n);
+    if (work_bytes < l.bytes) {
+        dgrp_set_error("dgrp_mss_labels: workspace %lld < %lld bytes", (long long)work_bytes, (long long)l.bytes);
+        return DGRP_ENOMEM;
+    }
+    DGRP_HIP(hipMemsetAsync(l.blk, 0, (l.nblk + 1) * 8, stream));
+    const int rc = launch_blockstat(d_scores, n, l.blk, l.blk_sum, l.blk_abs, l.blk_q, l.flags, stream);
+    if (rc) return rc;
+    return mss_labels_from_stats(l, d_scores, d_cls, n, nof_labels, min_mss_len, xdrop_len, d_labels_out, d_nseg, stream);
+}
+
+DGRP_EXPORT int dgrp_scores_mss_labels(const float *d_probs, int64_t n, int C, int min_mss_len, int xdrop_len, double *d_scores,
+                                       int8_t *d_cls, int8_t *d_labels_out, int64_t *d_nseg, void *d_work, int64_t work_bytes,
+                                       void *stream_)
+{
+    hipStream_t stream = (hipStream_t)stream_;
+    DGRP_REQUIRE(n >= 0 && n < (1ll << 31), "dgrp_scores_mss_labels: n=%lld out of range (the reference indexes with int)", (long long)n);
+    DGRP_REQUIRE(C >= 2 && C <= DGRP_MAXC, "dgrp_scores_mss_labels: C must be in 2..64");
+    if (n == 0) {
+        if (d_nseg) DGRP_HIP(hipMemsetAsync(d_nseg, 0, sizeof(int64_t), stream));
+        return DGRP_OK;
+    }
+    DGRP_REQUIRE(d_probs && d_scores && d_cls && d_labels_out && d_work, "dgrp_scores_mss_labels: NULL pointer");
+    mss_layout l = mss_carve(d_work, n);
+    if (work_bytes < l.bytes) {
+        dgrp_set_error("dgrp_scores_mss_labels: workspace %lld < %lld bytes", (long long)work_bytes, (long long)l.bytes);
+        return DGRP_ENOMEM;
+    }
+    DGRP_HIP(hipMemsetAsync(l.blk + l.nblk, 0, 8, stream));
+    const int rc = launch_scores_blockstat(d_probs, n, C, d_scores, d_cls, l.blk, l.blk_sum, l.blk_abs, l.blk_q, l.flags, stream);
+    if (rc) return rc;
+    return mss_labels_from_stats(l, d_scores, d_cls, n, C, min_mss_len, xdrop_len, d_labels_out, d_nseg, stream);
+}
+
 DGRP_EXPORT int dgrp_mss_segments_host(const void *d_work, int64_t work_bytes, int32_t *h_st_en, int64_t cap, int64_t *n_seg)
 {
     DGRP_REQUIRE(d_work && n_seg, "dgrp_mss_segments_host: NULL pointer");
diff --git a/deepgrp_amd/csrc/post_kernels.hip b/deepgrp_amd/csrc/post_kernels.hip
--- a/deepgrp_amd/csrc/post_kernels.hip
+++ b/deepgrp_amd/csrc/post_kernels.hip
@@ -1,28 +1,9 @@
 #include "dgrp_common.h"
 #include "scan.h"
+#include "score_transform.h"
 #include <vector>
 
 #include <math.h>
-
-__device__ __forceinline__ float np_logf(float xin)
-{
-    const uint32_t bits = __float_as_uint(xin);
-    float k = (float)((int)(bits >> 23) - 126);
-    float m = __uint_as_float((bits & 0x007fffffu) | 0x3f000000u);
-    if (m <= 0.70710678118654752440f) { m = m + m; k = k - 1.0f; }
-    const float x = m - 1.0f;
-    float den = fmaf(5.875095403124574342950e-03f, x, 1.546476374983906719538e-01f);
-    den = fmaf(den, x, 9.864942958519418960339e-01f);
-    den = fmaf(den, x, 2.453006071784736363091e+00f);
-    den = fmaf(den, x, 2.612677543073109236779e+00f);
-    den = fmaf(den, x, 1.0f);
-    float num = fmaf(2.589979117907922693523e-02f, x, 3.808837741388407920751e-01f);
-    num = fmaf(num, x, 1.480000633576506585156e+00f);
-    num = fmaf(num, x, 2.112677543073053063722e+00f);
-    num = fmaf(num, x, 9.999999999999998702752e-01f);
-    num = fmaf(num, x, 0.0f);
-    return fmaf(k, 0.693147180559945309417232121458176568f, __fdiv_rn(num, den));
-}
 
 __device__ __forceinline__ float np_expf(float x)
 {
@@ -47,17 +28,9 @@
 {
     const int64_t nthreads = (int64_t)gridDim.x * blockDim.x;
     for (int64_t i = (int64_t)blockIdx.x * blockDim.x + threadIdx.x; i < n; i += nthreads) {
-        const float *p = probs + i * C;
-        int a = 0;
-        float mx = p[0];
-        for (int c = 1; c < C; ++c) {
-            const float v = p[c];
-            if (v > mx) { mx = v; a = c; }
-        }
-        float m = mx + 1e-6f;
-        if (m > 0.99f) m = 0.99f;
-        const float t = np_logf(__fdiv_rn(m, 1.0f - m));
-        const float sc = a > 0 ? t : -10.0f * t;
+        int a;
+        const float mx = row_first_max(probs + i * C, C, a);
+        const float sc = score_of_max(mx, a);
         scores[i] = (double)sc;
         cls[i] = (int8_t)a;
     }
@@ -141,32 +114,28 @@
     return DGRP_OK;
 }
 
-__device__ __forceinline__ bool seg_is_start(const int8_t *lab, int64_t i, int64_t n)
-{
-    const int8_t v = lab[i];
-    return v != 0 && (i == 0 || i == n - 1 || lab[i - 1] != v);
-}
-__device__ __forceinline__ bool seg_is_end(const int8_t *lab, int64_t i, int64_t n)
-{
-    const int8_t v = lab[i];
-    return v != 0 && (i >= n - 2 || lab[i + 1] != v);
-}
-
-__device__ __forceinline__ uint64_t seg_flags_batch(const int8_t *lab, const uint8_t *marks, int64_t i)
-{
-    const uint8_t m = marks[i];
-    const int8_t v = lab[i];
+__device__ __forceinline__ bool seg_is_start(int8_t v, int8_t prev, int64_t i, int64_t n)
+{
+    return v != 0 && (i == 0 || i == n - 1 || prev != v);
+}
+__device__ __forceinline__ bool seg_is_end(int8_t v, int8_t next, int64_t i, int64_t n)
+{
+    return v != 0 && (i >= n - 2 || next != v);
+}
+
+__device__ __forceinline__ uint64_t seg_flags_batch(int8_t v, int8_t prev, int8_t next, uint8_t m)
+{
     if ((m & 8) || v == 0) return 0;
-    const bool st = (m & 1) || (m & 2) || lab[i - 1] != v;
-    const bool en = (m & 2) || (m & 4) || lab[i + 1] != v;
+    const bool st = (m & 1) || (m & 2) || prev != v;
+    const bool en = (m & 2) || (m & 4) || next != v;
     return ((uint64_t)st << 32) + (uint64_t)en;
 }
 
 template <bool BATCH>
-__device__ __forceinline__ uint64_t seg_flags(const int8_t *lab, const uint8_t *marks, int64_t i, int64_t n)
-{
-    if (BATCH) return seg_flags_batch(lab, marks, i);
-    return ((uint64_t)seg_is_start(lab, i, n) << 32) + (uint64_t)seg_is_end(lab, i, n);
+__device__ __forceinline__ uint64_t seg_flags(int8_t v, int8_t prev, int8_t next, uint8_t m, int64_t i, int64_t n)
+{
+    if (BATCH) return seg_flags_batch(v, prev, next, m);
+    return ((uint64_t)seg_is_start(v, prev, i, n) << 32) + (uint64_t)seg_is_end(v, next, i, n);
 }
 
 struct seg_records {
@@ -176,17 +145,56 @@
     int64_t nrec;
 };
 
+#define SEG_TILE 4096
+static_assert(SEG_TILE == 256 * 16 && SEG_TILE >= SCAN_TILE, "seg kernels: 256 threads x 16 labels; the workspace is sized by SCAN_TILE");
+
+__device__ __forceinline__ uint32_t seg_byte(const uint32_t w[4], int j) { return (w[j >> 2] >> (8 * (j & 3))) & 0xffu; }
+
+__device__ __forceinline__ void seg_load16(const uint8_t *p, int64_t n, int64_t i0, uint32_t w[4])
+{
+    if (i0 >= 0 && i0 + 16 <= n && ((uintptr_t)(p + i0) & 15) == 0) {
+        const uint4 x = *(const uint4 *)(p + i0);
+        w[0] = x.x; w[1] = x.y; w[2] = x.z; w[3] = x.w;
+    } else {
+        w[0] = w[1] = w[2] = w[3] = 0;
+#pragma unroll
+        for (int j = 0; j < 16; ++j) {
+            const int64_t i = i0 + j;
+            if (i >= 0 && i < n) w[j >> 2] |= (uint32_t)p[i] << (8 * (j & 3));
+        }
+    }
+}
+
+template <bool BATCH>
+__device__ __forceinline__ void seg_thread_flags(const int8_t *lab, const uint8_t *marks, int64_t n, int64_t i0, uint32_t w[4],
+                                                 uint32_t &st, uint32_t &en)
+{
+    uint32_t m[4] = { 0, 0, 0, 0 };
+    seg_load16((const uint8_t *)lab, n, i0, w);
+    if (BATCH) seg_load16(marks, n, i0, m);
+    const int lane = threadIdx.x & 63;
+    uint32_t prev = __shfl_up(w[3] >> 24, 1), next = __shfl_down(w[0] & 0xffu, 1);
+    if (lane == 0) prev = i0 >= 1 && i0 - 1 < n ? (uint8_t)lab[i0 - 1] : 0;
+    if (lane == 63) next = i0 + 16 >= 0 && i0 + 16 < n ? (uint8_t)lab[i0 + 16] : 0;
+    st = en = 0;
+#pragma unroll
+    for (int j = 0; j < 16; ++j) {
+        const uint32_t v = seg_byte(w, j), p = j ? seg_byte(w, j - 1) : prev, q = j < 15 ? seg_byte(w, j + 1) : next;
+        const uint64_t f = seg_flags<BATCH>((int8_t)v, (int8_t)p, (int8_t)q, (uint8_t)seg_byte(m, j), i0 + j, n);
+        st |= (uint32_t)(f >> 32) << j;
+        en |= (uint32_t)(f & 1) << j;
+    }
+}
+
 template <bool BATCH>
 __global__ void __launch_bounds__(256) seg_count_kernel(const int8_t *__restrict__ lab, const uint8_t *__restrict__ marks, int64_t n,
-                                                        uint64_t *__restrict__ tilecnt)
+                                                        int mis, uint64_t *__restrict__ tilecnt)
 {
     __shared__ uint64_t lds[4];
-    const int64_t base = (int64_t)blockIdx.x * SCAN_TILE;
-    uint64_t c = 0;
-    for (int j = 0; j < 8; ++j) {
-        const int64_t i = base + j * 256 + threadIdx.x;
-        if (i < n) c += seg_flags<BATCH>(lab, marks, i, n);
-    }
+    const int64_t i0 = (int64_t)blockIdx.x * SEG_TILE + (int64_t)threadIdx.x * 16 - mis;
+    uint32_t w[4], st, en;
+    seg_thread_flags<BATCH>(lab, marks, n, i0, w, st, en);
+    uint64_t c = ((uint64_t)__popc(st) << 32) + (uint64_t)__popc(en);
     for (int o = 32; o > 0; o >>= 1) c += __shfl_xor(c, o);
     if ((threadIdx.x & 63) == 0) lds[threadIdx.x >> 6] = c;
     __syncthreads();
@@ -195,42 +203,38 @@
 
 template <bool BATCH>
 __global__ void __launch_bounds__(256) seg_emit_kernel(const int8_t *__restrict__ lab, const uint8_t *__restrict__ marks, int64_t n,
-                                                       int64_t offset, int32_t contig, seg_records recs,
+                                                       int mis, int64_t offset, int32_t contig, seg_records recs,
                                                        const uint64_t *__restrict__ tileoff, dgrp_segment *__restrict__ rec, int64_t cap)
 {
     __shared__ uint64_t lds[4];
-    const int64_t base = (int64_t)blockIdx.x * SCAN_TILE + (int64_t)threadIdx.x * 8;
-    uint64_t f[8], s = 0;
-    for (int j = 0; j < 8; ++j) {
-        const int64_t i = base + j;
-        f[j] = i < n ? seg_flags<BATCH>(lab, marks, i, n) : 0;
-        s += f[j];
-    }
-    uint64_t ex = block_exclusive_scan(s, nullptr, lds) + tileoff[blockIdx.x];
-    for (int j = 0; j < 8; ++j) {
-        const int64_t i = base + j;
-        if (f[j]) {
-            int64_t off = offset;
-            int32_t tag = contig;
-            if (BATCH) {
-                int64_t lo = 0, hi = recs.nrec;
-                while (hi - lo > 1) {
-                    const int64_t mid = (lo + hi) >> 1;
-                    if (recs.start[mid] <= i) lo = mid; else hi = mid;
-                }
-                off = recs.startpos[lo] - recs.start[lo];
-                tag = recs.contig[lo];
+    const int64_t i0 = (int64_t)blockIdx.x * SEG_TILE + (int64_t)threadIdx.x * 16 - mis;
+    uint32_t w[4], st, en;
+    seg_thread_flags<BATCH>(lab, marks, n, i0, w, st, en);
+    const uint64_t s = ((uint64_t)__popc(st) << 32) + (uint64_t)__popc(en);
+    const uint64_t ex = block_exclusive_scan(s, nullptr, lds) + tileoff[blockIdx.x];
+    int64_t ks = (int64_t)(ex >> 32), ke = (int64_t)(ex & 0xffffffffull);
+    for (uint32_t both = st | en; both; both &= both - 1) {
+        const int j = __ffs(both) - 1;
+        const int64_t i = i0 + j;
+        int64_t off = offset;
+        int32_t tag = contig;
+        if (BATCH) {
+            int64_t lo = 0, hi = recs.nrec;
+            while (hi - lo > 1) {
+                const int64_t mid = (lo + hi) >> 1;
+                if (recs.start[mid] <= i) lo = mid; else hi = mid;
             }
-            if (f[j] >> 32) {
-                const int64_t k = (int64_t)(ex >> 32);
-                if (k < cap) { rec[k].start = i + off; rec[k].label = lab[i]; rec[k].contig = tag; }
-            }
-            if (f[j] & 1) {
-                const int64_t k = (int64_t)(ex & 0xffffffffull);
-                if (k < cap) rec[k].end = i + 1 + off;
-            }
-        }
-        ex += f[j];
+            off = recs.startpos[lo] - recs.start[lo];
+            tag = recs.contig[lo];
+        }
+        if ((st >> j) & 1) {
+            if (ks < cap) { rec[ks].start = i + off; rec[ks].label = (int8_t)seg_byte(w, j); rec[ks].contig = tag; }
+            ++ks;
+        }
+        if ((en >> j) & 1) {
+            if (ke < cap) rec[ke].end = i + 1 + off;
+            ++ke;
+        }
     }
 }
 
@@ -278,13 +282,14 @@
         dgrp_set_error("dgrp_batch_segments: workspace too small");
         return DGRP_ENOMEM;
     }
-    const int64_t ntiles = (total_n + SCAN_TILE - 1) / SCAN_TILE;
+    const int mis = (int)((uintptr_t)d_labels & 15);
+    const int64_t ntiles = (total_n + mis + SEG_TILE - 1) / SEG_TILE;
     uint64_t *tiles = (uint64_t *)d_work;
     uint64_t *grand = tiles + ntiles + 1;
-    hipLaunchKernelGGL(seg_count_kernel<true>, dim3((unsigned)ntiles), dim3(256), 0, stream, d_labels, d_marks, total_n, tiles);
-    hipLaunchKernelGGL(scan_sums_kernel, dim3(1), dim3(256), 0, stream, tiles, ntiles, grand);
-    hipLaunchKernelGGL(seg_emit_kernel<true>, dim3((unsigned)ntiles), dim3(256), 0, stream, d_labels, d_marks, total_n, (int64_t)0,
-                       (int32_t)0, seg_records{ d_start, d_startpos, d_contig, nrec }, tiles, d_records, cap);
+    hipLaunchKernelGGL(seg_count_kernel<true>, dim3((unsigned)ntiles), dim3(256), 0, stream, d_labels, d_marks, total_n, mis, tiles);
+    hipLaunchKernelGGL(scan_sums_kernel, dim3(1), dim3(SCAN_SUMS_THREADS), 0, stream, tiles, ntiles, grand);
+    hipLaunchKernelGGL(seg_emit_kernel<true>, dim3((unsigned)ntiles), dim3(256), 0, stream, d_labels, d_marks, total_n, mis,
+                       (int64_t)0, (int32_t)0, seg_records{ d_start, d_startpos, d_contig, nrec }, tiles, d_records, cap);
     hipLaunchKernelGGL(seg_total_kernel, dim3(1), dim3(1), 0, stream, grand, d_count);
     DGRP_LAUNCH_CHECK();
     return DGRP_OK;
@@ -310,15 +315,17 @@
         dgrp_set_error("dgrp_segments: workspace too small");
         return DGRP_ENOMEM;
     }
-    const int64_t ntiles = (n + SCAN_TILE - 1) / SCAN_TILE;
+    const int mis = (int)((uintptr_t)d_labels & 15);
+    const int64_t ntiles = (n + mis + SEG_TILE - 1) / SEG_TILE;
     uint64_t *tiles = (uint64_t *)d_work;
     uint64_t *grand = tiles + ntiles + 1;
-    hipLaunchKernelGGL(seg_count_kernel<false>, dim3((unsigned)ntiles), dim3(256), 0, stream, d_labels, (const uint8_t *)nullptr, n, tiles);
-    DGRP_LAUNCH_CHECK();
-    hipLaunchKernelGGL(scan_sums_kernel, dim3(1), dim3(256), 0, stream, tiles, ntiles, grand);
-    DGRP_LAUNCH_CHECK();
-    hipLaunchKernelGGL(seg_emit_kernel<false>, dim3((unsigned)ntiles), dim3(256), 0, stream, d_labels, (const uint8_t *)nullptr, n, offset,
-                       contig, seg_records{ nullptr, nullptr, nullptr, 0 }, tiles, d_records, cap);
+    hipLaunchKernelGGL(seg_count_kernel<false>, dim3((unsigned)ntiles), dim3(256), 0, stream, d_labels, (const uint8_t *)nullptr, n, mis,
+                       tiles);
+    DGRP_LAUNCH_CHECK();
+    hipLaunchKernelGGL(scan_sums_kernel, dim3(1), dim3(SCAN_SUMS_THREADS), 0, stream, tiles, ntiles, grand);
+    DGRP_LAUNCH_CHECK();
+    hipLaunchKernelGGL(seg_emit_kernel<false>, dim3((unsigned)ntiles), dim3(256), 0, stream, d_labels, (const uint8_t *)nullptr, n, mis,
+                       offset, contig, seg_records{ nullptr, nullptr, nullptr, 0 }, tiles, d_records, cap);
     DGRP_LAUNCH_CHECK();
     hipLaunchKernelGGL(seg_total_kernel, dim3(1), dim3(1), 0, stream, grand, d_count);
     DGRP_LAUNCH_CHECK();
diff --git a/deepgrp_amd/csrc/scan.h b/deepgrp_amd/csrc/scan.h
--- a/deepgrp_amd/csrc/scan.h
+++ b/deepgrp_amd/csrc/scan.h
@@ -13,6 +13,7 @@
 
 #define SCAN_TILE 2048
 
+template <int WAVES = 4>
 __device__ __forceinline__ uint64_t block_exclusive_scan(uint64_t v, uint64_t *total, uint64_t *lds)
 {
     const int lane = threadIdx.x & 63, wave = threadIdx.x >> 6;
@@ -24,9 +25,14 @@
     }
     if (lane == 63) lds[wave] = x;
     __syncthreads();
-    uint64_t base = 0;
-    for (int w = 0; w < wave; ++w) base += lds[w];
-    if (total) *total = lds[0] + lds[1] + lds[2] + lds[3];
+    uint64_t base = 0, all = 0;
+#pragma unroll
+    for (int w = 0; w < WAVES; ++w) {
+        const uint64_t t = lds[w];
+        if (w < wave) base += t;
+        all += t;
+    }
+    if (total) *total = all;
     __syncthreads();
     return base + x - v;
 }
@@ -46,16 +52,25 @@
     if (threadIdx.x == 0) tilesum[blockIdx.x] = lds[0] + lds[1] + lds[2] + lds[3];
 }
 
-__global__ void __launch_bounds__(256) scan_sums_kernel(uint64_t *__restrict__ tilesum, int64_t ntiles, uint64_t *__restrict__ grand)
+#define SCAN_SUMS_THREADS 1024
+#define SCAN_SUMS_ITEMS 8
+
+__global__ void __launch_bounds__(SCAN_SUMS_THREADS) scan_sums_kernel(uint64_t *__restrict__ tilesum, int64_t ntiles, uint64_t *__restrict__ grand)
 {
-    __shared__ uint64_t lds[4];
+    __shared__ uint64_t lds[SCAN_SUMS_THREADS / 64];
     uint64_t carry = 0;
-    for (int64_t base = 0; base < ntiles; base += 256) {
-        const int64_t i = base + threadIdx.x;
-        const uint64_t v = i < ntiles ? tilesum[i] : 0;
+    for (int64_t base = 0; base < ntiles; base += SCAN_SUMS_THREADS * SCAN_SUMS_ITEMS) {
+        const int64_t i0 = base + (int64_t)threadIdx.x * SCAN_SUMS_ITEMS;
+        uint64_t v[SCAN_SUMS_ITEMS], s = 0;
+#pragma unroll
+        for (int j = 0; j < SCAN_SUMS_ITEMS; ++j) { v[j] = i0 + j < ntiles ? tilesum[i0 + j] : 0; s += v[j]; }
         uint64_t tot;
-        const uint64_t ex = block_exclusive_scan(v, &tot, lds);
-        if (i < ntiles) tilesum[i] = carry + ex;
+        uint64_t ex = carry + block_exclusive_scan<SCAN_SUMS_THREADS / 64>(s, &tot, lds);
+#pragma unroll
+        for (int j = 0; j < SCAN_SUMS_ITEMS; ++j) {
+            if (i0 + j < ntiles) tilesum[i0 + j] = ex;
+            ex += v[j];
+        }
         carry += tot;
     }
     if (threadIdx.x == 0 && grand) *grand = carry;
@@ -85,7 +100,7 @@
     const int64_t ntiles = (n + SCAN_TILE - 1) / SCAN_TILE;
     hipLaunchKernelGGL(scan_tilesum_kernel, dim3((unsigned)ntiles), dim3(256), 0, stream, in, n, tiles);
     DGRP_LAUNCH_CHECK();
-    hipLaunchKernelGGL(scan_sums_kernel, dim3(1), dim3(256), 0, stream, tiles, ntiles, grand);
+    hipLaunchKernelGGL(scan_sums_kernel, dim3(1), dim3(SCAN_SUMS_THREADS), 0, stream, tiles, ntiles, grand);
     DGRP_LAUNCH_CHECK();
     hipLaunchKernelGGL(scan_apply_kernel, dim3((unsigned)ntiles), dim3(256), 0, stream, in, n, tiles, out);
     DGRP_LAUNCH_CHECK();
diff --git a/deepgrp_amd/csrc/score_transform.h b/deepgrp_amd/csrc/score_transform.h
--- /dev/null
+++ b/deepgrp_amd/csrc/score_transform.h
@@ -0,0 +1,42 @@
+#pragma once
+#include "dgrp_common.h"
+#include <math.h>
+
+__device__ __forceinline__ float np_logf(float xin)
+{
+    const uint32_t bits = __float_as_uint(xin);
+    float k = (float)((int)(bits >> 23) - 126);
+    float m = __uint_as_float((bits & 0x007fffffu) | 0x3f000000u);
+    if (m <= 0.70710678118654752440f) { m = m + m; k = k - 1.0f; }
+    const float x = m - 1.0f;
+    float den = fmaf(5.875095403124574342950e-03f, x, 1.546476374983906719538e-01f);
+    den = fmaf(den, x, 9.864942958519418960339e-01f);
+    den = fmaf(den, x, 2.453006071784736363091e+00f);
+    den = fmaf(den, x, 2.612677543073109236779e+00f);
+    den = fmaf(den, x, 1.0f);
+    float num = fmaf(2.589979117907922693523e-02f, x, 3.808837741388407920751e-01f);
+    num = fmaf(num, x, 1.480000633576506585156e+00f);
+    num = fmaf(num, x, 2.112677543073053063722e+00f);
+    num = fmaf(num, x, 9.999999999999998702752e-01f);
+    num = fmaf(num, x, 0.0f);
+    return fmaf(k, 0.693147180559945309417232121458176568f, __fdiv_rn(num, den));
+}
+
+__device__ __forceinline__ float row_first_max(const float *p, int C, int &a)
+{
+    a = 0;
+    float mx = p[0];
+    for (int c = 1; c < C; ++c) {
+        const float v = p[c];
+        if (v > mx) { mx = v; a = c; }
+    }
+    return mx;
+}
+
+__device__ __forceinline__ float score_of_max(float mx, int a)
+{
+    float m = mx + 1e-6f;
+    if (m > 0.99f) m = 0.99f;
+    const float t = np_logf(__fdiv_rn(m, 1.0f - m));
+    return a > 0 ? t : -10.0f * t;
+}
diff --git a/deepgrp_amd/csrc/track_kernels.hip b/deepgrp_amd/csrc/track_kernels.hip
--- a/deepgrp_amd/csrc/track_kernels.hip
+++ b/deepgrp_amd/csrc/track_kernels.hip
@@ -332,7 +332,7 @@
     const int64_t tpc = D->tpc, ntiles = D->ntiles;
     hipLaunchKernelGGL(tb_count_kernel, dim3((unsigned)ntiles), dim3(256), 0, stream, q, d_recs, d_pref, G, tiles);
     DGRP_LAUNCH_CHECK();
-    hipLaunchKernelGGL(scan_sums_kernel, dim3(1), dim3(256), 0, stream, tiles, ntiles, grand);
+    hipLaunchKernelGGL(scan_sums_kernel, dim3(1), dim3(SCAN_SUMS_THREADS), 0, stream, tiles, ntiles, grand);
     DGRP_LAUNCH_CHECK();
     hipLaunchKernelGGL(tb_bounds_kernel, dim3(1), dim3(128), 0, stream, tiles, tpc, ncls, grand, bounds);
     DGRP_LAUNCH_CHECK();
@@ -735,7 +735,7 @@
     hipLaunchKernelGGL(ix_tile_kernel<1>, grid, block, 0, stream, D.q, D.recs, D.pref, d_wpref, D.G, W, D.tiles, D.bounds, state, tilechunks,
                        cbounds, d_chunks, d_linear);
     DGRP_LAUNCH_CHECK();
-    hipLaunchKernelGGL(scan_sums_kernel, dim3(1), block, 0, stream, tilechunks, D.ntiles, cgrand);
+    hipLaunchKernelGGL(scan_sums_kernel, dim3(1), dim3(SCAN_SUMS_THREADS), 0, stream, tilechunks, D.ntiles, cgrand);
     DGRP_LAUNCH_CHECK();
     hipLaunchKernelGGL(tb_bounds_kernel, dim3(1), dim3(128), 0, stream, tilechunks, D.tpc, ncls, cgrand, cbounds);
     DGRP_LAUNCH_CHECK();
diff --git a/deepgrp_amd/pipeline.py b/deepgrp_amd/pipeline.py
--- a/deepgrp_amd/pipeline.py
+++ b/deepgrp_amd/pipeline.py
@@ -356,8 +356,12 @@
         if self.use_mss:
             scores = torch.empty(n, dtype=torch.float64, device=dev)
             cls = torch.empty(n, dtype=torch.int8, device=dev)
-            check(L.dgrp_scores(_ptr(merged), n, c, _ptr(scores), _ptr(cls), stream_ptr()), "dgrp_scores")
-            return self.labels_from_scores(scores, cls)
+            labels = torch.empty(n, dtype=torch.int8, device=dev)
+            wb = L.dgrp_mss_workspace_bytes(n)
+            work = torch.empty(wb, dtype=torch.uint8, device=dev)
+            check(L.dgrp_scores_mss_labels(_ptr(merged), n, c, self.min_mss_len, self.xdrop_len, _ptr(scores), _ptr(cls), _ptr(labels),
+                                           None, _ptr(work), wb, stream_ptr()), "dgrp_scores_mss_labels")
+            return labels
         labels = torch.empty(n, dtype=torch.int8, device=dev)
         work = torch.empty(4096, dtype=torch.uint8, device=dev)
         check(L.dgrp_softmax_labels(_ptr(merged), n, c, None, _ptr(labels), _ptr(work), work.numel(),
diff --git a/include/deepgrp_hip.h b/include/deepgrp_hip.h
--- a/include/deepgrp_hip.h
+++ b/include/deepgrp_hip.h
@@ -135,6 +135,14 @@
 int dgrp_mss_labels(const double *d_scores, const int8_t *d_cls, int64_t n, int nof_labels,
                     int min_mss_len, int xdrop_len, int8_t *d_labels_out, int64_t *d_nseg,
                     void *d_work, int64_t work_bytes, void *stream);
+int dgrp_mss_blockstats(const double *d_scores, int64_t n, uint64_t *d_blk, double *d_blk_sum,
+                        double *d_blk_abs, int32_t *d_blk_q, uint8_t *d_flags, void *stream);
+int dgrp_scores_blockstats(const float *d_probs, int64_t n, int C, double *d_scores, int8_t *d_cls,
+                           uint64_t *d_blk, double *d_blk_sum, double *d_blk_abs, int32_t *d_blk_q,
+                           uint8_t *d_flags, void *stream);
+int dgrp_scores_mss_labels(const float *d_probs, int64_t n, int C, int min_mss_len, int xdrop_len,
+                           double *d_scores, int8_t *d_cls, int8_t *d_labels_out, int64_t *d_nseg,
+                           void *d_work, int64_t work_bytes, void *stream);
 int dgrp_mss_segments_host(const void *d_work, int64_t work_bytes, int32_t *h_st_en, int64_t cap,
                            int64_t *n_seg);
 
```

New measurement: 567.7 (median of 6 runs). No clear change (+0.5%).
